# LANL-Bioinformatics/FaQCs

Measured on AMD Instinct MI355X. Metric: M reads/sec (paired 2x150bp), higher is better.
Workload: dtype u8; 1 GPU; synthetic 100M-pair 2x150bp Q33 reads resident in HBM per GPU, BWA_plus -q 5 --min_L 50, 1 step = 1 pass (trim_lds + counter all-reduce); pairs_per_gpu=100000000, read_len=150, terminal_n_supplied=True

## Files before the change

faqcs_amd/csrc/faqcs_capi.hip:

```cpp
#include "faqcs_ctx.h"

static uint8_t na_to_bits_host(char c)
{
    switch (c) {
    case 'A': case 'a': return 1;  case 'C': case 'c': return 2;  case 'G': case 'g': return 4;
    case 'T': case 't': return 8;  case 'M': case 'm': return 3;  case 'R': case 'r': return 5;
    case 'S': case 's': return 6;  case 'V': case 'v': return 7;  case 'W': case 'w': return 9;
    case 'Y': case 'y': return 10; case 'H': case 'h': return 11; case 'K': case 'k': return 12;
    case 'D': case 'd': return 13; case 'B': case 'b': return 14; case 'N': case 'n': return 15;
    case '-': return 16;
    }
    return 0;
}

static void build_tables(const faqcs_params &p, std::vector<uint32_t> &lcthr, std::vector<int32_t> &avgq,
                         std::vector<float> &norm, std::vector<uint32_t> &magic, std::vector<uint32_t> &base)
{
    const int N = FAQCS_TAB_LEN + 1;
    lcthr.assign(N, 0xffffffffu); avgq.assign(N, 0); norm.assign(N, 0.f); magic.assign(N, 0);
    const volatile float lc = p.low_complexity_cutoff_ratio;
    const volatile float avg = p.average_quality;
    for (int len = 1; len < N; ++len) {
        uint32_t mono = 0xffff, di = 0xffff;
        volatile float nrm = (float)(1.0 / (double)len);
// ... 40 lines not shown
    if (p->n_adapters > FAQCS_MAX_ADAPTERS)
        return fail(FAQCS_E_INVAL, "faqcs_create: " + std::to_string(p->n_adapters) + " adapters, at most " + std::to_string(FAQCS_MAX_ADAPTERS) + " are supported");
    if (p->mode < 0 || p->mode > 2) return fail(FAQCS_E_INVAL, "trim.cpp:trim_read: Undefined trimming mode!");
    if (p->quality < -93 || p->quality > 93) return fail(FAQCS_E_INVAL, "faqcs_create: quality threshold outside [-93, 93]");
    if (p->kmer_rarefaction && (p->kmer < 2 || p->kmer > 31 || p->split_size == 0)) return fail(FAQCS_E_INVAL, "faqcs_create: kmer / split_size out of range");
    int ndev = 0;
    if (hipGetDeviceCount(&ndev) != hipSuccess || ndev == 0)
        return fail(FAQCS_E_NODEVICE, "faqcs_create: no HIP device (the FaQCs MI355X hot path has no CPU fallback)");
    if (device_id < 0) HIPCHK(hipGetDevice(&device_id));
    HIPCHK(hipSetDevice(device_id));
    std::unique_ptr<faqcs_ctx, void (*)(faqcs_ctx *)> guard(new faqcs_ctx(), faqcs_destroy);
    faqcs_ctx *c = guard.get();
    c->prm = *p;
    c->prm.adapter_seq = nullptr;
    c->device = device_id;
    hipDeviceProp_t prop;
    HIPCHK(hipGetDeviceProperties(&prop, device_id));
    c->n_cu = prop.multiProcessorCount > 0 ? prop.multiProcessorCount : 256;
    HIPCHK(hipStreamCreateWithFlags(&c->compute, hipStreamNonBlocking));
    HIPCHK(hipStreamCreateWithFlags(&c->copy, hipStreamNonBlocking));
    HIPCHK(hipStreamCreateWithFlags(&c->aux, hipStreamNonBlocking));
    for (auto &rs : c->rec) { HIPCHK(hipEventCreateWithFlags(&rs.trimmed, hipEventDisableTiming)); HIPCHK(hipEventCreateWithFlags(&rs.folded, hipEventDisableTiming)); }
    HIPCHK(hipEventCreateWithFlags(&c->copied, hipEventDisableTiming));
    for (auto &sl : c->slot) HIPCHK(hipEventCreateWithFlags(&sl.done, hipEventDisableTiming));
    for (auto &e : c->ticket_ev) HIPCHK(hipEventCreateWithFlags(&e, hipEventDisableTiming));
    faqcs_counters_layout(p->max_read_length, p->n_adapters, &c->lay);

    std::vector<uint32_t> lcthr, magic, basetab; std::vector<int32_t> avgq; std::vector<float> norm;
    build_tables(*p, lcthr, avgq, norm, magic, basetab);
    HIPCHK(upload(&c->d_lcthr, lcthr)); HIPCHK(upload(&c->d_avgq, avgq)); HIPCHK(upload(&c->d_norm, norm));
    HIPCHK(upload(&c->d_magic, magic)); HIPCHK(upload(&c->d_basetab, basetab));
    HIPCHK(hipMalloc((void **)&c->d_counters, c->lay.total * sizeof(uint64_t)));
    HIPCHK(hipMemset(c->d_counters, 0, c->lay.total * sizeof(uint64_t)));
    HIPCHK(hipMalloc((void **)&c->d_err, 256));
    HIPCHK(hipMemset(c->d_err, 0, 256));
    {
        const size_t dwords = (size_t)c->n_cu * FAQCS_PARTIAL_FLUSHES * FAQCS_PARTIAL_ROW + (size_t)c->n_cu;
        HIPCHK(hipMalloc((void **)&c->d_partials, dwords * sizeof(uint32_t)));
        HIPCHK(hipMemset(c->d_partials, 0, dwords * sizeof(uint32_t)));
    }

    if (p->n_adapters) {
        std::vector<uint8_t> bits; std::vector<uint32_t> start(1, 0);
        for (uint32_t j = 0; j < p->n_adapters; ++j) {
            const char *s = p->adapter_seq[j];
            const size_t L = strlen(s);
            if (L == 0 || L > FAQCS_MAX_ADAPTER_LENGTH)
                return fail(FAQCS_E_INVAL, "faqcs_create: adapter " + std::to_string(j) + " has " + std::to_string(L) + " bases, 1 ... " +
                                               std::to_string(FAQCS_MAX_ADAPTER_LENGTH) + " are supported");
            c->adapters.emplace_back(s);
            for (size_t k = 0; k < L; ++k) {
                const uint8_t b = na_to_bits_host(s[k]);
                if (!b) return fail(FAQCS_E_BASE, "seq_overlap.cpp:na_to_bits: Unknown base!");
                bits.push_back(b);
            }
            start.push_back((uint32_t)bits.size());
        }
        std::vector<uint32_t> planes, wstart(1, 0);
        for (uint32_t j = 0; j < p->n_adapters; ++j) {
            const uint32_t L = start[j + 1] - start[j], nw = (L + 31) / 32;
            for (uint32_t w = 0; w < nw; ++w) {
                uint32_t pl[4] = {0, 0, 0, 0};
                for (uint32_t k = 0; k < 32 && 32 * w + k < L; ++k)
                    for (int b = 0; b < 4; ++b) pl[b] |= (uint32_t)((bits[start[j] + 32 * w + k] >> b) & 1u) << k;
                planes.insert(planes.end(), pl, pl + 4);
            }
            wstart.push_back(wstart.back() + nw);
        }
        HIPCHK(upload(&c->d_abits, bits)); HIPCHK(upload(&c->d_astart, start));
        HIPCHK(upload(&c->d_aplanes, planes)); HIPCHK(upload(&c->d_awstart, wstart));
        c->adapter_plane_dwords = (uint32_t)planes.size();
        for (uint32_t j = 0; j < p->n_adapters; ++j) c->adapter_longest = std::max(c->adapter_longest, start[j + 1] - start[j]);
        c->match_rate = (float)(1.0 - (double)p->filterAdapterMismatchRate);
        if (p->n_adapters > FAQCS_ADAPTER_GROUP || c->adapter_longest > FAQCS_ADAPTER_SINGLE_LENGTH) {
            std::vector<uint32_t> wgrp;
            for (uint32_t j = 0; j < p->n_adapters;) {
                faqcs_ctx::AdapterGroupHost g{j, 0, wstart[j], 0, 0};
                while (j < p->n_adapters && g.n < FAQCS_ADAPTER_GROUP && 4u * (wstart[j + 1] - g.w0) <= FAQCS_ADAPTER_TPL_CAP) {
                    g.longest = std::max(g.longest, start[j + 1] - start[j]);
                    ++g.n; ++j;
                }
                g.plane_dwords = 4u * (wstart[j] - g.w0);
                for (uint32_t k = g.j0; k <= j; ++k) wgrp.push_back(wstart[k] - g.w0);
                c->agroups.push_back(g);
            }
            HIPCHK(upload(&c->d_awstart_grp, wgrp));
        }
    }

    DevParams &d = c->dp;
    memset(&d, 0, sizeof(d));
    d.mode = p->mode; d.Q = p->quality; d.in_off = p->input_quality_offset; d.out_off = p->output_quality_offset;
    auto cap16 = [](uint32_t v) { return v > 65535u ? 65535u : v; };
    d.min_len = cap16(p->min_read_length); d.max_poly_n = cap16(p->max_num_poly_N); d.trim5 = cap16(p->trim_5); d.trim3 = cap16(p->trim_3);
    d.replace_q = p->replace_to_N_q; d.protect5 = p->protect_5; d.qc_only = p->qc_only;
    d.has_adapters = p->n_adapters ? 1 : 0; d.avgq_on = p->average_quality > 0.0f ? 1 : 0;
    d.R = p->max_read_length; d.n_adapters = p->n_adapters;
    d.lc_ratio = p->low_complexity_cutoff_ratio; d.avg_q = p->average_quality;
    if (const char *e = getenv("FAQCS_DBG")) d.dbg = (uint32_t)strtoul(e, nullptr, 0);
    d.lc_thr = c->d_lcthr; d.avgq_min_v = c->d_avgq; d.comp_norm = c->d_norm; d.div_magic = c->d_magic; d.base_tab = c->d_basetab;
    d.partials = c->d_partials;
    d.partial_rows = c->d_partials + (size_t)c->n_cu * FAQCS_PARTIAL_FLUSHES * FAQCS_PARTIAL_ROW;
    d.lay = c->lay;

    c->kmer_active = p->kmer_rarefaction ? 1 : 0;
    if (p->kmer_rarefaction) {
        uint64_t slots = p->kmer_table_slots ? p->kmer_table_slots : (1ull << 28);
        uint64_t pow2 = 1; while (pow2 < slots) pow2 <<= 1;
        if (pow2 < (uint64_t)KG_SLICE_MIN << 16) pow2 = (uint64_t)KG_SLICE_MIN << 16;
        if (pow2 > (uint64_t)KG_SLICE_MAX << 16) return fail(FAQCS_E_INVAL, "faqcs_create: kmer_table_slots above 2^32");
        c->kt.mask = pow2 - 1;
        { uint32_t lg = 0; while ((1ull << lg) < pow2) ++lg; if (lg > 46) return fail(FAQCS_E_INVAL, "faqcs_create: kmer_table_slots too large"); c->kt.shift = 62 - lg; }
        if (const char *e = getenv("FAQCS_KMER_DIRECT")) c->kg.direct = atoi(e) != 0;
        c->kt.ovf_mask = std::max<uint64_t>(pow2 >> 4, 1ull << 16) - 1;
        { const uint32_t lg = 62 - c->kt.shift;
          int f = (int)lg - 27; f = f < 0 ? 0 : (f > 3 ? 3 : f);
          if (const char *e = getenv("FAQCS_KMER_FINE_BITS")) { const int v = atoi(e); if (v >= 0 && v <= 3) f = v; }
          while (f > 0 && (pow2 >> (16 + f)) < 16) --f;
          while (f < 3 && (pow2 >> (16 + f)) > (uint64_t)KG_SLICE_MAX / 8) ++f;
          c->kt.fine = (uint32_t)f; }
        HIPCHK(hipMalloc((void **)&c->kt.dirty, (size_t)(1u << (16 + c->kt.fine)) / 8));
        HIPCHK(hipMemset(c->kt.dirty, 0, (size_t)(1u << (16 + c->kt.fine)) / 8));
        HIPCHK(hipMalloc((void **)&c->kt.slots, kmer_table_total(c->kt) * sizeof(KmerSlot)));
        HIPCHK(hipMalloc((void **)&c->kt.stats, 64));
        HIPCHK(faqcs_launch_kmer_table_init(c->kt, c->n_cu, c->compute));
        HIPCHK(hipMemset(c->kt.stats, 0, 64));
        c->snap_cap = 4096;
        HIPCHK(hipMalloc((void **)&c->d_snaps, c->snap_cap * 16));
    }
    *out = guard.release();
    return 0;
}

extern "C" void faqcs_destroy(faqcs_ctx *c)
{
    if (!c) return;
    (void)hipSetDevice(c->device);
    if (c->compute) (void)hipStreamSynchronize(c->compute);
    if (c->copy) (void)hipStreamSynchronize(c->copy);
    if (c->aux) (void)hipStreamSynchronize(c->aux);
    for (auto &t : c->timings) { (void)hipEventDestroy(t.a); (void)hipEventDestroy(t.b); (void)hipEventDestroy(t.p); (void)hipEventDestroy(t.k0); (void)hipEventDestroy(t.k1); }
    if (c->comm) comm_release(c->comm);
    if (c->comm_ev) (void)hipEventDestroy(c->comm_ev);
    c->emit.release(); c->parse.release(); c->render.release(); c->inflate.release(); c->deflate.release();
    if (c->ins_a) (void)hipEventDestroy(c->ins_a);
    if (c->ins_b) (void)hipEventDestroy(c->ins_b);
    for (int k = 0; k < 2; ++k) { if (c->fwd_free[k]) (void)hipEventDestroy(c->fwd_free[k]); if (c->fwd_copied[k]) (void)hipEventDestroy(c->fwd_copied[k]); c->fwd_items[k].release(); }
    void *ptrs[] = {c->d_lcthr, c->d_basetab, c->d_avgq, c->d_norm, c->d_magic, c->d_counters, c->d_err, c->d_partials, c->d_abits, c->d_astart, c->d_aplanes, c->d_awstart,
                    c->d_awstart_grp, c->kt.slots, c->kt.stats, c->kt.dirty, c->d_fold_claim, c->d_snaps, c->d_ob, c->d_tot_by_epoch, c->d_first_hist};
    for (void *q : ptrs) if (q) (void)hipFree(q);
    for (auto &sl : c->slot) { sl.seq.release(); sl.qual.release(); sl.tn.release(); sl.off.release(); if (sl.done) (void)hipEventDestroy(sl.done); }
    for (auto &e : c->ticket_ev) if (e) (void)hipEventDestroy(e);
    c->s_seg.release(); c->s_sl.release(); c->s_hit.release(); c->s_res.release(); c->s_astate.release(); c->s_amask.release();
    for (auto &rs : c->rec) { rs.pre.release(); rs.post.release(); if (rs.trimmed) (void)hipEventDestroy(rs.trimmed); if (rs.folded) (void)hipEventDestroy(rs.folded); }
    if (c->aux) (void)hipStreamDestroy(c->aux);
    c->ob_items.release(); c->ob_wave_count.release(); c->ob_wave_offset.release();
    { void *kg_ptrs[] = {c->kg.dev.l1, c->kg.dev.l2, c->kg.dev.cur1, c->kg.dev.cur2, c->kg.dev.run_epoch, c->kg.dev.first_hist, c->kg.dev.tot_by_epoch, c->kg.dev.dense, c->kg.dev.big, c->kg.dev.n_big, c->kg.dev.redo};
      for (void *q : kg_ptrs) if (q) (void)hipFree(q);
      c->kg.defer.release();
      c->ks.l1.release(); c->ks.spill.release(); c->ks.cur1.release(); c->ks.run_epoch.release(); c->ks.defer.release(); c->ks.scratch.release();
      for (auto &ev : c->kg.flush_ev) { (void)hipEventDestroy(ev.first); (void)hipEventDestroy(ev.second); } }
    if (c->copied) (void)hipEventDestroy(c->copied);
    if (c->compute) (void)hipStreamDestroy(c->compute);
    if (c->copy) (void)hipStreamDestroy(c->copy);
    delete c;
}

extern "C" int faqcs_set_quality(faqcs_ctx *c, int quality)
{
    if (!c) return fail(FAQCS_E_INVAL, "null ctx");
    if (quality < -93 || quality > 93) return fail(FAQCS_E_INVAL, "faqcs_set_quality: quality threshold outside [-93, 93]");
    c->prm.quality = quality;
    c->dp.Q = quality;
    return 0;
}

static int take_timing(faqcs_ctx *c, Timing *&tm)
{
    if (c->timing_used == c->timings.size()) {
        Timing t; HIPCHK(hipEventCreate(&t.a)); HIPCHK(hipEventCreate(&t.b)); HIPCHK(hipEventCreate(&t.p)); HIPCHK(hipEventCreate(&t.k0)); HIPCHK(hipEventCreate(&t.k1));
        t.adapter = false; t.kmer = false; c->timings.push_back(t);
    }
    tm = &c->timings[c->timing_used++];
    tm->adapter = c->prm.n_adapters != 0;
    tm->kmer = false;
    return 0;
}

static int enqueue_adapter(faqcs_ctx *c, Timing &t, const Submission &s)
{
    const uint32_t n = s.n;
    HIPCHK(hipEventRecord(t.p, c->compute));
    HIPCHK(c->s_sl.reserve(n)); HIPCHK(c->s_hit.reserve(n)); HIPCHK(c->s_seg.reserve(s.n_seg + 1));
    HIPCHK(hipMemcpyAsync(c->s_seg.p, s.seg, (s.n_seg + 1) * 4, hipMemcpyHostToDevice, c->compute));
    auto launch = [&](const AdapterDev &A, const AdapterGroup *G) {
        return faqcs_launch_adapter(A, G, s.seq, s.off, n, s.max_len, c->s_seg.p, s.n_seg, c->s_sl.p, c->s_hit.p,
                                    c->d_counters + c->lay.adapter_stats, c->d_err, c->dp.dbg, c->n_cu, c->compute);
    };
    if (c->agroups.empty()) {
        AdapterDev A{c->d_abits, c->d_astart, c->d_aplanes, c->d_awstart, c->prm.n_adapters, c->match_rate, c->adapter_longest, c->adapter_plane_dwords};
        HIPCHK(launch(A, nullptr));
        return 0;
    }
    AdapterGroup G{};
    G.mask_words = (s.max_len + 63) / 64;
    HIPCHK(c->s_astate.reserve(n)); HIPCHK(c->s_amask.reserve((size_t)n * G.mask_words));
    HIPCHK(hipMemsetAsync(c->s_astate.p, 0, (size_t)n * sizeof(uint4), c->compute));
    G.state = c->s_astate.p; G.mask = c->s_amask.p; G.gstart = c->d_astart;
    for (size_t k = 0; k < c->agroups.size(); ++k) {
        const faqcs_ctx::AdapterGroupHost &g = c->agroups[k];
        AdapterDev A{c->d_abits, c->d_astart + g.j0, c->d_aplanes + 4 * (size_t)g.w0, c->d_awstart_grp + g.j0 + k, g.n, c->match_rate,
                     g.longest, g.plane_dwords};
        G.j0 = g.j0; G.last = k + 1 == c->agroups.size() ? 1u : 0u;
        HIPCHK(launch(A, &G));
    }
    return 0;
}

static int enqueue_trim(faqcs_ctx *c, Timing &t, const Submission &s, const uint32_t *d_sl, const uint16_t *d_hit)
{
    const uint32_t n = s.n, max_len = s.max_len;
    HIPCHK(hipEventRecord(t.a, c->compute));
    const bool wide = max_len > 256;
    const int set = (int)(c->n_enqueued++ & 1);
    faqcs_ctx::RecSet &rs = c->rec[set];
    if (rs.used) { HIPCHK(hipStreamWaitEvent(c->compute, rs.folded, 0)); rs.used = false; }
    const char *e_long = getenv("FAQCS_TRIM_LONG");
    const bool force_long = e_long && atoi(e_long) != 0;
    const bool long_reads = max_len > FAQCS_FAST_READ_LENGTH || force_long;
    const size_t need = long_reads ? (size_t)n / 2 + 1 : (size_t)n * (wide ? 2 : 1);
    if (need > rs.pre.cap) { HIPCHK(hipStreamSynchronize(c->aux)); HIPCHK(hipStreamSynchronize(c->compute)); }
    HIPCHK(rs.pre.reserve(need)); HIPCHK(rs.post.reserve(need));
    DevParams dp = c->dp;
    static const bool tail_on = [] { const char *e = getenv("FAQCS_TAIL_FOLD"); return !e || atoi(e) != 0; }();
    if (c->pending_fold >= 0 && !c->pending_wide && tail_on) {
        const faqcs_ctx::RecSet &ps = c->rec[c->pending_fold];
        if (!c->d_fold_claim) HIPCHK(hipMalloc((void **)&c->d_fold_claim, 8));
        HIPCHK(hipMemsetAsync(c->d_fold_claim, 0, 8, c->compute));
        dp.fold_pre = ps.pre.p; dp.fold_post = ps.post.p; dp.fold_n = c->pending_n; dp.fold_claim = c->d_fold_claim;
        dp.fold_dst_pre = c->d_counters + c->lay.pre_comp; dp.fold_dst_post = c->d_counters + c->lay.post_comp;
    }
    HIPCHK(faqcs_launch_trim(dp, s.seq, s.qual, s.off, n, max_len, d_sl, d_hit, s.res, rs.pre.p, rs.post.p,
                             c->d_counters, c->d_err, c->n_cu, c->compute, s.tn));
    HIPCHK(hipEventRecord(t.b, c->compute));
    c->trim_kernel = faqcs_last_trim_kernel();
    if (c->pending_fold >= 0) {
        if (!(dp.fold_n && faqcs_last_trim_folded())) {
            faqcs_ctx::RecSet &ps = c->rec[c->pending_fold];
            HIPCHK(hipStreamWaitEvent(c->aux, ps.trimmed, 0));
            HIPCHK(faqcs_launch_composition(ps.pre.p, ps.post.p, c->pending_n, c->pending_wide, c->d_norm, c->d_counters + c->lay.pre_comp,
                                            c->d_counters + c->lay.post_comp, c->n_cu, c->aux));
            HIPCHK(hipEventRecord(ps.folded, c->aux));
            ps.used = true;
        }
        c->pending_fold = -1;
    }
    static const bool no_comp = [] { const char *e = getenv("FAQCS_DIAG_NO_COMPOSITION"); return e && atoi(e) != 0; }();
    if (!(c->dp.dbg & 1u) && !long_reads && !no_comp) {
        HIPCHK(hipEventRecord(rs.trimmed, c->compute));
        c->pending_fold = set; c->pending_n = n; c->pending_wide = wide;
    }
    return 0;
}

static int enqueue(faqcs_ctx *c, const uint8_t *d_seq, const uint8_t *d_qual, const uint32_t *d_off, uint32_t n,
                   uint32_t max_len, const uint32_t *seg, uint32_t n_seg, faqcs_read_result *d_res, const uint8_t *d_tn = nullptr,
                   const uint32_t *host_off = nullptr)
{
    const Submission s{d_seq, d_qual, d_tn, d_off, seg, host_off, n, max_len, n_seg, d_res};
    Timing *tm = nullptr;
    const bool adapters = s.n && c->prm.n_adapters;
    if (s.n) { if (int rc = take_timing(c, tm)) return rc; }
    if (adapters) { if (int rc = enqueue_adapter(c, *tm, s)) return rc; }
    if (s.n) { if (int rc = enqueue_trim(c, *tm, s, adapters ? c->s_sl.p : nullptr, adapters ? c->s_hit.p : nullptr)) return rc; }
    return enqueue_kmers(c, tm, s);
}

static int scan_offsets(const uint32_t *off, uint32_t n, uint32_t cap, uint32_t *max_len)
{
    uint32_t m = 0;
    for (uint32_t i = 0; i < n; ++i) {
        if (off[i + 1] < off[i]) return fail(FAQCS_E_INVAL, "faqcs_submit: offsets must be non-decreasing");
        const uint32_t l = off[i + 1] - off[i];
        m = l > m ? l : m;
    }
    if (m > cap) return fail(FAQCS_E_INVAL, "faqcs_submit: read longer than max_read_length");
    if (m > FAQCS_MAX_READ_LENGTH) return fail(FAQCS_E_INVAL, "faqcs_submit: reads longer than FAQCS_MAX_READ_LENGTH bases are not supported by the HIP kernels");
    *max_len = m;
    return 0;
}

static int check_segments(const faqcs_batch *b)
{
    if (!b || !b->offset) return fail(FAQCS_E_INVAL, "faqcs_submit: null batch");
    if (!b->segment_start || b->segment_start[0] != 0 || b->segment_start[b->n_segments] != b->n_reads)
        return fail(FAQCS_E_INVAL, "faqcs_submit: segment_start must span [0, n_reads]");
    for (uint32_t s = 0; s < b->n_segments; ++s)
        if (b->segment_start[s + 1] < b->segment_start[s]) return fail(FAQCS_E_INVAL, "faqcs_submit: segment_start must be non-decreasing");
    return 0;
}

extern "C" int faqcs_submit_async(faqcs_ctx *c, const faqcs_batch *b, faqcs_read_result *results, uint64_t *ticket)
{
    if (!c) return fail(FAQCS_E_INVAL, "null ctx");
    if (int rc = check_segments(b)) return rc;
    HIPCHK(hipSetDevice(c->device));
    const uint32_t n = b->n_reads;
    uint32_t max_len = 0;
    if (int rc = scan_offsets(b->offset, n, c->prm.max_read_length, &max_len)) return rc;
    const uint32_t o0 = b->offset[0], o1 = b->offset[n];
    const size_t bytes = (size_t)(o1 - o0);
    faqcs_ctx::Slot &sl = c->slot[c->n_submits & 1];
    hipEvent_t tk = c->ticket_ev[c->n_submits & 7];
    if (c->n_submits >= 8) HIPCHK(hipEventSynchronize(tk));
    if (sl.used) {
        if (bytes + FAQCS_ARENA_PAD_BEFORE + FAQCS_ARENA_PAD_AFTER > sl.seq.cap || (size_t)n + 1 > sl.off.cap || (b->terminal_n && (size_t)n + 64 > sl.tn.cap)) HIPCHK(hipEventSynchronize(sl.done));
        else HIPCHK(hipStreamWaitEvent(c->copy, sl.done, 0));
    }
    HIPCHK(sl.seq.reserve(bytes + FAQCS_ARENA_PAD_BEFORE + FAQCS_ARENA_PAD_AFTER)); HIPCHK(sl.qual.reserve(bytes + FAQCS_ARENA_PAD_BEFORE + FAQCS_ARENA_PAD_AFTER)); HIPCHK(sl.off.reserve((size_t)n + 1));
    if (b->terminal_n) HIPCHK(sl.tn.reserve((size_t)n + 64));
    if ((size_t)n + 1 > c->s_res.cap) HIPCHK(hipStreamSynchronize(c->compute));
    HIPCHK(c->s_res.reserve((size_t)n + 1));
    if (bytes) {
        HIPCHK(hipMemcpyAsync(sl.seq.p + 16, b->seq + o0, bytes, hipMemcpyHostToDevice, c->copy));
        HIPCHK(hipMemcpyAsync(sl.qual.p + 16, b->qual + o0, bytes, hipMemcpyHostToDevice, c->copy));
    }
    HIPCHK(hipMemcpyAsync(sl.off.p, b->offset, ((size_t)n + 1) * 4, hipMemcpyHostToDevice, c->copy));
    const uint8_t *d_tn = nullptr;
    if (b->terminal_n && n) {
        HIPCHK(hipMemcpyAsync(sl.tn.p, b->terminal_n, n, hipMemcpyHostToDevice, c->copy));
        d_tn = sl.tn.p;
    }
    HIPCHK(hipEventRecord(c->copied, c->copy));
    HIPCHK(hipStreamWaitEvent(c->compute, c->copied, 0));
    const uint8_t *d_seq = sl.seq.p + 16 - o0, *d_qual = sl.qual.p + 16 - o0;
    if (int rc = enqueue(c, d_seq, d_qual, sl.off.p, n, max_len, b->segment_start, b->n_segments, c->s_res.p, d_tn, b->offset)) return rc;
    if (n && results) HIPCHK(hipMemcpyAsync(results, c->s_res.p, (size_t)n * sizeof(faqcs_read_result), hipMemcpyDeviceToHost, c->compute));
    HIPCHK(hipEventRecord(sl.done, c->compute));
    HIPCHK(hipEventRecord(tk, c->compute));
    sl.used = true;
    if (ticket) *ticket = c->n_submits;
    ++c->n_submits;
    return 0;
}

extern "C" int faqcs_submit(faqcs_ctx *c, const faqcs_batch *b, faqcs_read_result *results)
{
    return faqcs_submit_async(c, b, results, nullptr);
}

extern "C" int faqcs_wait(faqcs_ctx *c, uint64_t ticket)
{
    if (!c) return fail(FAQCS_E_INVAL, "null ctx");
    if (ticket >= c->n_submits) return fail(FAQCS_E_INVAL, "faqcs_wait: unknown ticket");
    if (ticket + 8 < c->n_submits) return 0;
    HIPCHK(hipEventSynchronize(c->ticket_ev[ticket & 7]));
    return 0;
}

extern "C" void *faqcs_host_alloc(size_t bytes)
{
    void *p = nullptr;
    if (hipHostMalloc(&p, bytes, hipHostMallocPortable) != hipSuccess) return nullptr;
    return p;
}

extern "C" void faqcs_host_free(void *p)
{
    if (p) (void)hipHostFree(p);
}

extern "C" int faqcs_submit_device(faqcs_ctx *c, const faqcs_batch *b, faqcs_read_result *d_results)
{
    if (!c) return fail(FAQCS_E_INVAL, "null ctx");
    if (!b || !b->segment_start) return fail(FAQCS_E_INVAL, "faqcs_submit_device: null batch");
    HIPCHK(hipSetDevice(c->device));
    const uint32_t n = b->n_reads;
    uint32_t max_len = b->max_read_len ? b->max_read_len : c->prm.max_read_length;
    if (max_len > c->prm.max_read_length) return fail(FAQCS_E_INVAL, "faqcs_submit_device: max_read_len exceeds the context capacity");
    if (max_len > FAQCS_MAX_READ_LENGTH) return fail(FAQCS_E_INVAL, "faqcs_submit_device: reads longer than FAQCS_MAX_READ_LENGTH bases are not supported by the HIP kernels");
    if (!d_results) { HIPCHK(c->s_res.reserve((size_t)n + 1)); d_results = c->s_res.p; }
    return enqueue(c, b->seq, b->qual, b->offset, n, max_len, b->segment_start, b->n_segments, d_results, b->terminal_n);
}

extern "C" int faqcs_terminal_n_flags(int device_id, const uint8_t *d_seq, const uint32_t *d_offset, uint32_t n_reads, uint8_t *d_flags)
{
    if (!d_seq || !d_offset || !d_flags) return fail(FAQCS_E_INVAL, "null argument");
    if (device_id >= 0) HIPCHK(hipSetDevice(device_id));
    HIPCHK(faqcs_launch_terminal_n_flags(d_seq, d_offset, n_reads, d_flags, nullptr));
    HIPCHK(hipDeviceSynchronize());
    return 0;
}

int fold_pending_now(faqcs_ctx *c)
{
    if (c->pending_fold < 0) return 0;
    faqcs_ctx::RecSet &ps = c->rec[c->pending_fold];
    HIPCHK(faqcs_launch_composition(ps.pre.p, ps.post.p, c->pending_n, c->pending_wide, c->d_norm, c->d_counters + c->lay.pre_comp,
                                    c->d_counters + c->lay.post_comp, c->n_cu, c->compute));
    c->pending_fold = -1;
    return 0;
}

extern "C" int faqcs_sync(faqcs_ctx *c)
{
    if (!c) return fail(FAQCS_E_INVAL, "null ctx");
    HIPCHK(hipSetDevice(c->device));
    HIPCHK(hipStreamSynchronize(c->copy));
    if (int rc = fold_pending_now(c)) return rc;
    HIPCHK(hipStreamSynchronize(c->compute));
    HIPCHK(hipStreamSynchronize(c->aux));
    for (size_t i = 0; i < c->kg.flush_ev_used; ++i) {
        float ms = 0.f;
        if (hipEventElapsedTime(&ms, c->kg.flush_ev[i].first, c->kg.flush_ev[i].second) == hipSuccess) c->kmer_flush_ms += ms;
    }
    c->kg.flush_ev_used = 0;
    for (size_t i = 0; i < c->timing_used; ++i) {
        float ms = 0.f;
        if (hipEventElapsedTime(&ms, c->timings[i].a, c->timings[i].b) == hipSuccess) { c->kernel_ms += ms; ++c->kernel_launches; }
        if (c->timings[i].kmer && hipEventElapsedTime(&ms, c->timings[i].k0, c->timings[i].k1) == hipSuccess) c->kmer_ms += ms;
        if (c->timings[i].adapter && hipEventElapsedTime(&ms, c->timings[i].p, c->timings[i].a) == hipSuccess) c->adapter_ms += ms;
    }
    c->timing_used = 0;
    if (int rc = resolve_points(c)) return rc;
    uint32_t e = 0;
    HIPCHK(hipMemcpy(&e, c->d_err, 4, hipMemcpyDeviceToHost));
    if (e & 1u) return fail(FAQCS_E_QUALITY, "fastq.h:quality_score: Found a quality score value that is greater than the maximum allowed quality score");
    if (e & 2u) return fail(FAQCS_E_BASE, "seq_overlap.cpp:na_to_bits: Unknown base!");
    if (e & 4u) return fail(FAQCS_E_INVAL, "faqcs: internal error, the trim kernel's LDS block does not start at address 0");
    if (c->kt.stats) {
        unsigned long long st[3];
        HIPCHK(hipMemcpy(st, c->kt.stats, 24, hipMemcpyDeviceToHost));
        if (st[2] & 2ull) return fail(FAQCS_E_NOMEM, "faqcs: the k-mer exchange staging overflowed (more runs of k-mers per read than it is sized for): submit smaller batches");
        if (st[2]) return fail(FAQCS_E_KMER_FULL, "faqcs: device k-mer table is full (raise faqcs_params.kmer_table_slots)");
    }
    return 0;
}

extern "C" int faqcs_counters_device(faqcs_ctx *c, void **d_ptr, uint64_t *n_u64)
{
    if (!c || !d_ptr || !n_u64) return fail(FAQCS_E_INVAL, "null argument");
    *d_ptr = c->d_counters;
    *n_u64 = c->lay.total;
    return 0;
}

static int counters_copy(faqcs_ctx *c, void *d_dst, const void *d_src)
{
    HIPCHK(hipSetDevice(c->device));
    if (int rc = fold_pending_now(c)) return rc;
    HIPCHK(hipStreamSynchronize(c->aux));
    HIPCHK(hipMemcpyAsync(d_dst, d_src, c->lay.total * sizeof(uint64_t), hipMemcpyDeviceToDevice, c->compute));
    HIPCHK(hipStreamSynchronize(c->compute));
    return 0;
}

extern "C" int faqcs_counters_export(faqcs_ctx *c, void *d_dst, uint64_t n_u64)
{
    if (!c || !d_dst || n_u64 < c->lay.total) return fail(FAQCS_E_INVAL, "faqcs_counters_export: buffer too small");
    return counters_copy(c, d_dst, c->d_counters);
}

extern "C" int faqcs_counters_import(faqcs_ctx *c, const void *d_src, uint64_t n_u64)
{
    if (!c || !d_src || n_u64 < c->lay.total) return fail(FAQCS_E_INVAL, "faqcs_counters_import: buffer too small");
    return counters_copy(c, c->d_counters, d_src);
}

extern "C" int faqcs_finish(faqcs_ctx *c, uint64_t *counters, uint64_t n_u64)
{
    if (!c || !counters || n_u64 < c->lay.total) return fail(FAQCS_E_INVAL, "faqcs_finish: counter buffer too small");
    if (int rc = faqcs_sync(c)) return rc;
    HIPCHK(hipMemcpy(counters, c->d_counters, c->lay.total * sizeof(uint64_t), hipMemcpyDeviceToHost));
    return 0;
}

extern "C" int faqcs_reset_counters(faqcs_ctx *c)
{
    if (!c) return fail(FAQCS_E_INVAL, "null ctx");
    HIPCHK(hipSetDevice(c->device));
    c->pending_fold = -1;
    HIPCHK(hipStreamSynchronize(c->aux));
    HIPCHK(hipMemsetAsync(c->d_counters, 0, c->lay.total * sizeof(uint64_t), c->compute));
    return 0;
}

static int synth_fill_impl(int device_id, uint8_t *d_seq, uint8_t *d_qual, uint32_t *d_offset, uint32_t n_reads, uint32_t L,
                           uint64_t seed, uint64_t first_read, float adapter_frac, uint64_t genome_len)
{
    if (device_id >= 0) HIPCHK(hipSetDevice(device_id));
    if ((uint64_t)n_reads * L + L > 0xffffffffull) return fail(FAQCS_E_INVAL, "faqcs_synth_fill: arena exceeds 32-bit offsets");
    const char *at = getenv("FAQCS_SYNTH_AT");
    HIPCHK(faqcs_launch_synth(d_seq, d_qual, d_offset, n_reads, L, seed, first_read, adapter_frac, genome_len, at ? (float)atof(at) : -1.0f, nullptr));
    HIPCHK(hipDeviceSynchronize());
    return 0;
}

extern "C" int faqcs_synth_fill(int device_id, uint8_t *d_seq, uint8_t *d_qual, uint32_t *d_offset, uint32_t n_reads,
                                uint32_t L, uint64_t seed, uint64_t first_read, float adapter_frac)
{
    return synth_fill_impl(device_id, d_seq, d_qual, d_offset, n_reads, L, seed, first_read, adapter_frac, 0);
}

extern "C" int faqcs_synth_fill_genome(int device_id, uint8_t *d_seq, uint8_t *d_qual, uint32_t *d_offset, uint32_t n_reads,
                                       uint32_t L, uint64_t seed, uint64_t first_read, uint64_t genome_len)
{
    if (genome_len <= L) return fail(FAQCS_E_INVAL, "faqcs_synth_fill_genome: the genome must be longer than a read");
    return synth_fill_impl(device_id, d_seq, d_qual, d_offset, n_reads, L, seed, first_read, 0.f, genome_len);
}

extern "C" int faqcs_debug_words(faqcs_ctx *c, uint64_t *out, uint32_t n)
{
    if (!c || !out || n > 16) return fail(FAQCS_E_INVAL, "faqcs_debug_words: bad argument");
    HIPCHK(hipSetDevice(c->device));
    HIPCHK(hipStreamSynchronize(c->compute));
    HIPCHK(hipMemcpy(out, reinterpret_cast<const uint8_t *>(c->d_err) + 64, (size_t)n * 8, hipMemcpyDeviceToHost));
    HIPCHK(hipMemset(reinterpret_cast<uint8_t *>(c->d_err) + 64, 0, 128));
    return 0;
}

extern "C" int faqcs_kernel_report(faqcs_ctx *c, faqcs_kernel_times *out)
{
    if (!c || !out) return fail(FAQCS_E_INVAL, "null argument");
    if (int rc = faqcs_sync(c)) return rc;
    out->n_launches = c->kernel_launches;
    out->trim_ms = c->kernel_launches ? c->kernel_ms / (double)c->kernel_launches : 0.0;
    out->adapter_ms = c->kernel_launches ? c->adapter_ms / (double)c->kernel_launches : 0.0;
    out->trim_kernel = c->trim_kernel;
    out->kmer_ms = c->kernel_launches ? (c->kmer_ms + c->kmer_flush_ms) / (double)c->kernel_launches : 0.0;
    out->kmer_insert_ms = c->kernel_launches ? c->kmer_insert_ms / (double)c->kernel_launches : 0.0;
    c->kernel_ms = 0.0; c->adapter_ms = 0.0; c->kmer_ms = 0.0; c->kmer_insert_ms = 0.0; c->kmer_flush_ms = 0.0; c->kernel_launches = 0;
    return 0;
}

extern "C" int faqcs_kernel_time_ms(faqcs_ctx *c, double *avg_ms, uint64_t *n_launches)
{
    faqcs_kernel_times t;
    if (!c || !avg_ms || !n_launches) return fail(FAQCS_E_INVAL, "null argument");
    if (int rc = faqcs_kernel_report(c, &t)) return rc;
    *n_launches = t.n_launches; *avg_ms = t.trim_ms;
    return 0;
}
```

faqcs_amd/csrc/faqcs_ctx.h:

```cpp
#pragma once
#include <hip/hip_runtime.h>

#include <algorithm>
#include <cmath>
#include <cstdio>
#include <cstdlib>
#include <cstring>
#include <map>
#include <memory>
#include <string>
#include <vector>

#include "faqcs_dev.h"
#include "faqcs_host.h"
#include "faqcs_kmer.h"
#include "faqcs_skm.h"

struct AdapterDev {
    const uint8_t *bits;
    const uint32_t *start, *planes, *wstart;
    uint32_t n_adapters;
    float match_rate;
    uint32_t longest, plane_dwords;
};
const char *faqcs_last_trim_kernel();
bool faqcs_last_trim_folded();
hipError_t faqcs_launch_trim(const DevParams &P, const uint8_t *seq, const uint8_t *qual, const uint32_t *off,
                             uint32_t n_reads, uint32_t max_len, const uint32_t *ad_sl, const uint16_t *ad_hit,
                             faqcs_read_result *out, unsigned long long *rec_pre, unsigned long long *rec_post,
                             uint64_t *counters, uint32_t *err, int n_cu, hipStream_t st, const uint8_t *tn_flags);
hipError_t faqcs_launch_terminal_n_flags(const uint8_t *seq, const uint32_t *off, uint32_t n_reads, uint8_t *flags, hipStream_t st);
hipError_t faqcs_launch_composition(const unsigned long long *rec_pre, const unsigned long long *rec_post, uint32_t n, bool wide,
                                    const float *comp_norm, uint64_t *dst_pre, uint64_t *dst_post, int n_cu, hipStream_t st);
hipError_t faqcs_launch_adapter(const AdapterDev &A, const AdapterGroup *G, const uint8_t *seq, const uint32_t *off, uint32_t n_reads,
                                uint32_t max_len, const uint32_t *seg_start, uint32_t n_segments, uint32_t *ad_sl,
                                uint16_t *ad_hit, uint64_t *adapter_stats, uint32_t *err, uint32_t dbg, int n_cu, hipStream_t st);
hipError_t faqcs_launch_synth(uint8_t *d_seq, uint8_t *d_qual, uint32_t *d_offset, uint32_t n_reads, uint32_t L,
                              uint64_t seed, uint64_t first_read, float adapter_frac, uint64_t genome_len, float at_frac, hipStream_t st);

size_t faqcs_emit_scratch_bytes(uint32_t n_reads);
hipError_t faqcs_launch_emit_scan(const uint8_t *seq, const uint32_t *off, const uint8_t *tn, uint32_t n_reads, const faqcs_read_result *res,
                                  const uint8_t *keep, const faqcs_emit_out *out, void *scratch, hipStream_t st);
hipError_t faqcs_launch_emit_gather(const uint8_t *seq, const uint8_t *qual, uint32_t n_reads, const faqcs_emit_out *out, const void *scratch,
                                    int in_off, int out_off, uint32_t replace_q, int n_cu, hipStream_t st);

size_t faqcs_parse_scratch_bytes(unsigned long long n_text);
hipError_t faqcs_launch_parse_index(const uint8_t *text, unsigned long long n_text, int final, void *scratch, hipStream_t st);
hipError_t faqcs_launch_parse_records(const uint8_t *text, unsigned long long n_text, const faqcs_parse_out *out, void *scratch, int n_cu, hipStream_t st);
hipError_t faqcs_launch_parse_gather(const uint8_t *text, unsigned long long n_text, const faqcs_parse_out *out, const void *scratch, int n_cu, hipStream_t st);

size_t faqcs_render_scratch_bytes(uint32_t n_reads);
hipError_t faqcs_launch_render_scan(const faqcs_batch *b, const faqcs_read_result *res, const uint32_t *def_pos, const uint32_t *def_len,
                                    const uint8_t *select, const uint32_t *order, const faqcs_render_out *out, void *scratch, hipStream_t st);
hipError_t faqcs_launch_render_gather(const faqcs_batch *b, bool trimmed, const uint8_t *text, const faqcs_render_out *out, const void *scratch,
                                      int in_off, int out_off, uint32_t replace_q, int n_cu, hipStream_t st);

size_t faqcs_inflate_scratch_bytes(uint32_t n_members);
hipError_t faqcs_launch_inflate_scan(const uint8_t *comp, unsigned long long n_comp, const uint32_t *moff, uint32_t n, const faqcs_inflate_out *out, void *scratch, hipStream_t st);
hipError_t faqcs_launch_inflate_decode(const uint8_t *comp, const uint32_t *moff, uint32_t n, const faqcs_inflate_out *out, void *scratch, int n_cu, hipStream_t st);
size_t faqcs_deflate_scratch_bytes(uint32_t n, uint32_t n_data, uint32_t member_bytes, int n_cu);
hipError_t faqcs_launch_deflate_encode(const uint8_t *text, unsigned long long n_text, uint32_t member_bytes, uint32_t n, uint32_t n_data, void *scratch, int n_cu, hipStream_t st);
hipError_t faqcs_launch_deflate_gather(uint32_t member_bytes, uint32_t n, uint32_t n_data, const faqcs_deflate_out *out, void *scratch, int n_cu, hipStream_t st);

#define HIPCHK(x)                                                                                         \
    do {                                                                                                  \
        hipError_t e_ = (x);                                                                              \
        if (e_ != hipSuccess)                                                                             \
            return fail(FAQCS_E_NODEVICE, std::string(#x) + ": " + hipGetErrorString(e_));                \
    } while (0)

struct faqcs_ctx;

#pragma GCC visibility push(hidden)

template <class T> struct DevBuf {
    T *p = nullptr;
    size_t cap = 0;
    hipError_t reserve(size_t n)
    {
        if (n <= cap) return hipSuccess;
        if (p) (void)hipFree(p);
        p = nullptr; cap = 0;
        const size_t want = n + n / 4 + 64;
        hipError_t e = hipMalloc((void **)&p, want * sizeof(T));
        if (e == hipSuccess) cap = want;
        return e;
    }
    void release() { if (p) (void)hipFree(p); p = nullptr; cap = 0; }
};

struct Timing { hipEvent_t a, b, p, k0, k1; bool adapter, kmer; };

struct PackStage {
    DevBuf<uint4> scratch;
    hipEvent_t ev[3] = {nullptr, nullptr, nullptr};
    hipStream_t st = nullptr;
    bool timed = false;
    int begin(faqcs_ctx *c, size_t scratch_bytes);
    int mark(int i);
    int times(faqcs_ctx *c, const char *not_yet, double *first_ms, double *second_ms);
    void release();
};

#pragma GCC visibility pop

struct faqcs_ctx {
    faqcs_params prm;
    int device = 0, n_cu = 256;
    hipStream_t compute = nullptr, copy = nullptr;
    hipEvent_t copied = nullptr;
    DevParams dp;
    faqcs_layout lay;
    uint32_t *d_lcthr = nullptr, *d_magic = nullptr, *d_basetab = nullptr;
    int32_t *d_avgq = nullptr;
    float *d_norm = nullptr;
    uint64_t *d_counters = nullptr;
    uint32_t *d_err = nullptr;
    uint32_t *d_partials = nullptr;
    std::vector<std::string> adapters;
    uint8_t *d_abits = nullptr;
    uint32_t *d_astart = nullptr, *d_aplanes = nullptr, *d_awstart = nullptr;
    float match_rate = 0.f;
    uint32_t adapter_longest = 0, adapter_plane_dwords = 0;
    struct AdapterGroupHost { uint32_t j0, n, w0, longest, plane_dwords; };
    std::vector<AdapterGroupHost> agroups;
    uint32_t *d_awstart_grp = nullptr;
    DevBuf<uint4> s_astate;
    DevBuf<uint64_t> s_amask;
    struct Slot { DevBuf<uint8_t> seq, qual, tn; DevBuf<uint32_t> off; hipEvent_t done = nullptr; bool used = false; };
    Slot slot[2];
    uint64_t n_submits = 0;
    hipEvent_t ticket_ev[8] = {nullptr, nullptr, nullptr, nullptr, nullptr, nullptr, nullptr, nullptr};
    DevBuf<uint32_t> s_seg, s_sl;
    DevBuf<uint16_t> s_hit;
    DevBuf<faqcs_read_result> s_res;
    PackStage emit;
    PackStage parse;
    PackStage render;
    PackStage inflate;
    PackStage deflate;
    struct RecSet { DevBuf<unsigned long long> pre, post; hipEvent_t trimmed = nullptr, folded = nullptr; bool used = false; };
    RecSet rec[2];
    uint64_t n_enqueued = 0;
    int pending_fold = -1;
    uint32_t pending_n = 0;
    bool pending_wide = false;
    uint32_t *d_fold_claim = nullptr;
    hipStream_t aux = nullptr;
    uint64_t total_number = 0;
    int kmer_active = 0;
    std::vector<faqcs_rarefaction> points;
    struct PendingPoint { size_t point_index; size_t snap_index; };
    std::vector<PendingPoint> pending;
    KmerTable kt{nullptr, 0, nullptr, 0};
    bool partitioned = false;
    uint32_t part_rank = 0, part_world = 1, n_epochs = 0;
    std::vector<uint32_t> seg_epoch;
    DevBuf<ulonglong2> ob_items;
    bool ob_fresh = false;
    DevBuf<uint32_t> ob_wave_count;
    DevBuf<unsigned long long> ob_wave_offset;
    unsigned long long *d_ob = nullptr;
    unsigned long long *d_tot_by_epoch = nullptr, *d_first_hist = nullptr;
    unsigned long long *d_snaps = nullptr;
    size_t snap_cap = 0, n_snaps = 0;
    std::map<uint64_t, uint64_t> kmer_hist;
    struct KmerGroup {
        bool ready = false;
        bool direct = false;
        bool owner = false;
        bool skm = false;
        uint32_t skm_w = 1;
        DevBuf<uint32_t> defer;
        uint64_t cap_items = 0;
        uint64_t bound_items = 0;
        std::vector<uint32_t> run_epoch, upload[2];
        unsigned n_flushes = 0;
        uint64_t n_launches = 0;
        uint32_t epoch_base = 0;
        std::vector<uint64_t> sub_fill;
        KmerGroupDev dev{};
        uint32_t ep_cap = 0;
        uint32_t ep_used = 0;
        size_t points_final = 0;
        std::vector<std::pair<hipEvent_t, hipEvent_t>> flush_ev; size_t flush_ev_used = 0;
        bool table_live = false;
        bool pass_done = false;
        bool pass_used = false;
        bool hist_in_table = false;
        bool hist_in_overflow = false;
        uint64_t last_distinct = 0, last_total = 0;
    } kg;
    struct KmerSend {
        KmerGroupDev dev{};
        DevBuf<ulonglong2> l1, spill;
        DevBuf<uint32_t> cur1, run_epoch, defer;
        DevBuf<unsigned long long> scratch;
        uint32_t *spill_n = nullptr;
    } ks;
    std::vector<Timing> timings;
    size_t timing_used = 0;
    double kernel_ms = 0.0, adapter_ms = 0.0, kmer_ms = 0.0, kmer_insert_ms = 0.0, kmer_flush_ms = 0.0;
    uint64_t kernel_launches = 0;
    hipEvent_t ins_a = nullptr, ins_b = nullptr;
    DevBuf<ulonglong2> fwd_items[2];
    hipEvent_t fwd_free[2] = {nullptr, nullptr}, fwd_copied[2] = {nullptr, nullptr};
    unsigned fwd_n = 0;
    const char *trim_kernel = "";
    void *comm = nullptr;
    hipEvent_t comm_ev = nullptr;
};

struct Submission {
    const uint8_t *seq, *qual, *tn;
    const uint32_t *off, *seg, *host_off;
    uint32_t n, max_len, n_seg;
    faqcs_read_result *res;
};

FAQCS_HIDDEN int fold_pending_now(faqcs_ctx *c);
FAQCS_HIDDEN int enqueue_kmers(faqcs_ctx *c, Timing *tm, const Submission &s);
FAQCS_HIDDEN int resolve_points(faqcs_ctx *c);
FAQCS_HIDDEN void comm_release(void *comm);
```

faqcs_amd/csrc/faqcs_dev.h:

```cpp
#pragma once
#include <hip/hip_runtime.h>
#include <stdint.h>

#include "../../include/faqcs_mi.h"

#define FAQCS_WAVE 64
#define FAQCS_FAST_READ_LENGTH 1024
#define FAQCS_TAB_LEN FAQCS_FAST_READ_LENGTH

struct DevParams {
    int32_t mode, Q, in_off, out_off;
    uint32_t min_len, max_poly_n, trim5, trim3, replace_q;
    uint32_t protect5, qc_only, has_adapters, avgq_on;
    uint32_t R;
    uint32_t n_adapters;
    uint32_t dbg;
    uint32_t wide_records;
    float lc_ratio, avg_q;
    const uint32_t *lc_thr;
    const int32_t  *avgq_min_v;
    const uint32_t *div_magic;
    const float    *comp_norm;
    const uint32_t *base_tab;
    uint32_t *partials;
    uint32_t *partial_rows;
    faqcs_layout lay;
    const unsigned long long *fold_pre, *fold_post;
    uint32_t fold_n;
    uint32_t *fold_claim;
    uint64_t *fold_dst_pre, *fold_dst_post;
};

#define FAQCS_ADAPTER_GROUP 64
#define FAQCS_ADAPTER_TPL_CAP 4096
#define FAQCS_ADAPTER_SINGLE_LENGTH 8192

struct AdapterGroup {
    uint4 *state;
    uint64_t *mask;
    const uint32_t *gstart;
    uint32_t j0;
    uint32_t mask_words;
    uint32_t last;
};

enum { FS_SLOTS = 32 };
enum { FAQCS_PARTIAL_ROW = 16896 };
enum { FAQCS_PARTIAL_FLUSHES = 8 };

#define BT_SHIFT(code) (6 * (code))
#define BT_FIELDS 0x3fffffffu
#define BT_IS_NU (1u << 31)
#define BT_IS_GU (1u << 30)

#define CR_VALID (1ull << 63)

#ifdef __HIPCC__
__device__ __forceinline__ uint32_t umax_(uint32_t a, uint32_t b) { return a > b ? a : b; }
__device__ __forceinline__ uint32_t umin_(uint32_t a, uint32_t b) { return a < b ? a : b; }
__device__ __forceinline__ int uni(int v) { return __builtin_amdgcn_readfirstlane(v); }
__device__ __forceinline__ uint32_t uniu(uint32_t v) { return (uint32_t)__builtin_amdgcn_readfirstlane((int)v); }

__device__ __forceinline__ int wave_incl_scan_add(int v)
{
    v += __builtin_amdgcn_update_dpp(0, v, 0x111, 0xf, 0xf, false);
    v += __builtin_amdgcn_update_dpp(0, v, 0x112, 0xf, 0xf, false);
    v += __builtin_amdgcn_update_dpp(0, v, 0x114, 0xf, 0xf, false);
    v += __builtin_amdgcn_update_dpp(0, v, 0x118, 0xf, 0xf, false);
    v += __builtin_amdgcn_update_dpp(0, v, 0x142, 0xa, 0xf, false);
    v += __builtin_amdgcn_update_dpp(0, v, 0x143, 0xc, 0xf, false);
    return v;
}
__device__ __forceinline__ uint32_t wave_max_u32(uint32_t v)
{
    v = umax_(v, (uint32_t)__builtin_amdgcn_update_dpp(0, (int)v, 0x111, 0xf, 0xf, false));
    v = umax_(v, (uint32_t)__builtin_amdgcn_update_dpp(0, (int)v, 0x112, 0xf, 0xf, false));
    v = umax_(v, (uint32_t)__builtin_amdgcn_update_dpp(0, (int)v, 0x114, 0xf, 0xf, false));
    v = umax_(v, (uint32_t)__builtin_amdgcn_update_dpp(0, (int)v, 0x118, 0xf, 0xf, false));
    v = umax_(v, (uint32_t)__builtin_amdgcn_update_dpp(0, (int)v, 0x142, 0xa, 0xf, false));
    v = umax_(v, (uint32_t)__builtin_amdgcn_update_dpp(0, (int)v, 0x143, 0xc, 0xf, false));
    return (uint32_t)__builtin_amdgcn_readlane((int)v, 63);
}
__device__ __forceinline__ int wave_sum_i32(int v) { return __builtin_amdgcn_readlane(wave_incl_scan_add(v), 63); }

#define FAQCS_ROW_ALL(OP)                                                              \
    v = OP(v, __builtin_amdgcn_update_dpp(0, v, 0xB1, 0xf, 0xf, false));                \
    v = OP(v, __builtin_amdgcn_update_dpp(0, v, 0x4E, 0xf, 0xf, false));                \
    v = OP(v, __builtin_amdgcn_update_dpp(0, v, 0x141, 0xf, 0xf, false));               \
    v = OP(v, __builtin_amdgcn_update_dpp(0, v, 0x140, 0xf, 0xf, false));
__device__ __forceinline__ int op_add_(int a, int b) { return a + b; }
__device__ __forceinline__ int op_or_(int a, int b) { return a | b; }
__device__ __forceinline__ int op_umax_(int a, int b) { return (int)umax_((uint32_t)a, (uint32_t)b); }
__device__ __forceinline__ int row_all_sum(int v) { FAQCS_ROW_ALL(op_add_) return v; }
__device__ __forceinline__ uint32_t row_all_or(uint32_t x) { int v = (int)x; FAQCS_ROW_ALL(op_or_) return (uint32_t)v; }
__device__ __forceinline__ uint32_t row_all_umax(uint32_t x) { int v = (int)x; FAQCS_ROW_ALL(op_umax_) return (uint32_t)v; }
__device__ __forceinline__ int row_incl_scan_add(int v)
{
    v += __builtin_amdgcn_update_dpp(0, v, 0x111, 0xf, 0xf, false);
    v += __builtin_amdgcn_update_dpp(0, v, 0x112, 0xf, 0xf, false);
    v += __builtin_amdgcn_update_dpp(0, v, 0x114, 0xf, 0xf, false);
    v += __builtin_amdgcn_update_dpp(0, v, 0x118, 0xf, 0xf, false);
    return v;
}
__device__ __forceinline__ uint32_t row_next(uint32_t v) { return (uint32_t)__builtin_amdgcn_update_dpp(0, (int)v, 0x101, 0xf, 0xf, false); }
__device__ __forceinline__ uint32_t row_prev(uint32_t v) { return (uint32_t)__builtin_amdgcn_update_dpp(0, (int)v, 0x111, 0xf, 0xf, false); }
__device__ __forceinline__ uint32_t row_incl_scan_umax(uint32_t x)
{
    int v = (int)x;
    v = op_umax_(v, __builtin_amdgcn_update_dpp(0, v, 0x111, 0xf, 0xf, false));
    v = op_umax_(v, __builtin_amdgcn_update_dpp(0, v, 0x112, 0xf, 0xf, false));
    v = op_umax_(v, __builtin_amdgcn_update_dpp(0, v, 0x114, 0xf, 0xf, false));
    v = op_umax_(v, __builtin_amdgcn_update_dpp(0, v, 0x118, 0xf, 0xf, false));
    return (uint32_t)v;
}

template <int LPR> struct RowOps;
template <> struct RowOps<16> {
    static __device__ __forceinline__ int all_sum(int v) { return row_all_sum(v); }
    static __device__ __forceinline__ uint32_t all_or(uint32_t v) { return row_all_or(v); }
    static __device__ __forceinline__ uint32_t all_umax(uint32_t v) { return row_all_umax(v); }
    static __device__ __forceinline__ int incl_scan_add(int v) { return row_incl_scan_add(v); }
    static __device__ __forceinline__ uint32_t incl_scan_umax(uint32_t v) { return row_incl_scan_umax(v); }
    static __device__ __forceinline__ uint32_t next(uint32_t v) { return row_next(v); }
    static __device__ __forceinline__ uint32_t prev(uint32_t v) { return row_prev(v); }
};
template <> struct RowOps<8> {
#define FAQCS_HALF_ALL(OP)                                                             \
    v = OP(v, __builtin_amdgcn_update_dpp(0, v, 0xB1, 0xf, 0xf, false));                \
    v = OP(v, __builtin_amdgcn_update_dpp(0, v, 0x4E, 0xf, 0xf, false));                \
    v = OP(v, __builtin_amdgcn_update_dpp(0, v, 0x141, 0xf, 0xf, false));
    static __device__ __forceinline__ int all_sum(int v) { FAQCS_HALF_ALL(op_add_) return v; }
    static __device__ __forceinline__ uint32_t all_or(uint32_t x) { int v = (int)x; FAQCS_HALF_ALL(op_or_) return (uint32_t)v; }
    static __device__ __forceinline__ uint32_t all_umax(uint32_t x) { int v = (int)x; FAQCS_HALF_ALL(op_umax_) return (uint32_t)v; }
#undef FAQCS_HALF_ALL
    static __device__ __forceinline__ int ge_(int k) { return ((int)(threadIdx.x & 7u) >= k) ? -1 : 0; }
    static __device__ __forceinline__ int incl_scan_add(int v)
    {
        v += __builtin_amdgcn_update_dpp(0, v, 0x111, 0xf, 0xf, false) & ge_(1);
        v += __builtin_amdgcn_update_dpp(0, v, 0x112, 0xf, 0xf, false) & ge_(2);
        v += __builtin_amdgcn_update_dpp(0, v, 0x114, 0xf, 0xa, false);
        return v;
    }
    static __device__ __forceinline__ uint32_t incl_scan_umax(uint32_t x)
    {
        int v = (int)x;
        v = op_umax_(v, __builtin_amdgcn_update_dpp(0, v, 0x111, 0xf, 0xf, false) & ge_(1));
        v = op_umax_(v, __builtin_amdgcn_update_dpp(0, v, 0x112, 0xf, 0xf, false) & ge_(2));
        v = op_umax_(v, __builtin_amdgcn_update_dpp(0, v, 0x114, 0xf, 0xf, false) & ge_(4));
        return (uint32_t)v;
    }
    static __device__ __forceinline__ uint32_t next(uint32_t v)
    {
        return (uint32_t)__builtin_amdgcn_update_dpp(0, (int)v, 0x101, 0xf, 0xf, false) & (((threadIdx.x & 7u) == 7u) ? 0u : 0xffffffffu);
    }
    static __device__ __forceinline__ uint32_t prev(uint32_t v)
    {
        return (uint32_t)__builtin_amdgcn_update_dpp(0, (int)v, 0x111, 0xf, 0xf, false) & (uint32_t)ge_(1);
    }
};
template <> struct RowOps<4> {
#define FAQCS_QUAD_ALL(OP)                                                             \
    v = OP(v, __builtin_amdgcn_update_dpp(0, v, 0xB1, 0xf, 0xf, false));                \
    v = OP(v, __builtin_amdgcn_update_dpp(0, v, 0x4E, 0xf, 0xf, false));
    static __device__ __forceinline__ int all_sum(int v) { FAQCS_QUAD_ALL(op_add_) return v; }
    static __device__ __forceinline__ uint32_t all_or(uint32_t x) { int v = (int)x; FAQCS_QUAD_ALL(op_or_) return (uint32_t)v; }
    static __device__ __forceinline__ uint32_t all_umax(uint32_t x) { int v = (int)x; FAQCS_QUAD_ALL(op_umax_) return (uint32_t)v; }
#undef FAQCS_QUAD_ALL
    static __device__ __forceinline__ int ge_(int k) { return ((int)(threadIdx.x & 3u) >= k) ? -1 : 0; }
    static __device__ __forceinline__ int incl_scan_add(int v)
    {
        v += __builtin_amdgcn_update_dpp(0, v, 0x90, 0xf, 0xf, false) & ge_(1);
        v += __builtin_amdgcn_update_dpp(0, v, 0x44, 0xf, 0xf, false) & ge_(2);
        return v;
    }
    static __device__ __forceinline__ uint32_t incl_scan_umax(uint32_t x)
    {
        int v = (int)x;
        v = op_umax_(v, __builtin_amdgcn_update_dpp(0, v, 0x90, 0xf, 0xf, false) & ge_(1));
        v = op_umax_(v, __builtin_amdgcn_update_dpp(0, v, 0x44, 0xf, 0xf, false) & ge_(2));
        return (uint32_t)v;
    }
    static __device__ __forceinline__ uint32_t next(uint32_t v)
    {
// ... 74 lines not shown
```

faqcs_amd/csrc/faqcs_trim_common.h:

```cpp
#pragma once
#include "faqcs_dev.h"

#include <stdlib.h>

static inline hipError_t ensure_dynamic_lds(const void *kernel, size_t bytes, unsigned long long &done)
{
    int dev = 0;
    hipError_t e = hipGetDevice(&dev);
    if (e != hipSuccess) return e;
    const unsigned long long bit = 1ull << (dev & 63);
    if (__atomic_load_n(&done, __ATOMIC_ACQUIRE) & bit) return hipSuccess;
    e = hipFuncSetAttribute(kernel, hipFuncAttributeMaxDynamicSharedMemorySize, (int)bytes);
    if (e == hipSuccess) __atomic_fetch_or(&done, bit, __ATOMIC_RELEASE);
    return e;
}

namespace {

template <int C, int LPR, int WQ_ = 0> struct RowCfg {
    static constexpr int D = (C + 3) / 4;
    static constexpr int W = LPR * C;
    static constexpr int WQ = WQ_ ? WQ_ : W;
    static constexpr bool HQ8 = W > 768;
    static constexpr int HQ8_EVERY = 16;
    static constexpr int HQ = HQ8 ? FAQCS_NQ * W / 2 : FAQCS_NQ * WQ;
    static constexpr int KEY_BIAS = LPR <= 16 ? (1 << 16) : (1 << 18);
    static constexpr int PB = LPR <= 16 ? 9 : 11;
    static constexpr int FK = 2 * W;
    static constexpr int HB = FAQCS_NBASE * W;
    static constexpr int O_HQ = 0;
    static constexpr int O_HB = O_HQ + HQ;
    static constexpr int O_LEN = O_HB + HB;
    static constexpr int O_RQ = O_LEN + W + 2;
    static constexpr int O_BQPRE = O_RQ + 42;
    static constexpr int O_BQPOST = O_BQPRE + 42;
    static constexpr int O_FS = O_BQPOST + 42;
    static constexpr int N_ZERO = O_FS + FS_SLOTS;
    static constexpr int O_TBASE = N_ZERO;
    static constexpr int O_TLC = O_TBASE + 256;
    static constexpr int O_TAVGQ = O_TLC + W + 1;
    static constexpr int O_TMAGIC = O_TAVGQ + W + 1;
    static constexpr int BMW = D <= 4 ? 4 : 8;
    static constexpr int O_TBM = (O_TMAGIC + W + 1 + 3) & ~3;
    static constexpr int LDS_DWORDS = O_TBM + BMW * (C + 2);
    static constexpr int JB = C > 16 ? 5 : 4;
};

template <int D> struct __attribute__((packed, aligned(1))) PackedBytes { uint32_t w[D]; };

__device__ __forceinline__ int med3i(int x, int lo, int hi) { return x < lo ? lo : (x > hi ? hi : x); }

template <int C> __device__ __forceinline__ uint32_t range_mask(int lo, int hi, int pbase)
{
    const int s = med3i(lo - pbase, 0, C);
    int e = med3i(hi - pbase, 0, C);
    e = e > s ? e : s;
    uint32_t m;
    asm("v_bfm_b32 %0, %1, %2" : "=v"(m) : "v"(e - s), "v"(s));
    return m;
}
template <int K> __device__ __forceinline__ uint32_t byte_times4(uint32_t w, uint32_t two)
{
    uint32_t r;
    if (K == 0) asm("v_lshlrev_b32_sdwa %0, %1, %2 dst_sel:DWORD dst_unused:UNUSED_PAD src0_sel:DWORD src1_sel:BYTE_0" : "=v"(r) : "v"(two), "v"(w));
    else if (K == 1) asm("v_lshlrev_b32_sdwa %0, %1, %2 dst_sel:DWORD dst_unused:UNUSED_PAD src0_sel:DWORD src1_sel:BYTE_1" : "=v"(r) : "v"(two), "v"(w));
    else if (K == 2) asm("v_lshlrev_b32_sdwa %0, %1, %2 dst_sel:DWORD dst_unused:UNUSED_PAD src0_sel:DWORD src1_sel:BYTE_2" : "=v"(r) : "v"(two), "v"(w));
    else asm("v_lshlrev_b32_sdwa %0, %1, %2 dst_sel:DWORD dst_unused:UNUSED_PAD src0_sel:DWORD src1_sel:BYTE_3" : "=v"(r) : "v"(two), "v"(w));
    return r;
}
typedef const __attribute__((address_space(3))) uint32_t *lds_u32_ptr;
typedef __attribute__((address_space(3))) uint32_t *lds_u32_mut;
__device__ __forceinline__ void lds_add_u32(uint32_t byte_offset, uint32_t v)
{
    __hip_atomic_fetch_add((lds_u32_mut)(size_t)byte_offset, v, __ATOMIC_RELAXED, __HIP_MEMORY_SCOPE_WORKGROUP);
}
__device__ __forceinline__ void lds_add_u32_quiet(uint32_t byte_offset, uint32_t v)
{
    asm volatile("ds_add_u32 %0, %1" : : "v"(byte_offset), "v"(v) : "memory");
}
__device__ __forceinline__ void lds_add_u32_quiet(uint32_t *cell, uint32_t v) { lds_add_u32_quiet((uint32_t)(size_t)(lds_u32_mut)cell, v); }
template <int C, int J> struct BaseLookup {
    static __device__ __forceinline__ void run(const uint32_t t_base_lds, const uint32_t *ws, uint32_t two, uint32_t *inc)
    {
        inc[J] = *(lds_u32_ptr)(size_t)(byte_times4<J & 3>(ws[J >> 2], two) + t_base_lds);
        BaseLookup<C, J + 1>::run(t_base_lds, ws, two, inc);
    }
};
template <int C> struct BaseLookup<C, C> {
    static __device__ __forceinline__ void run(const uint32_t, const uint32_t *, uint32_t, uint32_t *) {}
};
__device__ __forceinline__ uint32_t umax3_(uint32_t a, uint32_t b, uint32_t c)
{
    uint32_t r;
    asm("v_max3_u32 %0, %1, %2, %3" : "=v"(r) : "v"(a), "v"(b), "v"(c));
    return r;
}
__device__ __forceinline__ int bit_m1(uint32_t mask, int j)
{
    int r;
    asm("v_bfe_i32 %0, %1, %2, 1" : "=v"(r) : "v"(mask), "n"(j));
    return r;
}

}

template <int C, int LPR, int NW, bool PAST_END = true>
__device__ __noinline__ void flush_block(uint32_t *smem, uint64_t *counters, const uint32_t R, const int tid)
{
    using Cfg = RowCfg<C, LPR>;
    constexpr int W = Cfg::W;
    uint32_t *hq = smem + Cfg::O_HQ, *hb = smem + Cfg::O_HB, *hlen = smem + Cfg::O_LEN, *hrq = smem + Cfg::O_RQ;
    uint32_t *hbqpre = smem + Cfg::O_BQPRE, *hbqpost = smem + Cfg::O_BQPOST, *lfs = smem + Cfg::O_FS;
    faqcs_layout L;
    {
        uint64_t o = 0;
        L.filter_stats = o;    o += 32;
        L.pre_read_qhist = o;  o += FAQCS_NQ;
        L.pre_base_qhist = o;  o += FAQCS_NQ;
        L.post_read_qhist = o; o += FAQCS_NQ;
        L.post_base_qhist = o; o += FAQCS_NQ;
        L.pre_len_hist = o;    o += (uint64_t)R + 1;
        L.post_len_hist = o;   o += (uint64_t)R + 1;
        L.pre_qual = o;        o += (uint64_t)R * FAQCS_NQ;
        L.post_qual = o;       o += (uint64_t)R * FAQCS_NQ;
        L.pre_base = o;        o += (uint64_t)R * FAQCS_NBASE;
        L.post_base = o;
    }
    __syncthreads();
    for (int i = tid; i < (Cfg::HQ8 ? 0 : Cfg::HQ); i += NW * 64) {
        const uint32_t v = hq[i];
        if (v) {
            hq[i] = 0;
            const uint32_t q = i / W, p = i % W;
            uint32_t pre = v & 0xffffu;
            if (PAST_END && q == 0) {
                uint32_t shorter = 0;
                for (uint32_t l = 0; l <= p; ++l) shorter += hlen[l] & 0xffffu;
                pre -= shorter;
            }
            if (p < R) {
                if (pre) atomicAdd((unsigned long long *)(counters + L.pre_qual + (uint64_t)p * FAQCS_NQ + q), (unsigned long long)pre);
                if (v >> 16) atomicAdd((unsigned long long *)(counters + L.post_qual + (uint64_t)p * FAQCS_NQ + q), (unsigned long long)(v >> 16));
            }
        }
    }
    __syncthreads();
    for (int i = tid; i < Cfg::HB; i += NW * 64) {
        const uint32_t v = hb[i];
        if (v) {
            hb[i] = 0;
            const uint32_t c = i / W, p = i % W;
            if (p < R) {
                if (v & 0xffffu) atomicAdd((unsigned long long *)(counters + L.pre_base + (uint64_t)p * FAQCS_NBASE + c), (unsigned long long)(v & 0xffffu));
                if (v >> 16) atomicAdd((unsigned long long *)(counters + L.post_base + (uint64_t)p * FAQCS_NBASE + c), (unsigned long long)(v >> 16));
            }
        }
    }
    for (int i = tid; i <= W; i += NW * 64) {
        const uint32_t v = hlen[i];
        if (v && (uint32_t)i <= R) {
            hlen[i] = 0;
            if (v & 0xffffu) atomicAdd((unsigned long long *)(counters + L.pre_len_hist + i), (unsigned long long)(v & 0xffffu));
            if (v >> 16) atomicAdd((unsigned long long *)(counters + L.post_len_hist + i), (unsigned long long)(v >> 16));
        }
    }
    if (tid < FAQCS_NQ) {
        const uint32_t v = hrq[tid], x = hbqpre[tid], y = hbqpost[tid];
        hrq[tid] = 0; hbqpre[tid] = 0; hbqpost[tid] = 0;
        if (v & 0xffffu) atomicAdd((unsigned long long *)(counters + L.pre_read_qhist + tid), (unsigned long long)(v & 0xffffu));
        if (v >> 16) atomicAdd((unsigned long long *)(counters + L.post_read_qhist + tid), (unsigned long long)(v >> 16));
        if (x) atomicAdd((unsigned long long *)(counters + L.pre_base_qhist + tid), (unsigned long long)x);
        if (y) atomicAdd((unsigned long long *)(counters + L.post_base_qhist + tid), (unsigned long long)y);
    }
    if (tid >= 64 && tid < 64 + FAQCS_NUM_STAT) {
        const int k = tid - 64;
        const uint32_t v = lfs[k];
        if (v) { atomicAdd((unsigned long long *)(counters + L.filter_stats + k), (unsigned long long)v); lfs[k] = 0; }
    }
    __syncthreads();
}

template <int C, int LPR, int NW>
__device__ __noinline__ void flush_hq8(uint32_t *smem, uint64_t *counters, const uint32_t R, const int tid)
{
    using Cfg = RowCfg<C, LPR>;
    constexpr int HW = Cfg::W / 2;
    uint32_t *hq = smem + Cfg::O_HQ;
    const uint64_t pre_qual = 32 + 4 * FAQCS_NQ + 2 * ((uint64_t)R + 1), post_qual = pre_qual + (uint64_t)R * FAQCS_NQ;
    __syncthreads();
    for (int i = tid; i < Cfg::HQ; i += NW * 64) {
        const uint32_t v = hq[i];
        if (v) {
            hq[i] = 0;
            const uint32_t q = i / HW, p = 2u * (uint32_t)(i % HW);
#pragma unroll
            for (int h = 0; h < 2; ++h) {
                const uint32_t a = (v >> (16 * h)) & 0xffu, b = (v >> (16 * h + 8)) & 0xffu;
                if (p + h < R) {
                    if (a) atomicAdd((unsigned long long *)(counters + pre_qual + (uint64_t)(p + h) * FAQCS_NQ + q), (unsigned long long)a);
                    if (b) atomicAdd((unsigned long long *)(counters + post_qual + (uint64_t)(p + h) * FAQCS_NQ + q), (unsigned long long)b);
                }
            }
        }
    }
    __syncthreads();
}

struct ReadOutcome {
    uint32_t an, fl, pAT, pCG, cAT, cCG, N;
    int Vpre, Vpost;
};
struct FsAcc { uint32_t tot = 0, trim = 0, len = 0, qt = 0; };
__device__ __forceinline__ void fs_acc_flush(FsAcc &f, const int lane, uint32_t *lfs)
{
    const uint32_t m = (1u << 20) - 1u;
    const uint32_t s_tot = (uint32_t)wave_sum_i32((int)f.tot), s_trim = (uint32_t)wave_sum_i32((int)f.trim), s_len = (uint32_t)wave_sum_i32((int)f.len);
    const uint32_t s_qt = (uint32_t)wave_sum_i32((int)f.qt);
    const uint32_t s_nn = 0, s_lc = 0, s_avg = 0;
    if (lane == 0) {
        if (s_tot) { lds_add_u32_quiet(&lfs[FAQCS_TOTAL_COUNT], s_tot >> 20); lds_add_u32_quiet(&lfs[FAQCS_TOTAL_NUMBER], s_tot >> 20); lds_add_u32_quiet(&lfs[FAQCS_TOTAL_LENGTH], s_tot & m); }
        if (s_trim) { lds_add_u32_quiet(&lfs[FAQCS_TOTAL_TRIMMED_NUMBER], s_trim >> 20); lds_add_u32_quiet(&lfs[FAQCS_TOTAL_TRIMMED_LENGTH], s_trim & m); }
        if (s_len) { lds_add_u32_quiet(&lfs[FAQCS_READ_LENGTH], s_len >> 20); lds_add_u32_quiet(&lfs[FAQCS_BASE_LENGTH], s_len & m); }
        if (s_nn) { lds_add_u32_quiet(&lfs[FAQCS_READ_NN], s_nn >> 20); lds_add_u32_quiet(&lfs[FAQCS_BASE_NN], s_nn & m); }
        if (s_avg) { lds_add_u32_quiet(&lfs[FAQCS_READ_AVG_Q], s_avg >> 20); lds_add_u32_quiet(&lfs[FAQCS_BASE_AVG_Q], s_avg & m); }
        if (s_qt) { lds_add_u32_quiet(&lfs[FAQCS_READ_QUAL_TRIM], s_qt >> 20); lds_add_u32_quiet(&lfs[FAQCS_BASE_QUAL_TRIM], s_qt & m); }
        if (s_lc) { lds_add_u32_quiet(&lfs[FAQCS_READ_LOW_COMPLEXITY], s_lc >> 20); lds_add_u32_quiet(&lfs[FAQCS_BASE_LOW_COMPLEXITY], s_lc & m); }
    }
    f = FsAcc();
}

__device__ __forceinline__ void chunk_epilogue_pre(const bool mine, const bool e_err, const uint32_t e_len, const int Vpre, const int lane, uint32_t *hlen,
                                                   uint32_t *hrq, uint32_t *hbqpre, const uint32_t *t_magic, FsAcc *defer)
{
        int qb_pre = 0;
        if (mine && e_len > 0 && Vpre > 0) qb_pre = e_len == 1 ? Vpre : (int)__umulhi((uint32_t)Vpre, t_magic[e_len]);
        qb_pre = qb_pre > 41 ? 41 : qb_pre;
        const bool act = mine && !e_err;
        if (act) {
            const uint32_t key = e_len | ((uint32_t)qb_pre << 16);
            const bool same = key == (uint32_t)__builtin_amdgcn_readfirstlane((int)key);
            const uint32_t cnt = (uint32_t)__builtin_popcountll(__ballot(same));
            if (same) {
                if (lane == __ffsll((unsigned long long)__ballot(true)) - 1) {
                    lds_add_u32_quiet(hlen + e_len, cnt);
                    lds_add_u32_quiet(hrq + qb_pre, cnt);
                    if (e_len) lds_add_u32_quiet(hbqpre + qb_pre, cnt * e_len);
                }
            } else {
                lds_add_u32_quiet(hlen + e_len, 1u);
                lds_add_u32_quiet(hrq + qb_pre, 1u);
                if (e_len) lds_add_u32_quiet(hbqpre + qb_pre, e_len);
            }
        }
        const uint32_t one = 1u << 20;
        defer->tot += mine ? one | e_len : 0u;
}

template <int LPR>
__device__ __forceinline__ void chunk_epilogue(const ReadOutcome &o, const bool mine, const uint32_t my, const uint32_t v_len,
                                               const uint32_t v_hit, const int lane, uint32_t *hlen, uint32_t *hrq, uint32_t *hbqpre,
                                               uint32_t *hbqpost, uint32_t *lfs, const uint32_t *t_magic, uint2 *__restrict__ out,
                                               unsigned long long *__restrict__ rec_pre, unsigned long long *__restrict__ rec_post,
                                               const bool o_avgq_on, const uint32_t o_dbg, FsAcc *defer = nullptr, const bool wide_rt = false,
                                               const bool pre_done = false)
{
        const bool e_ret = (o.fl & FAQCS_F_VALID) != 0, e_err = (o.fl & FAQCS_F_ERR_QUALITY) != 0;
        const uint32_t e_len = v_len, e_n = o.an >> 16, e_filt = (o.fl & FAQCS_F_FILTER_MASK) >> FAQCS_F_FILTER_SHIFT;
        int qb_pre = 0, qb_post = 0;
        if (!defer && mine && e_len > 0 && o.Vpre > 0) qb_pre = e_len == 1 ? o.Vpre : (int)__umulhi((uint32_t)o.Vpre, t_magic[e_len]);
        if (e_ret && o.Vpost > 0) qb_post = e_n == 1 ? o.Vpost : (int)__umulhi((uint32_t)o.Vpost, t_magic[e_n]);
        qb_pre = qb_pre > 41 ? 41 : qb_pre;
        qb_post = qb_post > 41 ? 41 : qb_post;
        if (defer) {
            if (!pre_done) chunk_epilogue_pre(mine, e_err, e_len, o.Vpre, lane, hlen, hrq, hbqpre, t_magic, defer);
            const bool act = mine && !e_err;
            if (act && e_ret) {
                const uint32_t key = e_n | ((uint32_t)qb_post << 16);
                const bool same = key == (uint32_t)__builtin_amdgcn_readfirstlane((int)key);
                const uint32_t cnt = (uint32_t)__builtin_popcountll(__ballot(same));
                if (same) {
                    if (lane == __ffsll((unsigned long long)__ballot(true)) - 1) {
                        lds_add_u32_quiet(hlen + e_n, cnt << 16);
                        lds_add_u32_quiet(hrq + qb_post, cnt << 16);
                        lds_add_u32_quiet(hbqpost + qb_post, cnt * e_n);
                    }
                } else {
                    lds_add_u32_quiet(hlen + e_n, 0x10000u);
                    lds_add_u32_quiet(hrq + qb_post, 0x10000u);
                    lds_add_u32_quiet(hbqpost + qb_post, e_n);
                }
            }
        } else if (!(o_dbg & 2u) && mine && !e_err) {
            atomicAdd(hlen + e_len, 1u);
            atomicAdd(hrq + qb_pre, 1u);
            if (e_len) atomicAdd(hbqpre + qb_pre, e_len);
            if (e_ret) {
                atomicAdd(hlen + e_n, 0x10000u);
                atomicAdd(hrq + qb_post, 0x10000u);
                atomicAdd(hbqpost + qb_post, e_n);
            }
        }
        if (mine) {
            const bool bad_base = v_hit == 0xffffu;
            out[my] = make_uint2(e_ret ? o.an : 0u, (o.fl & 0x3ffu) | (bad_base ? (uint32_t)FAQCS_F_ERR_BASE : (v_hit << 16)));
            const bool pre_on = !e_err, post_on = e_ret && !e_err;
            const unsigned long long pA = o.pAT & 0xffffu, pT = o.pAT >> 16, pC = o.pCG & 0xffffu, pG = o.pCG >> 16, pn = o.N & 0xffffu;
            const unsigned long long cA = o.cAT & 0xffffu, cT = o.cAT >> 16, cC = o.cCG & 0xffffu, cG = o.cCG >> 16, cn = o.N >> 16;
            if (LPR <= 16 && !wide_rt) {
                rec_pre[my] = pre_on ? (CR_VALID | e_len | (pA << 9) | (pT << 18) | (pC << 27) | (pG << 36) | (pn << 45)) : 0ull;
                rec_post[my] = post_on ? (CR_VALID | e_n | (cA << 9) | (cT << 18) | (cC << 27) | (cG << 36) | (cn << 45)) : 0ull;
            } else {
                reinterpret_cast<ulonglong2 *>(rec_pre)[my] =
                    pre_on ? make_ulonglong2(CR_VALID | e_len | (pA << 11) | (pT << 22) | (pC << 33), pG | (pn << 11)) : make_ulonglong2(0ull, 0ull);
                reinterpret_cast<ulonglong2 *>(rec_post)[my] =
                    post_on ? make_ulonglong2(CR_VALID | e_n | (cA << 11) | (cT << 22) | (cC << 33), cG | (cn << 11)) : make_ulonglong2(0ull, 0ull);
            }
        }
        const bool e_rlen = e_filt == FAQCS_FILT_LENGTH_PRE || e_filt == FAQCS_FILT_LENGTH_POST;
        const uint32_t one = 1u << 20;
        if (defer) {
            defer->trim += e_ret ? one | e_n : 0u;
            defer->len += e_rlen ? one | e_n : 0u;
            defer->qt += (o.fl & FAQCS_F_QUAL_TRIMMED) ? one | (o.fl >> 20) : 0u;
            const uint32_t m = one - 1u;
            const bool is_nn = (o.fl & FAQCS_F_POLY_N_SEEN) != 0, is_lc = e_filt == FAQCS_FILT_LOW_COMPLEXITY, is_avg = o_avgq_on && e_filt == FAQCS_FILT_AVG_Q;
            if (__any(is_nn)) { const uint32_t v = (uint32_t)wave_sum_i32((int)(is_nn ? one | e_n : 0u)); if (lane == 0) { lds_add_u32_quiet(&lfs[FAQCS_READ_NN], v >> 20); lds_add_u32_quiet(&lfs[FAQCS_BASE_NN], v & m); } }
            if (__any(is_lc)) { const uint32_t v = (uint32_t)wave_sum_i32((int)(is_lc ? one | e_n : 0u)); if (lane == 0) { lds_add_u32_quiet(&lfs[FAQCS_READ_LOW_COMPLEXITY], v >> 20); lds_add_u32_quiet(&lfs[FAQCS_BASE_LOW_COMPLEXITY], v & m); } }
            if (__any(is_avg)) { const uint32_t v = (uint32_t)wave_sum_i32((int)(is_avg ? one | e_n : 0u)); if (lane == 0) { lds_add_u32_quiet(&lfs[FAQCS_READ_AVG_Q], v >> 20); lds_add_u32_quiet(&lfs[FAQCS_BASE_AVG_Q], v & m); } }
            return;
        }
        const uint32_t s_tot = (uint32_t)wave_sum_i32((int)(mine ? one | e_len : 0u));
        const uint32_t s_trim = (uint32_t)wave_sum_i32((int)(e_ret ? one | e_n : 0u));
        const uint32_t s_len = (uint32_t)wave_sum_i32((int)(e_rlen ? one | e_n : 0u));
        const uint32_t s_nn = (uint32_t)wave_sum_i32((int)((o.fl & FAQCS_F_POLY_N_SEEN) ? one | e_n : 0u));
        const uint32_t s_qt = (uint32_t)wave_sum_i32((int)((o.fl & FAQCS_F_QUAL_TRIMMED) ? one | (o.fl >> 20) : 0u));
        const uint32_t s_lc = (uint32_t)wave_sum_i32((int)(e_filt == FAQCS_FILT_LOW_COMPLEXITY ? one | e_n : 0u));
        uint32_t s_avg = 0;
        if (o_avgq_on) s_avg = (uint32_t)wave_sum_i32((int)(e_filt == FAQCS_FILT_AVG_Q ? one | e_n : 0u));
        if (lane == 0) {
            const uint32_t m = one - 1u;
            if (s_tot) { atomicAdd(&lfs[FAQCS_TOTAL_COUNT], s_tot >> 20); atomicAdd(&lfs[FAQCS_TOTAL_NUMBER], s_tot >> 20); atomicAdd(&lfs[FAQCS_TOTAL_LENGTH], s_tot & m); }
            if (s_trim) { atomicAdd(&lfs[FAQCS_TOTAL_TRIMMED_NUMBER], s_trim >> 20); atomicAdd(&lfs[FAQCS_TOTAL_TRIMMED_LENGTH], s_trim & m); }
            if (s_len) { atomicAdd(&lfs[FAQCS_READ_LENGTH], s_len >> 20); atomicAdd(&lfs[FAQCS_BASE_LENGTH], s_len & m); }
            if (s_nn) { atomicAdd(&lfs[FAQCS_READ_NN], s_nn >> 20); atomicAdd(&lfs[FAQCS_BASE_NN], s_nn & m); }
            if (s_avg) { atomicAdd(&lfs[FAQCS_READ_AVG_Q], s_avg >> 20); atomicAdd(&lfs[FAQCS_BASE_AVG_Q], s_avg & m); }
            if (s_qt) { atomicAdd(&lfs[FAQCS_READ_QUAL_TRIM], s_qt >> 20); atomicAdd(&lfs[FAQCS_BASE_QUAL_TRIM], s_qt & m); }
            if (s_lc) { atomicAdd(&lfs[FAQCS_READ_LOW_COMPLEXITY], s_lc >> 20); atomicAdd(&lfs[FAQCS_BASE_LOW_COMPLEXITY], s_lc & m); }
        }
}

#ifdef __HIPCC__
template <int NT>
__device__ __forceinline__ void comp_fold_tail(uint32_t *tab, const DevParams &P, const int tid, const uint32_t which)
{
    constexpr int NE = FAQCS_NCOMP_BIN * FAQCS_NCOMP_KIND, ND = (NE + 1) / 2, U = 4;
    constexpr uint32_t CHUNK = NT * U, PER_CLAIM = 5, FLUSH_CLAIMS = 65535u / (CHUNK * PER_CLAIM);
    static_assert(FLUSH_CLAIMS >= 1, "a claim must fit the 16-bit counters");
    float *normt = reinterpret_cast<float *>(tab + ND);
    uint32_t *s_next = tab + ND + 512;
    const uint32_t n = P.fold_n, n_chunks = (n + CHUNK - 1) / CHUNK;
    if (tid == 0)
        *s_next = (__hip_atomic_load(&P.fold_claim[0], __ATOMIC_RELAXED, __HIP_MEMORY_SCOPE_AGENT) >= n_chunks &&
                   __hip_atomic_load(&P.fold_claim[1], __ATOMIC_RELAXED, __HIP_MEMORY_SCOPE_AGENT) >= n_chunks) ? 1u : 0u;
    __syncthreads();
    const bool nothing_left = *s_next != 0u;
    __syncthreads();
    if (nothing_left) return;
    for (int i = tid; i < ND; i += NT) tab[i] = 0;
    for (int i = tid; i < 512; i += NT) normt[i] = i <= FAQCS_TAB_LEN ? P.comp_norm[i] : 0.0f;
    __syncthreads();
#pragma unroll 1
    for (uint32_t pass = 0; pass < 2; ++pass) {
        const uint32_t a = which ^ pass;
        const unsigned long long *__restrict__ rec = a ? P.fold_post : P.fold_pre;
        uint64_t *__restrict__ dst = a ? P.fold_dst_post : P.fold_dst_pre;
        uint32_t since_flush = 0;
        bool dirty = false;
#pragma unroll 1
        for (;;) {
            if (tid == 0) *s_next = atomicAdd(&P.fold_claim[a], PER_CLAIM);
            __syncthreads();
            const uint32_t c0 = *s_next;
            __syncthreads();
            if (c0 >= n_chunks) break;
            dirty = true;
#pragma unroll 1
            for (uint32_t c = c0; c < c0 + PER_CLAIM && c < n_chunks; ++c) {
                unsigned long long x[U];
#pragma unroll
                for (int u = 0; u < U; ++u) { const uint32_t i = c * CHUNK + (uint32_t)(u * NT + tid); x[u] = i < n ? rec[i] : 0ull; }
#pragma unroll
                for (int u = 0; u < U; ++u) {
                    uint32_t nbin = 0xffffffffu;
                    if (x[u] & CR_VALID) {
                        const uint32_t len = (uint32_t)(x[u] & 511u);
                        uint32_t cnt[5];
#pragma unroll
                        for (int k = 0; k < 5; ++k) cnt[k] = (uint32_t)(x[u] >> (9 + 9 * k)) & 511u;
                        const float norm = normt[len];
                        uint32_t idx[6];
#pragma unroll
                        for (int k = 0; k < 5; ++k) idx[k] = (uint32_t)__fmul_rn(norm, (float)cnt[k]);
                        idx[5] = idx[3] + idx[2];
#pragma unroll
                        for (int k = 0; k < 6; ++k) {
                            if (k == 4) continue;
                            const uint32_t e = idx[k] * FAQCS_NCOMP_KIND + k;
                            atomicAdd(&tab[e >> 1], 1u << (16 * (e & 1u)));
                        }
                        nbin = idx[4] * FAQCS_NCOMP_KIND + 4;
                    }
                    constexpr uint32_t bin0 = 4u;
                    const unsigned long long zero = __ballot(nbin == bin0);
                    if (zero != 0ull && (tid & 63) == __builtin_ctzll(zero)) atomicAdd(&tab[bin0 >> 1], (uint32_t)__popcll(zero) << (16 * (bin0 & 1u)));
                    if (nbin != 0xffffffffu && nbin != bin0) atomicAdd(&tab[nbin >> 1], 1u << (16 * (nbin & 1u)));
                }
            }
            if (++since_flush == FLUSH_CLAIMS) {
                __syncthreads();
                for (int d = tid; d < ND; d += NT) {
                    const uint32_t v = tab[d];
                    if (v) {
                        tab[d] = 0;
                        if (v & 0xffffu) atomicAdd((unsigned long long *)(dst + 2 * d), (unsigned long long)(v & 0xffffu));
                        if (v >> 16) atomicAdd((unsigned long long *)(dst + 2 * d + 1), (unsigned long long)(v >> 16));
                    }
                }
                __syncthreads();
                since_flush = 0; dirty = false;
            }
        }
        if (dirty) {
            __syncthreads();
            for (int d = tid; d < ND; d += NT) {
                const uint32_t v = tab[d];
                if (v) {
                    tab[d] = 0;
                    if (v & 0xffffu) atomicAdd((unsigned long long *)(dst + 2 * d), (unsigned long long)(v & 0xffffu));
                    if (v >> 16) atomicAdd((unsigned long long *)(dst + 2 * d + 1), (unsigned long long)(v >> 16));
                }
            }
            __syncthreads();
        }
    }
}
#endif
```

faqcs_amd/csrc/faqcs_trim_kernel.hip:

```cpp
#include "faqcs_trim_common.h"

#ifndef FAQCS_TRIM_NW
#define FAQCS_TRIM_NW 4
#endif
#ifndef FAQCS_TRIM_MINWAVES
#define FAQCS_TRIM_MINWAVES 3
#endif

template <int C, int LPR, int NW, bool WINDOWED, bool GENERIC>
__global__ __launch_bounds__(NW * 64, (LPR == 8 || C > 10) ? 2 : FAQCS_TRIM_MINWAVES) void trim_filter_accumulate(
    const DevParams P, const uint8_t *__restrict__ seq, const uint8_t *__restrict__ qual,
    const uint32_t *__restrict__ off, const uint32_t n_reads, const uint32_t *__restrict__ ad_sl,
    const uint16_t *__restrict__ ad_hit, uint2 *__restrict__ out, unsigned long long *__restrict__ rec_pre,
    unsigned long long *__restrict__ rec_post, uint64_t *__restrict__ counters, uint32_t *__restrict__ err)
{
    using Cfg = RowCfg<C, LPR>;
    using RW = RowOps<LPR>;
    constexpr int D = Cfg::D, W = Cfg::W, KEY_BIAS = Cfg::KEY_BIAS, PB = Cfg::PB, FK = Cfg::FK;
    constexpr uint32_t PMX = (1u << PB) - 1u;
    constexpr int JB = Cfg::JB;
    constexpr uint32_t JM = (1u << JB) - 1u;
    static_assert(!Cfg::HQ8 || NW * Cfg::HQ8_EVERY <= 255, "an 8-bit cell must not overflow between two flushes");
    constexpr uint32_t CMASK = (1u << C) - 1u;
    extern __shared__ __attribute__((aligned(16))) uint32_t smem[];
// ... 340 lines not shown
#pragma unroll
                            for (int j = 0; j < C; ++j) {
                                const uint32_t lastnon = umax_(umax_(excl, loc[j]), (uint32_t)a);
                                best = umax_(best, ((nw >> j) & 1u) ? (uint32_t)(pbase + j) + 1u - lastnon : 0u);
                            }
                            trip = RW::all_umax(best) >= K;
                        }
                    }
                    if (trip) {
                        flags |= FAQCS_F_POLY_N_SEEN;
                        if (!o_qc_only) { ret = false; filt = FAQCS_FILT_POLY_N; }
                    }
                }

                uint32_t cAT = pAT, cCG = pCG, cN = pN;
                int V_post = V_pre;
                uint32_t repbits = 0;
                if (o_replace_q > 0) {
#pragma unroll
                    for (int j = 0; j < C; ++j) repbits |= (uint32_t)(q[j] < (int)o_replace_q) << j;
                    repbits &= gubits & win2;
                }
                if (!(o_dbg & 16u) && __any(ret && (!whole || repbits))) {
                    uint32_t cp = 0;
#pragma unroll
                    for (int j = 0; j < C; ++j) {
                        const uint32_t w = ((repbits >> j) & 1u) ? (1u << BT_SHIFT(4)) : incf[j];
                        cp += w & (uint32_t)bit_m1(win2, j);
                    }
                    const uint32_t at = (cp & 63u) | (((cp >> 6) & 63u) << 16), cg = ((cp >> 12) & 63u) | (((cp >> 18) & 63u) << 16);
                    cAT = (uint32_t)RW::all_sum((int)at);
                    cCG = (uint32_t)RW::all_sum((int)cg);
                    cN = (uint32_t)RW::all_sum((int)((cp >> 24) & 63u));
                    const bool clean = V_pre == len * Q - (WINDOWED ? 0 : T) && !WINDOWED;
                    if (__all(!ret || (clean && have_sums))) {
                        V_post = n * Q - (hi_sum - lo_sum);
                    } else {
                        int sv = 0;
#pragma unroll
                        for (int j = 0; j < C; ++j) {
                            const int sq = (int)(int8_t)((wq[j >> 2] >> (8 * (j & 3))) & 0xffu);
                            sv += (sq - in_off) & bit_m1(win2, j);
                        }
                        V_post = RW::all_sum(sv);
                    }
                }
                const uint32_t cA = cAT & 0xffffu, cT = cAT >> 16, cC = cCG & 0xffffu, cG = cCG >> 16;

                if (ret && o_avgq_on && V_post < t_avgq[n]) { ret = false; filt = FAQCS_FILT_AVG_Q; }

                if (ret && !(o_dbg & 16u)) {
                    const uint32_t thr = t_lc[n];
                    const uint32_t mthr = thr & 0xffffu, dthr = thr >> 16;
                    bool trip = cA >= mthr || cT >= mthr || cG >= mthr || cC >= mthr;
                    const uint32_t nbig = (cA >= dthr) + (cT >= dthr) + (cC >= dthr) + (cG >= dthr);
                    if (__any(!trip && nbig >= 2)) {
                        uint32_t cls[C];
#pragma unroll
                        for (int j = 0; j < C; ++j) {
                            const uint32_t w = (((repbits >> j) & 1u) ? 0u : incf[j] & 0xffffffu) & (uint32_t)bit_m1(win2, j);
                            cls[j] = w ? (uint32_t)(__builtin_ctz(w) / 6) : 7u;
                        }
                        const uint32_t prev_last = RW::prev(cls[C - 1] + 1u);
                        const uint32_t cnts[4] = {cA, cT, cC, cG};
#pragma unroll
                        for (int x = 0; x < 4; ++x)
#pragma unroll
                            for (int y = 0; y < 4; ++y)
                                if (x != y) {
                                    int dc = 0;
#pragma unroll
                                    for (int j = 0; j < C; ++j) {
                                        const uint32_t pv = j ? cls[j - 1] : prev_last - 1u;
                                        dc += (pv == (uint32_t)x && cls[j] == (uint32_t)y) ? 1 : 0;
                                    }
                                    dc = RW::all_sum(dc);
                                    trip = trip || (cnts[x] >= dthr && cnts[y] >= dthr && (uint32_t)dc >= dthr);
                                }
                    }
                    if (trip) { ret = false; filt = FAQCS_FILT_LOW_COMPLEXITY; }
                }

                if (read_err) { any_err = 1; flags |= FAQCS_F_ERR_QUALITY; }
                if (!(o_dbg & 2u)) {
                    if (__any(read_err)) {
#pragma unroll
                        for (int j = 0; j < C; ++j) { q[j] = read_err ? 0 : q[j]; incf[j] = read_err ? 0u : incf[j]; }
                    }
                    const uint32_t inr = Cfg::HQ8 ? ((act && !read_err) ? range_mask<C>(0, len, pbase) : 0u) : 0u;
                    const uint32_t counted = (act && !read_err) ? 1u : 0u;
                    const uint32_t pb4 = 4u * (uint32_t)pbase;
                    const uint32_t postm = ret ? (Cfg::HQ8 ? (win2 & inr) : win2) : 0u;
                    if (Cfg::HQ8) {
#pragma unroll
                        for (int j = 0; j < C; ++j) {
                            const int qq = q[j];
                            const uint32_t x = ((inr >> j) & 1u) | ((uint32_t)bit_m1(postm, j) & 0x100u);
                            lds_add_u32(__umul24((uint32_t)qq, (uint32_t)(W / 2 * 4)) + (uint32_t)(Cfg::O_HQ * 4) + 4u * (uint32_t)((pbase + j) >> 1),
                                        x << (16 * ((pbase + j) & 1)));
                        }
                    }
                    if (o_replace_q > 0) {
#pragma unroll
                        for (int j = 0; j < C; ++j) {
                            const int qq = q[j];
                            if (!Cfg::HQ8) lds_add_u32(__umul24((uint32_t)qq, (uint32_t)(W * 4)) + pb4 + (uint32_t)(Cfg::O_HQ * 4 + 4 * j),
                                                       counted | ((uint32_t)bit_m1(postm, j) & 0x10000u));
                            bpre[j] += incf[j];
                            const uint32_t w = ((repbits >> j) & 1u) ? (1u << BT_SHIFT(4)) : incf[j];
                            bpost[j] += w & (uint32_t)bit_m1(postm, j);
                        }
                    } else {
#pragma unroll
                        for (int j = 0; j < C; ++j) {
                            const int qq = q[j];
                            if (!Cfg::HQ8) lds_add_u32(__umul24((uint32_t)qq, (uint32_t)(W * 4)) + pb4 + (uint32_t)(Cfg::O_HQ * 4 + 4 * j),
                                                       counted | ((uint32_t)bit_m1(postm, j) & 0x10000u));
                            bpre[j] += incf[j];
                            bpost[j] += incf[j] & (uint32_t)bit_m1(postm, j);
                        }
                    }
                }

                if (rl == t) {
                    st_an = (uint32_t)a | ((uint32_t)n << 16);
                    st_fl = flags | (ret ? FAQCS_F_VALID : 0u) | (filt << FAQCS_F_FILTER_SHIFT) | (qt_removed << 20);
                    st_pAT = pAT; st_pCG = pCG; st_cAT = cAT; st_cCG = cCG; st_N = pN | (cN << 16);
                    st_Vpre = V_pre; st_Vpost = V_post;
                }
                if (Cfg::HQ8 && (t % Cfg::HQ8_EVERY) == Cfg::HQ8_EVERY - 1) flush_hq8<C, LPR, NW>(smem, counters, P.R, tid);
            }

            if (!(o_dbg & 32u)) {
                const ReadOutcome oc{st_an, st_fl, st_pAT, st_pCG, st_cAT, st_cCG, st_N, st_Vpre, st_Vpost};
                chunk_epilogue<LPR>(oc, mine, my, v_len, v_hit, lane, smem + Cfg::O_LEN, smem + Cfg::O_RQ, smem + Cfg::O_BQPRE,
                                    smem + Cfg::O_BQPOST, smem + Cfg::O_FS, smem + Cfg::O_TMAGIC, out, rec_pre, rec_post, o_avgq_on, o_dbg);
            }
        }

        const bool block_flush = ((it + 1) % FLUSH_EVERY) == 0 || it + 1 == n_iter;
        if (((it + 1) % REG_FLUSH_EVERY) == 0 || block_flush) spill_base_regs();

        if (block_flush && !(o_dbg & 64u)) flush_block<C, LPR, NW>(smem, counters, P.R, tid);
    }
    if (__any(any_err != 0) && lane == 0) atomicOr(err, 1u);
}

#ifndef FAQCS_COMP_U
#define FAQCS_COMP_U 4
#endif
template <int NT, bool WIDE>
__global__ __launch_bounds__(NT) void composition_histogram(const unsigned long long *__restrict__ rec_a, const unsigned long long *__restrict__ rec_b,
                                                            const uint32_t n, const float *__restrict__ comp_norm,
                                                            uint64_t *__restrict__ dst_a, uint64_t *__restrict__ dst_b )
{
    constexpr int NE = FAQCS_NCOMP_BIN * FAQCS_NCOMP_KIND;
    constexpr int ND = (NE + 1) / 2;
    constexpr int U = FAQCS_COMP_U;
    extern __shared__ __attribute__((aligned(16))) uint32_t tab[];
    const int tid = threadIdx.x;
    const bool second = (blockIdx.x & 1u) != 0u;
    const unsigned long long *__restrict__ rec = second ? rec_b : rec_a;
    uint64_t *__restrict__ dst = second ? dst_b : dst_a;
    const uint32_t bid = blockIdx.x >> 1, nblk = gridDim.x >> 1;
    float *normt = reinterpret_cast<float *>(tab + ND);
    constexpr int NNORM = WIDE ? FAQCS_TAB_LEN + 1 : 512;
    for (int i = tid; i < ND; i += NT) tab[i] = 0;
    for (int i = tid; i < NNORM; i += NT) normt[i] = i <= FAQCS_TAB_LEN ? comp_norm[i] : 0.0f;
    __syncthreads();
    const uint32_t per_round = nblk * NT * U;
    const uint32_t rounds = (n + per_round - 1) / per_round;
    constexpr uint32_t FLUSH_EVERY = 65535u / (NT * U);
    for (uint32_t r = 0; r < rounds; ++r) {
        const uint32_t i0 = (r * nblk + bid) * (NT * U) + tid;
        unsigned long long x[U], y[U];
#pragma unroll
        for (int u = 0; u < U; ++u) {
            const uint32_t i = i0 + u * NT;
            x[u] = 0; y[u] = 0;
            if (i < n) {
                if (WIDE) { const ulonglong2 v = reinterpret_cast<const ulonglong2 *>(rec)[i]; x[u] = v.x; y[u] = v.y; }
                else x[u] = rec[i];
            }
        }
#pragma unroll
        for (int u = 0; u < U; ++u) {
            uint32_t nbin = 0xffffffffu;
            if (x[u] & CR_VALID) {
                uint32_t len, cnt[5];
                if (WIDE) {
                    len = (uint32_t)(x[u] & 2047u);
                    cnt[0] = (uint32_t)(x[u] >> 11) & 2047u; cnt[1] = (uint32_t)(x[u] >> 22) & 2047u; cnt[2] = (uint32_t)(x[u] >> 33) & 2047u;
                    cnt[3] = (uint32_t)y[u] & 2047u; cnt[4] = (uint32_t)(y[u] >> 11) & 2047u;
                } else {
                    len = (uint32_t)(x[u] & 511u);
#pragma unroll
                    for (int k = 0; k < 5; ++k) cnt[k] = (uint32_t)(x[u] >> (9 + 9 * k)) & 511u;
                }
                const float norm = normt[len];
                uint32_t idx[6];
#pragma unroll
                for (int k = 0; k < 5; ++k) idx[k] = (uint32_t)__fmul_rn(norm, (float)cnt[k]);
                idx[5] = idx[3] + idx[2];
#pragma unroll
                for (int k = 0; k < 6; ++k) {
                    if (k == 4) continue;
                    const uint32_t e = idx[k] * FAQCS_NCOMP_KIND + k;
                    atomicAdd(&tab[e >> 1], 1u << (16 * (e & 1u)));
                }
                nbin = idx[4] * FAQCS_NCOMP_KIND + 4;
            }
            {
                constexpr uint32_t bin0 = 4u;
                const unsigned long long zero = __ballot(nbin == bin0);
                if (zero != 0ull && (int)(threadIdx.x & 63u) == __builtin_ctzll(zero)) atomicAdd(&tab[bin0 >> 1], (uint32_t)__popcll(zero) << (16 * (bin0 & 1u)));
                if (nbin != 0xffffffffu && nbin != bin0) atomicAdd(&tab[nbin >> 1], 1u << (16 * (nbin & 1u)));
            }
        }
        if (((r + 1) % FLUSH_EVERY) == 0 || r + 1 == rounds) {
            __syncthreads();
            for (int d = tid; d < ND; d += NT) {
                const uint32_t v = tab[d];
                if (v) {
                    tab[d] = 0;
                    if (v & 0xffffu) atomicAdd((unsigned long long *)(dst + 2 * d), (unsigned long long)(v & 0xffffu));
                    if (v >> 16) atomicAdd((unsigned long long *)(dst + 2 * d + 1), (unsigned long long)(v >> 16));
                }
            }
            __syncthreads();
        }
    }
}

template <int C, int LPR, int NW, bool WINDOWED, bool GENERIC>
static hipError_t launch_trim_t(const DevParams &P, const uint8_t *seq, const uint8_t *qual, const uint32_t *off,
                                uint32_t n_reads, const uint32_t *ad_sl, const uint16_t *ad_hit, faqcs_read_result *out,
                                unsigned long long *rec_pre, unsigned long long *rec_post, uint64_t *counters, uint32_t *err,
                                int n_cu, hipStream_t st)
{
    constexpr size_t lds = (size_t)RowCfg<C, LPR>::LDS_DWORDS * 4;
    static unsigned long long attr_done = 0;
    auto kern = trim_filter_accumulate<C, LPR, NW, WINDOWED, GENERIC>;
    if (hipError_t e = ensure_dynamic_lds(reinterpret_cast<const void *>(kern), lds, attr_done); e != hipSuccess) return e;
    const uint32_t chunks = (n_reads + 63) / 64;
    int blocks_per_cu = (int)((160 * 1024) / lds);
    constexpr int minwaves = (LPR == 8 || C > 10) ? 2 : (FAQCS_TRIM_MINWAVES > 2 ? FAQCS_TRIM_MINWAVES : 2);
    const int by_waves = (4 * minwaves + NW - 1) / NW;
    if (blocks_per_cu > by_waves) blocks_per_cu = by_waves;
    if (blocks_per_cu < 1) blocks_per_cu = 1;
    uint32_t grid = (chunks + NW - 1) / NW;
    const uint32_t cap = (uint32_t)(n_cu * blocks_per_cu);
    if (grid > cap) grid = cap;
    if (grid == 0) return hipSuccess;
    hipLaunchKernelGGL(kern, dim3(grid), dim3(NW * 64), lds, st, P, seq, qual, off, n_reads, ad_sl, ad_hit,
                       reinterpret_cast<uint2 *>(out), rec_pre, rec_post, counters, err);
    return hipGetLastError();
}

template <int C, int LPR, int NW, class... Args>
static hipError_t launch_trim_variant(const bool windowed, const bool generic, const Args &...args)
{
    return windowed ? (generic ? launch_trim_t<C, LPR, NW, true, true>(args...) : launch_trim_t<C, LPR, NW, true, false>(args...))
                    : (generic ? launch_trim_t<C, LPR, NW, false, true>(args...) : launch_trim_t<C, LPR, NW, false, false>(args...));
}

hipError_t faqcs_launch_trim_long(const DevParams &P, const uint8_t *seq, const uint8_t *qual, const uint32_t *off, uint32_t n_reads,
                                  const uint32_t *ad_sl, const uint16_t *ad_hit, faqcs_read_result *out, uint64_t *counters, uint32_t *err,
                                  int n_cu, hipStream_t st, uint32_t *lead_trail, uint32_t max_len);
hipError_t faqcs_launch_trim_lds(const DevParams &P, const uint8_t *seq, const uint8_t *qual, const uint32_t *off,
                                 uint32_t n_reads, uint32_t max_len, const uint32_t *ad_sl, const uint16_t *ad_hit,
                                 faqcs_read_result *out, unsigned long long *rec_pre, unsigned long long *rec_post,
                                 uint64_t *counters, uint32_t *err, int n_cu, hipStream_t st, const uint8_t *tn_flags);

static thread_local const char *g_last_trim_kernel = "";
const char *faqcs_last_trim_kernel() { return g_last_trim_kernel; }
bool faqcs_trim_lds_tail_folded();
static thread_local bool g_last_trim_folded = false;
bool faqcs_last_trim_folded() { return g_last_trim_folded; }

hipError_t faqcs_launch_trim(const DevParams &P, const uint8_t *seq, const uint8_t *qual, const uint32_t *off,
                             uint32_t n_reads, uint32_t max_len, const uint32_t *ad_sl, const uint16_t *ad_hit,
                             faqcs_read_result *out, unsigned long long *rec_pre, unsigned long long *rec_post,
                             uint64_t *counters, uint32_t *err, int n_cu, hipStream_t st, const uint8_t *tn_flags)
{
    g_last_trim_folded = false;
    {
        const char *e_long = getenv("FAQCS_TRIM_LONG");
        const bool force_long = e_long && atoi(e_long) != 0;
        if (max_len > FAQCS_FAST_READ_LENGTH || force_long) {
            g_last_trim_kernel = "trim_long";
            return faqcs_launch_trim_long(P, seq, qual, off, n_reads, ad_sl, ad_hit, out, counters, err, n_cu, st, reinterpret_cast<uint32_t *>(rec_pre), max_len);
        }
    }
    {
        static const bool lds_on = [] { const char *e = getenv("FAQCS_TRIM_LDS"); return !e || atoi(e) != 0; }();
        if (lds_on) {
            const hipError_t e = faqcs_launch_trim_lds(P, seq, qual, off, n_reads, max_len, ad_sl, ad_hit, out, rec_pre, rec_post, counters, err, n_cu, st, tn_flags);
            if (e != hipErrorNotSupported) { g_last_trim_kernel = "trim_lds"; g_last_trim_folded = e == hipSuccess && faqcs_trim_lds_tail_folded(); return e; }
        }
    }
    g_last_trim_kernel = "trim_filter_accumulate";
    const bool windowed = P.has_adapters || ((P.trim5 || P.trim3) && !P.qc_only);
    const bool generic = !(P.mode == FAQCS_MODE_BWA_PLUS && !P.protect5 && !P.qc_only && P.replace_q == 0 && !P.avgq_on &&
                           P.max_poly_n == 2 && P.dbg == 0);
    constexpr int NW = FAQCS_TRIM_NW;
#define FAQCS_TRIM_ARGS P, seq, qual, off, n_reads, ad_sl, ad_hit, out, rec_pre, rec_post, counters, err, n_cu, st
    if (max_len <= 64) return launch_trim_variant<16, 4, NW>(windowed, generic, FAQCS_TRIM_ARGS);
    if (max_len <= 76) return launch_trim_variant<19, 4, NW>(windowed, generic, FAQCS_TRIM_ARGS);
    if (max_len <= 104) return launch_trim_variant<13, 8, NW>(windowed, generic, FAQCS_TRIM_ARGS);
    if (max_len <= 128) return launch_trim_variant<16, 8, NW>(windowed, generic, FAQCS_TRIM_ARGS);
    if (max_len <= 152) return launch_trim_variant<19, 8, NW>(windowed, generic, FAQCS_TRIM_ARGS);
    if (max_len <= 160) return launch_trim_variant<20, 8, NW>(windowed, generic, FAQCS_TRIM_ARGS);
    if (max_len <= 208) return launch_trim_variant<13, 16, NW>(windowed, generic, FAQCS_TRIM_ARGS);
    if (max_len <= 256) return launch_trim_variant<16, 16, NW>(windowed, generic, FAQCS_TRIM_ARGS);
    if (max_len <= 320) return launch_trim_variant<10, 32, NW>(windowed, generic, FAQCS_TRIM_ARGS);
    if (max_len <= 512)
        return (windowed || generic) ? launch_trim_t<16, 32, NW, true, true>(FAQCS_TRIM_ARGS) : launch_trim_t<16, 32, NW, false, false>(FAQCS_TRIM_ARGS);
    if (max_len <= 768) return launch_trim_t<12, 64, NW, true, true>(FAQCS_TRIM_ARGS);
    if (max_len <= 1024) return launch_trim_t<16, 64, 8, true, true>(FAQCS_TRIM_ARGS);
#undef FAQCS_TRIM_ARGS
    return hipErrorInvalidValue;
}

hipError_t faqcs_launch_composition(const unsigned long long *rec_pre, const unsigned long long *rec_post, uint32_t n, bool wide,
                                    const float *comp_norm, uint64_t *dst_pre, uint64_t *dst_post, int n_cu, hipStream_t st)
{
    if (n == 0) return hipSuccess;
    constexpr int NT = 1024;
    constexpr size_t lds = (size_t)((FAQCS_NCOMP_BIN * FAQCS_NCOMP_KIND + 1) / 2) * 4 + (size_t)(FAQCS_TAB_LEN + 1) * 4;
    static unsigned long long attr_done_w = 0, attr_done_n = 0;
    auto kern = wide ? composition_histogram<NT, true> : composition_histogram<NT, false>;
    if (hipError_t e = ensure_dynamic_lds(reinterpret_cast<const void *>(kern), lds, wide ? attr_done_w : attr_done_n); e != hipSuccess) return e;
    uint32_t per_array = (n + NT * FAQCS_COMP_U - 1) / (NT * FAQCS_COMP_U);
    if (per_array > (uint32_t)(n_cu / 2)) per_array = (uint32_t)(n_cu / 2);
    if (per_array < 1) per_array = 1;
    hipLaunchKernelGGL(kern, dim3(2 * per_array), dim3(NT), lds, st, rec_pre, rec_post, n, comp_norm, dst_pre, dst_post);
    return hipGetLastError();
}
```

faqcs_amd/csrc/faqcs_trim_lds_kernel.hip:

```cpp
#include "faqcs_trim_common.h"

#include <stdlib.h>
#include <type_traits>

#ifndef FAQCS_LDS_SUM_UNROLL
#define FAQCS_LDS_SUM_UNROLL 4
#endif
#ifndef FAQCS_LDS16_RPC
#define FAQCS_LDS16_RPC 32
#endif
#ifndef FAQCS_LDS16_NW
#define FAQCS_LDS16_NW 12
#endif
#ifndef FAQCS_LDS_SA_UNROLL
#define FAQCS_LDS_SA_UNROLL 2
#endif

namespace {

constexpr int lds_cq(int C, int LPR = 8) { return C == 19 ? 20 : C; }
constexpr int lds_qstride(int C, int LPR = 8) { return LPR == 16 ? lds_cq(C, LPR) + 1 : lds_cq(C, LPR); }
constexpr int lds_wq(int C, int LPR = 8) { return (LPR == 16 || C == 19) ? (LPR * lds_qstride(C, LPR) + 31) / 32 * 32 : 0; }
constexpr int lds_nrot(int C, int LPR = 8) { return LPR == 16 ? 2 : (C == 19 ? 4 : 1); }
constexpr int lds_maxlen(int C, int LPR = 8) { return LPR * C <= 252 ? LPR * C : (LPR * C == 256 ? 252 : LPR * C); }
constexpr bool lds_wide(int C, int LPR = 8) { return lds_maxlen(C, LPR) > 252; }

template <int C, int NW, int LPR = 8, int RPC = 64> struct LdsCfg {
    using Row = RowCfg<C, LPR, lds_wq(C, LPR)>;
    static constexpr int CQ = lds_cq(C, LPR);
    static constexpr int QSTRIDE = lds_qstride(C, LPR);
    static constexpr int NROT = lds_nrot(C, LPR);
    static constexpr bool ROT = NROT > 1;
    static constexpr int W = Row::W;
    static constexpr int MAXLEN = lds_maxlen(C, LPR);
    static constexpr int ND = (W + 3) / 4;
    static constexpr int NP = (W + 15) / 16;
    static constexpr int NWORD = (ND * 4 + 31) / 32;
    static constexpr int O_T2 = (Row::LDS_DWORDS + 3) & ~3;
    static constexpr int O_T3 = O_T2 + 512;
    static constexpr int O_CTR = O_T3 + 512;
    static constexpr int O_TBQ = O_CTR + 8;
    static constexpr int O_STG = O_TBQ + (ROT ? NROT * (CQ + 1) * 8 : 0);
    static constexpr int PADLEN = MAXLEN / 32 * 32;
    static constexpr int STG_BYTES = RPC * (PADLEN + 16 > MAXLEN ? PADLEN + 16 : MAXLEN) + 32;
    static constexpr int STG_DW = (STG_BYTES + 15) / 16 * 4;
    static constexpr int TAIL_PAD = W + 64 > 256 ? (W + 64) / 4 : 64;
    static constexpr int lds_dwords() { return O_STG + NW * STG_DW + TAIL_PAD; }
};

typedef uint32_t LdsPair2 __attribute__((ext_vector_type(2)));
typedef const __attribute__((address_space(3))) LdsPair2 *lds_u2c_ptr;
typedef __attribute__((address_space(3))) uint8_t *lds_u8_mut;
typedef const __attribute__((address_space(3))) uint8_t *lds_u8_ptr;
struct __attribute__((packed, aligned(1))) U32u { uint32_t w; };
typedef const __attribute__((address_space(3))) U32u *lds_u32u_ptr;

__device__ __forceinline__ uint32_t lds_ld(uint32_t byte_offset) { return *(lds_u32_ptr)(size_t)byte_offset; }
__device__ __forceinline__ uint32_t lds_ld_any(uint32_t byte_offset)
{
    const uint32_t a4 = byte_offset & ~3u;
    return __builtin_amdgcn_alignbyte(lds_ld(a4 + 4u), lds_ld(a4), byte_offset & 3u);
}
__device__ __forceinline__ uint32_t lds_ld_u8(uint32_t byte_offset) { return (uint32_t) * (lds_u8_ptr)(size_t)byte_offset; }
__device__ __forceinline__ void lds_st_u8(uint32_t byte_offset, uint32_t v) { *(lds_u8_mut)(size_t)byte_offset = (uint8_t)v; }

template <int K> __device__ __forceinline__ uint32_t byte_x8(uint32_t w, uint32_t three)
{
    uint32_t r;
    if (K == 0) asm("v_lshlrev_b32_sdwa %0, %1, %2 dst_sel:DWORD dst_unused:UNUSED_PAD src0_sel:DWORD src1_sel:BYTE_0" : "=v"(r) : "v"(three), "v"(w));
    else if (K == 1) asm("v_lshlrev_b32_sdwa %0, %1, %2 dst_sel:DWORD dst_unused:UNUSED_PAD src0_sel:DWORD src1_sel:BYTE_1" : "=v"(r) : "v"(three), "v"(w));
    else if (K == 2) asm("v_lshlrev_b32_sdwa %0, %1, %2 dst_sel:DWORD dst_unused:UNUSED_PAD src0_sel:DWORD src1_sel:BYTE_2" : "=v"(r) : "v"(three), "v"(w));
    else asm("v_lshlrev_b32_sdwa %0, %1, %2 dst_sel:DWORD dst_unused:UNUSED_PAD src0_sel:DWORD src1_sel:BYTE_3" : "=v"(r) : "v"(three), "v"(w));
    return r;
}
template <int K> __device__ __forceinline__ uint32_t byte_mul(uint32_t w, uint32_t m)
{
    uint32_t r;
    if (K == 0) asm("v_mul_u32_u24_sdwa %0, %1, %2 dst_sel:DWORD dst_unused:UNUSED_PAD src0_sel:DWORD src1_sel:BYTE_0" : "=v"(r) : "v"(m), "v"(w));
    else if (K == 1) asm("v_mul_u32_u24_sdwa %0, %1, %2 dst_sel:DWORD dst_unused:UNUSED_PAD src0_sel:DWORD src1_sel:BYTE_1" : "=v"(r) : "v"(m), "v"(w));
    else if (K == 2) asm("v_mul_u32_u24_sdwa %0, %1, %2 dst_sel:DWORD dst_unused:UNUSED_PAD src0_sel:DWORD src1_sel:BYTE_2" : "=v"(r) : "v"(m), "v"(w));
    else asm("v_mul_u32_u24_sdwa %0, %1, %2 dst_sel:DWORD dst_unused:UNUSED_PAD src0_sel:DWORD src1_sel:BYTE_3" : "=v"(r) : "v"(m), "v"(w));
    return r;
}
__device__ __forceinline__ uint32_t low_bytes_(int nb) { return nb >= 4 ? 0xffffffffu : ((1u << (8 * nb)) - 1u); }
__device__ __forceinline__ uint32_t bit_range_(int s, int e)
{
    const uint32_t hi = e >= 32 ? 0xffffffffu : ((1u << e) - 1u), lo = s >= 32 ? 0xffffffffu : ((1u << s) - 1u);
    return hi & ~lo;
}

template <bool DESC, int CB>
__device__ __forceinline__ void walk_step(const uint32_t w, const int it, const int c0, const int dc, int &rb, const int rlim, int &a, int &K, int &best)
{
    unsigned long long sv, t;
    int s = uni(it), c = uni(c0);
#define FAQCS_WALK_POS(J, J2, B)                                                                                   \
    "v_cmpx_le_i32 vcc, " #J ", %[rb]\n\t"                                                                         \
    "v_cmp_gt_i32 vcc, 0, %[K]\n\t"                                                                                \
    "v_cmp_le_i32 %[t], %[rlim], %[s]\n\t"                                                                         \
    "s_or_b64 vcc, vcc, %[t]\n\t"                                                                                  \
    "v_cndmask_b32 %[rb], " #J2 ", %[rb], vcc\n\t"                                                                 \
    "v_sub_u32_sdwa %[a], %[a], %[w] dst_sel:DWORD dst_unused:UNUSED_PAD src0_sel:DWORD src1_sel:BYTE_" #B "\n\t"  \
    "v_lshl_add_u32 %[K], %[a], %[cb], %[c]\n\t"                                                                   \
    "v_max_i32 %[best], %[best], %[K]\n\t"                                                                         \
    "s_add_i32 %[s], %[s], 1\n\t"                                                                                  \
    "s_add_i32 %[c], %[c], %[dc]\n\t"
    if (DESC)
        asm volatile("s_mov_b64 %[sv], exec\n\t" FAQCS_WALK_POS(0, 2, 3) FAQCS_WALK_POS(1, 3, 2) FAQCS_WALK_POS(2, 4, 1) FAQCS_WALK_POS(3, 5, 0)
                     "s_mov_b64 exec, %[sv]\n\t"
                     "v_add_u32 %[rb], -4, %[rb]"
                     : [rb] "+v"(rb), [a] "+v"(a), [K] "+v"(K), [best] "+v"(best), [s] "+s"(s), [c] "+s"(c), [sv] "=&s"(sv), [t] "=&s"(t)
                     : [w] "v"(w), [rlim] "v"(rlim), [dc] "s"(dc), [cb] "n"(CB)
                     : "vcc");
    else
        asm volatile("s_mov_b64 %[sv], exec\n\t" FAQCS_WALK_POS(0, 2, 0) FAQCS_WALK_POS(1, 3, 1) FAQCS_WALK_POS(2, 4, 2) FAQCS_WALK_POS(3, 5, 3)
                     "s_mov_b64 exec, %[sv]\n\t"
                     "v_add_u32 %[rb], -4, %[rb]"
                     : [rb] "+v"(rb), [a] "+v"(a), [K] "+v"(K), [best] "+v"(best), [s] "+s"(s), [c] "+s"(c), [sv] "=&s"(sv), [t] "=&s"(t)
                     : [w] "v"(w), [rlim] "v"(rlim), [dc] "s"(dc), [cb] "n"(CB)
                     : "vcc");
#undef FAQCS_WALK_POS
}

template <int NI>
__device__ __forceinline__ void dma_span(const uint8_t *g, const uint32_t nbytes, uint32_t *slot, const int lane)
{
    const uint8_t *gl = g + lane * 16;
    const uint32_t l16 = (uint32_t)lane * 16u;
#pragma unroll
    for (int i = 0; i < NI; ++i) {
        if ((uint32_t)(i * 1024) >= nbytes) break;
        if (l16 < nbytes - (uint32_t)(i * 1024))
            __builtin_amdgcn_global_load_lds((const __attribute__((address_space(1))) void *)(gl + i * 1024),
                                             (__attribute__((address_space(3))) void *)(slot + i * 256), 16, 0, 0);
    }
}

template <int NI>
__device__ __forceinline__ void dma_rows(const uint8_t *g, const uint32_t L, const uint32_t n_rows, uint32_t *slot, const int lane)
{
    const uint32_t U = L / 16u + 1u, total = n_rows * U;
    const uint32_t M = (65536u + U - 1u) / U;
#pragma unroll
    for (int i = 0; i < NI; ++i) {
        if ((uint32_t)(i * 64) >= total) break;
        const uint32_t u = (uint32_t)(i * 64 + lane);
        if (u < total) {
            const uint32_t r = (u * M) >> 16, col = u - r * U;
            __builtin_amdgcn_global_load_lds((const __attribute__((address_space(1))) void *)(g + (size_t)(r * L + col * 16u)),
                                             (__attribute__((address_space(3))) void *)(slot + i * 256), 16, 0, 0);
        }
    }
}

template <int W, int STG_BYTES>
__device__ __forceinline__ void pad_behind_span(const uint32_t slot_b, const uint32_t span, const uint32_t slack, const int lane, const uint32_t in_off)
{
    if ((uint32_t)lane < slack) lds_st_u8(slot_b + (uint32_t)lane, in_off);
    const uint32_t o0 = span + (uint32_t)lane;
#pragma unroll
    for (int i = 0; i < (W + 20 + 63) / 64; ++i)
        if (lane < W + 20 - 64 * i && o0 < (uint32_t)(STG_BYTES - 64 * i)) lds_st_u8((slot_b + o0) + (uint32_t)(64 * i), in_off);
}

struct ExactQ { int sv, svp, mq; };
__device__ __noinline__ ExactQ exact_quality(const uint8_t *__restrict__ qual, const uint32_t v_off, const int len, const uint32_t patch,
                                             const int a, const int n, const int in_off, const bool need)
{
    const int lead = (int)(patch & 0xffffu), trail = (int)(patch >> 16);
    ExactQ r{0, 0, 0};
#pragma unroll 1
    for (int p = 0; __any(need && p < len); ++p) {
        if (need && p < len) {
            int v = (int)(int8_t)qual[(size_t)v_off + p] - in_off;
            if (p < lead || p >= trail) v = 0;
            r.sv += v;
            r.mq = r.mq > v ? r.mq : v;
            if ((unsigned)(p - a) < (unsigned)n) r.svp += v;
        }
    }
    return r;
}
struct ExactB { uint32_t npre, npost; bool trip; };
__device__ __noinline__ ExactB exact_bases(const uint8_t *__restrict__ seq, const uint32_t v_off, const int len, const int a, const int n,
                                           const bool need, const bool dinuc, const uint32_t dthr)
{
    ExactB r{0u, 0u, false};
    uint32_t prev = 4u, dmax = 0;
    uint32_t dc0 = 0, dc1 = 0, dc2 = 0, dc3 = 0;
#pragma unroll 1
    for (int p = 0; __any(need && p < len); ++p) {
        if (need && p < len) {
            const uint32_t b = (uint32_t)seq[(size_t)v_off + p];
            const bool inw = (unsigned)(p - a) < (unsigned)n;
            const uint32_t u = b & 0xdfu;
            const uint32_t isn = u == 'N' ? 1u : 0u;
            r.npre += isn;
            r.npost += inw ? isn : 0u;
            uint32_t cur = u == 'A' ? 0u : u == 'T' ? 1u : u == 'C' ? 2u : u == 'G' ? 3u : 4u;
            if (!inw) cur = 4u;
            if (dinuc && cur < 4u && prev < 4u && cur != prev) {
                const uint32_t k = prev * 4u + cur, sh = 8u * (k & 3u);
                uint32_t &d = (k >> 2) == 0 ? dc0 : (k >> 2) == 1 ? dc1 : (k >> 2) == 2 ? dc2 : dc3;
                uint32_t c = (d >> sh) & 0xffu;
                c = c < 255u ? c + 1u : c;
                d = (d & ~(0xffu << sh)) | (c << sh);
                dmax = dmax > c ? dmax : c;
            }
            prev = cur;
        }
    }
    r.trip = dinuc && dmax >= dthr;
    return r;
}

}

constexpr int lds_waves(int C, int LPR = 8, int RPC = 64) { return LPR == 4 ? 12 : LPR == 16 ? (RPC == 64 ? 6 : (C == 19 ? 12 : FAQCS_LDS16_NW)) : (C <= 19 ? 12 : 8); }

template <int C, int LPR, int NW>
__device__ __noinline__ void flush_block_partial(uint32_t *smem, uint32_t *__restrict__ row, const int tid)
{
    using Cfg = RowCfg<C, LPR, lds_wq(C, LPR)>;
    constexpr int N4 = (Cfg::N_ZERO + 3) / 4;
    static_assert(N4 * 4 <= FAQCS_PARTIAL_ROW, "partial-sum row");
    __syncthreads();
    for (int i = tid; i < N4; i += NW * 64) {
        const uint4 v = reinterpret_cast<const uint4 *>(smem)[i];
        reinterpret_cast<uint4 *>(row)[i] = v;
        if (4 * i + 3 < Cfg::N_ZERO) reinterpret_cast<uint4 *>(smem)[i] = make_uint4(0u, 0u, 0u, 0u);
        else for (int k = 4 * i; k < Cfg::N_ZERO; ++k) smem[k] = 0u;
    }
    __syncthreads();
}

template <int C, int LPR>
__global__ __launch_bounds__(1024) void fold_partials(const uint32_t *__restrict__ partials, const uint32_t *__restrict__ rows_used, const uint32_t n_blocks,
                                                      uint64_t *__restrict__ counters, const faqcs_layout lay, uint32_t *__restrict__ g_next)
{
    using Cfg = RowCfg<C, LPR, lds_wq(C, LPR)>;
    constexpr int W = Cfg::W;
    constexpr int CQ = lds_cq(C, LPR), QSTRIDE = lds_qstride(C, LPR);
    if (blockIdx.x == 0 && threadIdx.x == 0) *g_next = 0u;
    __shared__ unsigned long long part[2][16][64];
    const int i = blockIdx.x * 64 + (threadIdx.x & 63);
    unsigned long long lo = 0, hi = 0;
    if (i < Cfg::N_ZERO) {
        const bool halves = i < Cfg::O_BQPRE;
        for (uint32_t b = threadIdx.x >> 6; b < n_blocks; b += 16) {
            const uint32_t cnt = rows_used[b];
            const uint32_t *row = partials + (size_t)b * FAQCS_PARTIAL_FLUSHES * FAQCS_PARTIAL_ROW + i;
            for (uint32_t k = 0; k < cnt; ++k) {
                const uint32_t x = row[(size_t)k * FAQCS_PARTIAL_ROW];
                if (halves) { lo += x & 0xffffu; hi += x >> 16; } else lo += x;
            }
        }
    }
    part[0][threadIdx.x >> 6][threadIdx.x & 63] = lo;
    part[1][threadIdx.x >> 6][threadIdx.x & 63] = hi;
    __syncthreads();
    if (threadIdx.x >= 64 || i >= Cfg::N_ZERO) return;
    lo = 0; hi = 0;
#pragma unroll
    for (int g = 0; g < 16; ++g) { lo += part[0][g][threadIdx.x]; hi += part[1][g][threadIdx.x]; }
    if (!(lo | hi)) return;
    const uint64_t filter_stats = lay.filter_stats, pre_read_qhist = lay.pre_read_qhist, pre_base_qhist = lay.pre_base_qhist,
                   post_read_qhist = lay.post_read_qhist, post_base_qhist = lay.post_base_qhist, pre_len_hist = lay.pre_len_hist,
                   post_len_hist = lay.post_len_hist, pre_qual = lay.pre_qual, post_qual = lay.post_qual, pre_base = lay.pre_base,
                   post_base = lay.post_base;
    const uint32_t R = lay.max_read_length;
    auto add = [&](uint64_t idx, unsigned long long v) { if (v) atomicAdd((unsigned long long *)(counters + idx), v); };
    if (i < Cfg::O_HB) {
        const uint32_t q = (uint32_t)(i - Cfg::O_HQ) / Cfg::WQ, cell = (uint32_t)(i - Cfg::O_HQ) % Cfg::WQ;
        const uint32_t p = QSTRIDE == CQ ? cell : ((cell % QSTRIDE < (uint32_t)CQ && cell / QSTRIDE < (uint32_t)LPR) ? cell / QSTRIDE * CQ + cell % QSTRIDE : R);
        if (p < R) { add(pre_qual + (uint64_t)p * FAQCS_NQ + q, lo); add(post_qual + (uint64_t)p * FAQCS_NQ + q, hi); }
    } else if (i < Cfg::O_LEN) {
        const uint32_t c = (uint32_t)(i - Cfg::O_HB) / W, p = (uint32_t)(i - Cfg::O_HB) % W;
        if (p < R) { add(pre_base + (uint64_t)p * FAQCS_NBASE + c, lo); add(post_base + (uint64_t)p * FAQCS_NBASE + c, hi); }
    } else if (i < Cfg::O_RQ) {
        const uint32_t l = (uint32_t)(i - Cfg::O_LEN);
        if (l <= R) { add(pre_len_hist + l, lo); add(post_len_hist + l, hi); }
    } else if (i < Cfg::O_BQPRE) {
        const uint32_t k = (uint32_t)(i - Cfg::O_RQ);
        if (k < FAQCS_NQ) { add(pre_read_qhist + k, lo); add(post_read_qhist + k, hi); }
    } else if (i < Cfg::O_BQPOST) {
        add(pre_base_qhist + (uint32_t)(i - Cfg::O_BQPRE), lo);
    } else if (i < Cfg::O_FS) {
        add(post_base_qhist + (uint32_t)(i - Cfg::O_BQPOST), lo);
    } else {
        const uint32_t k = (uint32_t)(i - Cfg::O_FS);
        if (k < FAQCS_NUM_STAT) add(filter_stats + k, lo);
    }
}

template <int C, int NW, int LPR, int RPC> constexpr bool lds_tail_folds_v =
    LdsCfg<C, NW, LPR, RPC>::lds_dwords() >= (FAQCS_NCOMP_BIN * FAQCS_NCOMP_KIND + 1) / 2 + 512 + 8 && lds_maxlen(C, LPR) <= 256;
template <int C, int NW, bool WINDOWED, bool EXT, int LPR, int RPC>
__global__ __launch_bounds__(NW * 64, NW / 4) void trim_lds(
    const DevParams P, const uint8_t *__restrict__ seq, const uint8_t *__restrict__ qual,
    const uint32_t *__restrict__ off, const uint32_t n_reads, const uint32_t *__restrict__ ad_sl,
    const uint16_t *__restrict__ ad_hit, uint2 *__restrict__ out, unsigned long long *__restrict__ rec_pre,
    unsigned long long *__restrict__ rec_post, uint64_t *__restrict__ counters, uint32_t *__restrict__ err,
    const uint8_t *__restrict__ tn_flags)
{
    static_assert(LPR == 8 || (LPR == 16 && (C == 16 || C == 19)) || (LPR == 4 && (C == 13 || C == 19)), "lanes per read");
    using Cfg = RowCfg<C, LPR, lds_wq(C, LPR)>;
    static_assert(RPC <= 64 && (RPC * LPR) % 64 == 0, "reads per chunk: the same number for every row of LPR lanes");
    using T = LdsCfg<C, NW, LPR, RPC>;
    using RW = RowOps<LPR>;
    constexpr int TPR = RPC * LPR / 64;
    constexpr int D = Cfg::D, W = Cfg::W, ND = T::ND, NWORD = T::NWORD, NPOS = ND * 4, BMW = Cfg::BMW;
    constexpr int NI = (T::STG_BYTES + 1023) / 1024;
    constexpr bool WIDE = lds_wide(C, LPR);
    constexpr int AB = WIDE ? 9 : 8;
    constexpr uint32_t AM = (1u << AB) - 1u;
    constexpr int FB = 2 * AB;
    constexpr int CB = WIDE ? 9 : 8, CMAX = (1 << CB) - 1;
    static_assert(!Cfg::HQ8 && T::MAXLEN <= CMAX - 1, "step indices must fit the code field of the argmax keys");
    static_assert(T::lds_dwords() * 4 <= 160 * 1024, "LDS");
    extern __shared__ __attribute__((aligned(16))) uint32_t smem[];
    uint32_t *hb = smem + Cfg::O_HB;
    const uint32_t *t_lc = smem + Cfg::O_TLC;
    const uint32_t *t_bm = smem + Cfg::O_TBM;

#ifdef FAQCS_LDS_STAMPS
    const unsigned long long clk_entry = __builtin_amdgcn_s_memtime();
#endif
    const int tid = threadIdx.x;
    const int lane = tid & 63;
    const int rl = lane & (LPR - 1);
    const int rowb = lane & (64 - LPR);
    const int wave = uni(tid >> 6);
    const int pbase = rl * C;
    const bool owner = RPC == 64 || rl < TPR;
    const uint32_t ridx = RPC == 64 ? (uint32_t)lane : (uint32_t)((lane / LPR) * TPR + rl);

    for (int i = tid; i < Cfg::N_ZERO; i += NW * 64) smem[i] = 0u;
    for (int i = tid; i < 256; i += NW * 64) {
        const uint32_t w = P.base_tab[i];
        smem[T::O_T2 + 2 * i] = ((w >> BT_SHIFT(0)) & 1u) | (((w >> BT_SHIFT(1)) & 1u) << 8) | (((w >> BT_SHIFT(2)) & 1u) << 16) | (((w >> BT_SHIFT(3)) & 1u) << 24);
        smem[T::O_T2 + 2 * i + 1] = (w >> 31) | (((w >> BT_SHIFT(4)) & 1u) << 1);
    }
    for (int i = tid; i < 256; i += NW * 64) {
        const uint32_t f = P.base_tab[(i & 128) ? ((i ^ 0x88) & 127) : i] & BT_FIELDS;
        smem[T::O_T3 + 2 * i] = f;
        smem[T::O_T3 + 2 * i + 1] = i < 128 ? f : 0u;
    }
    for (int i = tid; i <= W; i += NW * 64) {
        smem[Cfg::O_TLC + i] = P.lc_thr[i];
        smem[Cfg::O_TAVGQ + i] = (uint32_t)P.avgq_min_v[i];
        smem[Cfg::O_TMAGIC + i] = P.div_magic[i];
    }
    for (int i = tid; i < BMW * (C + 2); i += NW * 64) {
        const int nb = med3i((i / BMW) - 4 * (i % BMW), 0, 4);
        smem[Cfg::O_TBM + i] = nb >= 4 ? 0xffffffffu : ((1u << (8 * nb)) - 1u);
    }
    constexpr int CQ = T::CQ;
    constexpr bool ROT = T::ROT;
    static_assert((CQ + 3) / 4 == D && (!ROT || CQ % 4 == 0), "Q-B works on the same number of dwords per lane");
    static_assert(T::QSTRIDE * LPR <= Cfg::WQ, "quality rows");
    const int pbase_q = rl * CQ;
    const uint32_t rot = ROT ? (uint32_t)((lane / LPR) & (T::NROT - 1)) : 0u;
    if (ROT) {
        for (int i = tid; i < T::NROT * (CQ + 1) * 8; i += NW * 64) {
            const int r_ = i / ((CQ + 1) * 8), vb_ = (i / 8) % (CQ + 1), k_ = i % 8;
            uint32_t w_ = 0;
            for (int b_ = 0; b_ < 4; ++b_)
                if (4 * k_ + b_ < CQ && (4 * k_ + b_ + r_) % CQ < vb_) w_ |= 0xffu << (8 * b_);
            smem[T::O_TBQ + i] = w_;
        }
    }
    uint32_t three = 3u, wx4 = (uint32_t)(Cfg::WQ * 4);
    asm volatile("" : "+v"(three), "+v"(wx4));
    if (tid == 0 && blockIdx.x == 0 && (uint32_t)(size_t)((lds_u32_ptr)smem) != 0u) atomicOr(err, 4u);
    const uint32_t total_chunks = (n_reads + RPC - 1) / RPC;
    const uint32_t n_groups = (total_chunks + NW - 1) / NW;
    uint32_t *g_next = err + 8;
    if (tid == 0) {
        smem[T::O_CTR] = (uint32_t)NW;
        smem[T::O_CTR + 1] = 0xffffffffu;
        smem[T::O_CTR + 4] = blockIdx.x;
        smem[T::O_CTR + 5] = 0xffffffffu; smem[T::O_CTR + 6] = 0xffffffffu; smem[T::O_CTR + 7] = 0xffffffffu;
        const uint32_t g1 = gridDim.x + atomicAdd(g_next, 1u);
        if (g1 < n_groups) smem[T::O_CTR + 5] = (1u << 20) | g1; else smem[T::O_CTR + 1] = (uint32_t)NW;
    }
    __syncthreads();

#ifdef FAQCS_LDS_TEST_FLUSH_CHUNKS
    constexpr uint32_t FLUSH_CHUNKS = (uint32_t)(FAQCS_LDS_TEST_FLUSH_CHUNKS) / NW * NW;
#else
    constexpr uint32_t FLUSH_CHUNKS = 65535u / RPC / NW * NW;
#endif
    constexpr uint32_t MAX_GROUPS = (uint32_t)FAQCS_PARTIAL_FLUSHES * FLUSH_CHUNKS / NW;
    constexpr uint32_t REG_FLUSH_EVERY = 63 / TPR;
    constexpr uint32_t NO_CHUNK = 0xffffffffu;
    auto lds_word = [&](const int i) { return uniu(*(volatile const __attribute__((address_space(3))) uint32_t *)(size_t)(uint32_t)((T::O_CTR + i) * 4)); };
    auto chunk_of = [&](const uint32_t c_) -> uint32_t {
        const uint32_t L = c_ / NW;
        for (;;) {
            if (c_ >= lds_word(1)) return NO_CHUNK;
            const uint32_t e = lds_word(4 + (int)(L & 3u));
            if ((e >> 20) == (L & 0xfffu)) return (e & 0xfffffu) * NW + c_ % NW;
            __builtin_amdgcn_s_sleep(8);
        }
    };

    const int in_off = P.in_off, Q = P.Q;
    uint32_t *slot = smem + T::O_STG + wave * T::STG_DW;
    const uint32_t slot_b = (uint32_t)(T::O_STG + wave * T::STG_DW) * 4u;
    const uint32_t offb = ((uint32_t)in_off & 0xffu) * 0x01010101u;
    const bool swar_ok = in_off >= 0 && in_off <= 86;
    const uint32_t hq_lane = (uint32_t)(Cfg::O_HQ * 4 + rl * T::QSTRIDE * 4) + rot * 4u - (uint32_t)in_off * (uint32_t)(Cfg::WQ * 4);
    const uint32_t *t_bmq = ROT ? smem + T::O_TBQ + rot * (uint32_t)((CQ + 1) * 8) : t_bm;
    constexpr int BMQ = ROT ? 8 : BMW, VQ = ROT ? CQ : C + 1;
    uint32_t bpre[C], bpost[C];
#pragma unroll
    for (int j = 0; j < C; ++j) { bpre[j] = 0; bpost[j] = 0; }
    uint32_t any_err = 0;
    FsAcc fs_acc;
    auto spill_base_regs = [&]() {
        uint32_t sh_c[FAQCS_NBASE], ad_c[FAQCS_NBASE], lane_o = (uint32_t)lane;
        asm volatile("" : "+v"(lane_o));
        const uint32_t hb_lane_o = (uint32_t)(Cfg::O_HB * 4) + (lane_o & (uint32_t)(LPR - 1)) * (uint32_t)(C * 4);
#pragma unroll
        for (int c = 0; c < FAQCS_NBASE; ++c) {
            uint32_t cp = (uint32_t)c + (lane_o / (uint32_t)LPR) % FAQCS_NBASE;
            cp = cp >= FAQCS_NBASE ? cp - FAQCS_NBASE : cp;
            sh_c[c] = cp * 6u;
            ad_c[c] = hb_lane_o + cp * (uint32_t)(W * 4);
        }
#pragma unroll
        for (int j = 0; j < C; ++j) {
            const uint32_t x = bpre[j], y = bpost[j];
#pragma unroll
            for (int c = 0; c < FAQCS_NBASE; ++c) {
                const uint32_t v = ((x >> sh_c[c]) & 63u) | (((y >> sh_c[c]) & 63u) << 16);
                lds_add_u32_quiet(ad_c[c] + (uint32_t)(j * 4), v);
            }
            bpre[j] = 0; bpost[j] = 0;
        }
        fs_acc_flush(fs_acc, lane, smem + Cfg::O_FS);
        asm volatile("s_waitcnt lgkmcnt(0)" ::: "memory");
    };

    struct RawB { uint32_t r[D + 1], mv[D], mh[D], ml[D]; };
    auto load_b = [&](const uint32_t i0, const uint32_t i1, RawB &x) {
        const int len = (int)(i0 >> 16), a = (int)(i1 & AM), n = (int)((i1 >> AB) & AM);
        const bool post = ((i1 >> FB) & 1u) != 0u, counted = ((i1 >> (FB + 1)) & 1u) != 0u;
        const int vb = counted ? med3i(len - pbase_q, 0, VQ) : 0;
        const int lo = post ? med3i(a - pbase_q, 0, VQ) : 0, hi = post ? med3i(a + n - pbase_q, 0, VQ) : 0;
#ifdef FAQCS_LDS_DIAG_LINEAR_LOADS
        const uint32_t qa = slot_b + (uint32_t)lane * 4u;
#pragma unroll
        for (int k = 0; k <= D; ++k) x.r[k] = lds_ld(qa + 256u * (uint32_t)k);
#else
        const uint32_t qa = (slot_b + (i0 & 0xffffu) + (uint32_t)pbase_q) & ~3u;
#pragma unroll
        for (int k = 0; k <= D; ++k) x.r[k] = lds_ld(qa + 4u * (uint32_t)k);
#endif
#pragma unroll
#ifdef FAQCS_LDS_DIAG_UNIFORM_MASKROWS
        for (int k = 0; k < D; ++k) { x.mv[k] = t_bmq[BMQ * VQ + k]; x.mh[k] = t_bmq[BMQ * VQ + k]; }
#else
        for (int k = 0; k < D; ++k) { x.mv[k] = t_bmq[BMQ * vb + k]; x.mh[k] = t_bmq[BMQ * hi + k]; }
#endif
        if (__any(lo != 0)) {
#pragma unroll
            for (int k = 0; k < D; ++k) x.ml[k] = t_bmq[BMQ * lo + k];
        } else {
#pragma unroll
            for (int k = 0; k < D; ++k) x.ml[k] = 0u;
        }
    };
#ifdef FAQCS_LDS_DIAG_CHECK_QB_ADDR
    unsigned long long *dbg_qb_bad = reinterpret_cast<unsigned long long *>(err + 16) + 3;
#endif
    uint32_t qb_sum = 0;
    auto quality_cells = [&](const RawB &x, const uint32_t i0, const uint32_t i1, auto undo_t, const int t, const bool sum) {
        constexpr bool undo = decltype(undo_t)::value;
        const uint32_t sh = ((i0 & 0xffffu) + (uint32_t)pbase_q + slot_b) & 3u;
        uint32_t cm[D], im[D], wq[D];
#pragma unroll
        for (int k = 0; k < D; ++k) {
            cm[k] = !undo ? x.mv[k] & 0x01010101u : 0u;
            im[k] = (x.mh[k] ^ x.ml[k]) & (undo ? 0xffffffffu : 0x01010101u);
            wq[k] = __builtin_amdgcn_alignbyte(x.r[k + 1], x.r[k], sh);
        }
        if (ROT) {
            uint32_t w0 = wq[0];
#pragma unroll
            for (int k = 0; k < D; ++k) wq[k] = __builtin_amdgcn_alignbyte(k + 1 < D ? wq[k + 1] : w0, wq[k], rot);
        }
        if (!undo && sum) {
            uint32_t qs = 0;
#pragma unroll
            for (int k = 0; k < D; ++k) {
                uint32_t m = x.mv[k];
                if (4 * k + 4 > CQ) m &= low_bytes_(CQ - 4 * k);
                qs = __builtin_amdgcn_sad_u8(wq[k] & m, 0u, qs);
            }
            qs = (uint32_t)RW::all_sum((int)qs);
            qb_sum = (rl == t) ? qs : qb_sum;
        }
#pragma unroll
        for (int j = 0; j < CQ; ++j) {
            const uint32_t b = (uint32_t)(j & 3);
            const uint32_t sel = undo ? (((b) << 24) | ((b) << 16) | 0x0c0cu) : ((0x0cu << 24) | (b << 16) | (0x0cu << 8) | (4u + b));
            const uint32_t data = __builtin_amdgcn_perm(cm[j >> 2], im[j >> 2], sel);
            const uint32_t ad = ((j & 3) == 0 ? byte_mul<0>(wq[j >> 2], wx4) : (j & 3) == 1 ? byte_mul<1>(wq[j >> 2], wx4)
                                 : (j & 3) == 2 ? byte_mul<2>(wq[j >> 2], wx4) : byte_mul<3>(wq[j >> 2], wx4)) +
                                ((ROT && j >= CQ - (T::NROT - 1) && rot >= (uint32_t)(CQ - j)) ? hq_lane - (uint32_t)(CQ * 4) : hq_lane);
#ifdef FAQCS_LDS_DIAG_CHECK_QB_ADDR
            {
                const uint32_t a_ = ad + 4u * (uint32_t)j;
                if (a_ < (uint32_t)(Cfg::O_HQ * 4) || a_ >= (uint32_t)((Cfg::O_HQ + Cfg::HQ) * 4)) atomicAdd(dbg_qb_bad, 1ull);
                else if (lane == 0 && j == 0) atomicAdd(dbg_qb_bad + 1, 1ull);
            }
#endif
#ifdef FAQCS_LDS_QB_NOCONFLICT
            lds_add_u32((ad & 0x3u) + (uint32_t)(Cfg::O_HQ * 4) + (uint32_t)lane * 4u + 256u * (uint32_t)j, data);
#elif !defined(FAQCS_LDS_NO_QB_ATOMICS)
            lds_add_u32(ad + 4u * (uint32_t)j, data);
#else
            asm volatile("" :: "v"(ad), "v"(data));
#endif
        }
    };
    uint32_t tot_pe = 0, tot_po = 0, tot_ce = 0, tot_co = 0;
    uint32_t tot_pn = 0;
    uint32_t seen7 = 0;
    bool pairhit = false;
// ... 567 lines not shown
#pragma unroll
                        for (int wd = 0; wd < NWORD; ++wd) {
                            if (8 * wd < kmax) {
                                uint32_t nw = 0;
#pragma unroll 2
                                for (int k = 8 * wd; k < 8 * wd + 8 && k < ND; ++k) {
                                    uint32_t w = lds_ld_any(slot_b + rows + 4u * (uint32_t)k) & low_bytes_(med3i(len - 4 * k, 0, 4));
                                    w ^= 0x4e4e4e4eu;
                                    const uint32_t nz = ((w & 0x7f7f7f7fu) + 0x7f7f7f7fu) | w;
                                    nw |= ((((~nz & 0x80808080u) >> 7) * 0x00204081u >> 21) & 0xfu) << (4 * (k & 7));
                                }
                                nub[wd] = scan ? nw : 0u;
                            }
                        }
                    }
                    if (P.max_poly_n != 0u) {
#pragma unroll
                        for (int w = 0; w < NWORD; ++w) run[w] = nub[w] & bit_range_(med3i(a - 32 * w, 0, 32), med3i(a + n - 32 * w, 0, 32));
#pragma unroll 1
                        for (uint32_t i = 1; i < P.max_poly_n && i <= (uint32_t)NPOS; ++i) {
                            uint32_t carry = 0;
#pragma unroll
                            for (int w = 0; w < NWORD; ++w) {
                                const uint32_t shifted = (run[w] << 1) | carry;
                                carry = run[w] >> 31;
                                run[w] = shifted & nub[w] & bit_range_(med3i(a - 32 * w, 0, 32), med3i(a + n - 32 * w, 0, 32));
                            }
                        }
#pragma unroll
                        for (int w = 0; w < NWORD; ++w) hit |= run[w];
                    }
                    polyn = P.max_poly_n == 0u || (hit != 0u && P.max_poly_n <= (uint32_t)NPOS);
                } else {
                    polyn = pairhit;
                }
                if (ret && polyn) {
                    flags |= FAQCS_F_POLY_N_SEEN;
                    if (do_trim) { ret = false; filt = FAQCS_FILT_POLY_N; }
                }
                if (EXT && ret && avgq_fail) { ret = false; filt = FAQCS_FILT_AVG_Q; }

                bool lc_trip = false, dinuc = false;
                uint32_t dthr = 0;
                if (ret) {
                    const uint32_t thr = t_lc[n];
                    const uint32_t mthr = thr & 0xffffu;
                    dthr = thr >> 16;
                    lc_trip = cA >= mthr || cT >= mthr || cG >= mthr || cC >= mthr;
                    dinuc = !lc_trip && ((cA >= dthr) + (cT >= dthr) + (cC >= dthr) + (cG >= dthr)) >= 2;
                }
                bool dinuc_general = false;
                if (__any(dinuc)) {
                    const int ncand = (int)(cA >= dthr) + (int)(cT >= dthr) + (int)(cC >= dthr) + (int)(cG >= dthr);
                    dinuc_general = dinuc && ncand > 2;
                    const bool two = dinuc && ncand == 2;
                    const uint32_t mA = cA >= dthr ? 0x000000ffu : 0u, mT = cT >= dthr ? 0x0000ff00u : 0u, mC = cC >= dthr ? 0x00ff0000u : 0u,
                                   mG = cG >= dthr ? 0xff000000u : 0u;
                    const uint32_t both = mA | mT | mC | mG;
                    const uint32_t mx = (both & 0xffu) ? 0xffu : (both & 0xff00u) ? 0xff00u : (both & 0xff0000u) ? 0xff0000u : (both ? 0xff000000u : 0u);
                    const uint32_t my_ = both & ~mx;
                    uint32_t dxy = 0, dyx = 0, prevx = 0, prevy = 0;
                    const int k0 = a >> 2, k1 = (a + n + 3) >> 2;
                    const int kmax2 = uni((int)wave_max_u32((uint32_t)(two && k1 > k0 ? k1 - k0 : 0)));
#pragma unroll 1
                    for (int i = 0; i < kmax2; ++i) {
                        const int k = k0 + i;
                        const uint32_t w = lds_ld_any(slot_b + rows + 4u * (uint32_t)k);
#pragma unroll
                        for (int j = 0; j < 4; ++j) {
                            const int p = 4 * k + j;
                            const uint32_t ad = (j == 0 ? byte_x8<0>(w, three) : j == 1 ? byte_x8<1>(w, three)
                                                 : j == 2 ? byte_x8<2>(w, three) : byte_x8<3>(w, three)) + (uint32_t)(T::O_T2 * 4);
                            uint32_t ex = ((lds_u2c_ptr)(size_t)ad)->x;
                            ex = ((unsigned)(p - a) < (unsigned)n) ? ex : 0u;
                            const uint32_t isx = (ex & mx) ? 1u : 0u, isy = (ex & my_) ? 1u : 0u;
                            dxy += prevx & isy;
                            dyx += prevy & isx;
                            prevx = isx; prevy = isy;
                        }
                    }
                    if (two) lc_trip = lc_trip || dxy >= dthr || dyx >= dthr;
                }
                if (__any(dinuc_general)) {
                    const ExactB xb = exact_bases(seq, v_off, len, a, n, dinuc_general, dinuc_general, dthr);
                    if (dinuc_general) lc_trip = lc_trip || xb.trip;
                }
                if (ret && lc_trip) { ret = false; filt = FAQCS_FILT_LOW_COMPLEXITY; }
            }

            FAQCS_STAMP(7)
            const bool veto = retc && !ret;
            if (__any(veto)) {
                const uint32_t vi1 = (uint32_t)a | ((uint32_t)n << AB) | (veto ? 1u << FB : 0u) | (veto ? 1u << (FB + 1) : 0u);
                FAQCS_S_LOOP(vi1, 1)
                asm volatile("s_waitcnt lgkmcnt(0)" ::: "memory");
                stage(qual, cs, ce, shq, pad_len);
                asm volatile("s_waitcnt vmcnt(0)" ::: "memory");
#ifdef FAQCS_LDS_DIAG_VERIFY_RESTAGE
                if (!pad_len) {
                    const uint32_t nb_ = ce - cs + shq;
                    uint32_t bad_ = 0, first_ = 0xffffffffu;
                    for (uint32_t u_ = (uint32_t)lane; u_ * 16u < nb_; u_ += 64u) {
                        const uint4 g_ = *reinterpret_cast<const uint4 *>(qual + cs - shq + (size_t)u_ * 16u);
                        const uint32_t l0_ = lds_ld(slot_b + u_ * 16u), l1_ = lds_ld(slot_b + u_ * 16u + 4u), l2_ = lds_ld(slot_b + u_ * 16u + 8u), l3_ = lds_ld(slot_b + u_ * 16u + 12u);
                        if (g_.x != l0_ || g_.y != l1_ || g_.z != l2_ || g_.w != l3_) { ++bad_; first_ = first_ == 0xffffffffu ? u_ : first_; }
                    }
                    if (bad_) {
                        atomicAdd(reinterpret_cast<unsigned long long *>(err + 16), (unsigned long long)bad_);
                        atomicMax(reinterpret_cast<unsigned long long *>(err + 16) + 1, ((unsigned long long)nb_ << 32) | first_);
                    }
                    atomicAdd(reinterpret_cast<unsigned long long *>(err + 16) + 2, 1ull);
                }
#endif
                pad_behind_span<W, T::STG_BYTES>(slot_b, pad_len ? (uint32_t)(RPC - 1) * pad_stride + pad_len + shq : ce - cs + shq, shq, lane, (uint32_t)in_off);
                if (__any((veto && tn) || badq)) {
#pragma unroll 1
                    for (int p = 0; __any(((veto && tn) || badq) && p < len); ++p) {
                        if (((veto && tn) || badq) && p < len) {
                            const uint32_t r = lds_ld_u8(slot_b + rowq + (uint32_t)p);
                            int v = (int)(int8_t)r - in_off;
                            v = v < 0 ? 0 : (v > 41 ? 41 : v);
                            if (p < (int)(v_patch & 0xffffu) || p >= (int)(v_patch >> 16)) v = 0;
                            lds_st_u8(slot_b + rowq + (uint32_t)p, (uint32_t)(v + in_off));
                        }
                    }
                }
                const uint32_t ui1 = (uint32_t)a | ((uint32_t)n << AB) | (veto ? 1u << FB : 0u);
#pragma unroll 1
                for (int t = 0; t < TPR; ++t) {
                    const uint32_t i1 = (uint32_t)__shfl((int)ui1, rowb + t);
                    if (!__any(((i1 >> FB) & 1u) != 0u)) continue;
                    const uint32_t i0 = (uint32_t)__shfl((int)qi0, rowb + t);
                    RawB x;
                    load_b(i0, i1, x);
                    quality_cells(x, i0, i1, std::true_type{}, t, false);
                }
                asm volatile("s_waitcnt lgkmcnt(0)" ::: "memory");
            }
#undef FAQCS_S_LOOP

            ChunkLoads ld_next = ld;
            pre_issued = chunk_next != NO_CHUNK;
            if (pre_issued) issue_loads(chunk_next, p_off, p_end, any_err >> 1, ld_next);
            any_err &= 1u;

            if (read_err) { any_err = 1; flags |= FAQCS_F_ERR_QUALITY; }
            oc.an = (uint32_t)a | ((uint32_t)n << 16);
            oc.fl = flags | (ret ? FAQCS_F_VALID : 0u) | (filt << FAQCS_F_FILTER_SHIFT);
            oc.pAT = pA | (pT << 16); oc.pCG = pC | (pG << 16);
            oc.cAT = cA | (cT << 16); oc.cCG = cC | (cG << 16);
            oc.N = pN | (cN << 16);
            oc.Vpre = V_pre; oc.Vpost = V_post;

            chunk_epilogue<LPR>(oc, mine, my, v_len, v_hit, lane, smem + Cfg::O_LEN, smem + Cfg::O_RQ, smem + Cfg::O_BQPRE,
                                smem + Cfg::O_BQPOST, smem + Cfg::O_FS, smem + Cfg::O_TMAGIC, out, rec_pre, rec_post, EXT && P.avgq_on != 0, 0u, &fs_acc,
                                WIDE && P.wide_records != 0u, true);
            ld = ld_next;
            }
        }

        FAQCS_STAMP(8)
        c_cur = c_next; chunk_cur = chunk_next;
    }
    if (__any((any_err & 1u) != 0) && lane == 0) atomicOr(err, 1u);
    if (tid == 0) P.partial_rows[blockIdx.x] = n_flushed;
    if (lds_tail_folds_v<C, NW, LPR, RPC> && P.fold_n) {
        __syncthreads();
        comp_fold_tail<NW * 64>(smem, P, tid, blockIdx.x & 1u);
    }
#ifdef FAQCS_LDS_STAMPS
    if (lane == 0) {
#pragma unroll
        for (int i = 0; i < 9; ++i) atomicAdd(reinterpret_cast<unsigned long long *>(err + 16) + i, st_acc[i]);
        atomicAdd(reinterpret_cast<unsigned long long *>(err + 16) + 9, __builtin_amdgcn_s_memtime() - clk0);
        atomicAdd(reinterpret_cast<unsigned long long *>(err + 16) + 11, st_flush);
#ifdef FAQCS_LDS_BLOCKLOG
        if (wave == 0) printf("block %u xcc %u chunks %u start %llu end %llu\n", blockIdx.x, __builtin_amdgcn_s_getreg((20 << 0) | (0 << 6) | (3 << 11)), smem[T::O_CTR + 1],
                              (unsigned long long)rt0, (unsigned long long)__builtin_amdgcn_s_memrealtime());
#endif
        if (wave == 0) {
            const unsigned long long te = __builtin_amdgcn_s_memrealtime();
            atomicMax(reinterpret_cast<unsigned long long *>(err + 16) + 13, te);
            atomicMax(reinterpret_cast<unsigned long long *>(err + 16) + 14, ~te);
            atomicMax(reinterpret_cast<unsigned long long *>(err + 16) + 15, ~rt0);
        }
        atomicAdd(reinterpret_cast<unsigned long long *>(err + 16) + 12, st_spill);
        (void)clk_entry;
        atomicAdd(reinterpret_cast<unsigned long long *>(err + 16) + 10, __builtin_amdgcn_s_memrealtime() - rt0);
    }
#endif
#undef FAQCS_STAMP
}

__global__ __launch_bounds__(256) void terminal_n_flags(const uint8_t *__restrict__ seq, const uint32_t *__restrict__ off, const uint32_t n, uint8_t *__restrict__ flags)
{
    const uint32_t i = blockIdx.x * 256u + threadIdx.x;
    if (i >= n) return;
    const uint32_t a = off[i], b = off[i + 1];
    flags[i] = b > a ? (uint8_t)((seq[a] == 'N' ? 1u : 0u) | (seq[(size_t)b - 1] == 'N' ? 2u : 0u)) : (uint8_t)0;
}
hipError_t faqcs_launch_terminal_n_flags(const uint8_t *seq, const uint32_t *off, uint32_t n_reads, uint8_t *flags, hipStream_t st)
{
    if (!n_reads) return hipSuccess;
    hipLaunchKernelGGL(terminal_n_flags, dim3((n_reads + 255) / 256), dim3(256), 0, st, seq, off, n_reads, flags);
    return hipGetLastError();
}

static thread_local bool g_trim_lds_tail_folded = false;
bool faqcs_trim_lds_tail_folded() { return g_trim_lds_tail_folded; }
template <int C, bool WINDOWED, bool EXT, int LPR = 8, int RPC = 64>
static hipError_t launch_trim_lds(const DevParams &P, const uint8_t *seq, const uint8_t *qual, const uint32_t *off,
                                  uint32_t n_reads, const uint32_t *ad_sl, const uint16_t *ad_hit, faqcs_read_result *out,
                                  unsigned long long *rec_pre, unsigned long long *rec_post, uint64_t *counters, uint32_t *err,
                                  int n_cu, hipStream_t st, const uint8_t *tn_flags)
{
    constexpr int NW = lds_waves(C, LPR, RPC);
    constexpr size_t lds = (size_t)LdsCfg<C, NW, LPR, RPC>::lds_dwords() * 4;
    static unsigned long long attr_done = 0;
    auto kern = trim_lds<C, NW, WINDOWED, EXT, LPR, RPC>;
    if (hipError_t e = ensure_dynamic_lds(reinterpret_cast<const void *>(kern), lds, attr_done); e != hipSuccess) return e;
    const uint32_t chunks = (n_reads + RPC - 1) / RPC;
    uint32_t grid = (chunks + NW - 1) / NW;
    if (grid > (uint32_t)n_cu) grid = (uint32_t)n_cu;
    if (grid == 0) return hipSuccess;
#ifdef FAQCS_LDS_TEST_FLUSH_CHUNKS
    if ((uint64_t)chunks > (uint64_t)grid * FAQCS_PARTIAL_FLUSHES * ((uint32_t)(FAQCS_LDS_TEST_FLUSH_CHUNKS) / NW * NW)) return hipErrorNotSupported;
#else
    if ((uint64_t)chunks > (uint64_t)grid * FAQCS_PARTIAL_FLUSHES * (65535u / RPC / NW * NW) * 3 / 4) return hipErrorNotSupported;
#endif
    hipLaunchKernelGGL(kern, dim3(grid), dim3(NW * 64), lds, st, P, seq, qual, off, n_reads, ad_sl, ad_hit,
                       reinterpret_cast<uint2 *>(out), rec_pre, rec_post, counters, err, tn_flags);
    if (hipError_t e = hipGetLastError(); e != hipSuccess) return e;
    g_trim_lds_tail_folded = lds_tail_folds_v<C, NW, LPR, RPC> && P.fold_n != 0;
    hipLaunchKernelGGL((fold_partials<C, LPR>), dim3((RowCfg<C, LPR, lds_wq(C, LPR)>::N_ZERO + 63) / 64), dim3(1024), 0, st, P.partials, P.partial_rows, grid, counters, P.lay, err + 8);
    return hipGetLastError();
}

template <int C, int LPR, int RPC, class... Args>
static hipError_t launch_trim_lds_variant(const bool windowed, const bool ext, const Args &...args)
{
    return ext ? (windowed ? launch_trim_lds<C, true, true, LPR, RPC>(args...) : launch_trim_lds<C, false, true, LPR, RPC>(args...))
               : (windowed ? launch_trim_lds<C, true, false, LPR, RPC>(args...) : launch_trim_lds<C, false, false, LPR, RPC>(args...));
}

hipError_t faqcs_launch_trim_lds(const DevParams &P, const uint8_t *seq, const uint8_t *qual, const uint32_t *off,
                                 uint32_t n_reads, uint32_t max_len, const uint32_t *ad_sl, const uint16_t *ad_hit,
                                 faqcs_read_result *out, unsigned long long *rec_pre, unsigned long long *rec_post,
                                 uint64_t *counters, uint32_t *err, int n_cu, hipStream_t st, const uint8_t *tn_flags)
{
    g_trim_lds_tail_folded = false;
    const bool windowed = P.has_adapters || ((P.trim5 || P.trim3) && !P.qc_only);
    const bool plain = P.mode == FAQCS_MODE_BWA_PLUS && !P.protect5 && !P.qc_only && P.replace_q == 0 && !P.avgq_on &&
                       P.max_poly_n == 2 && P.dbg == 0;
    const bool ext = !plain && P.replace_q == 0 && P.dbg == 0;
    if (!plain && !ext) return hipErrorNotSupported;
    DevParams Pw = P;
    Pw.wide_records = max_len > 256 ? 1u : 0u;
    static const bool lds4_on = [] { const char *e = getenv("FAQCS_TRIM_LDS4"); return !e || atoi(e) != 0; }();
    static const bool lds16_on = [] { const char *e = getenv("FAQCS_TRIM_LDS16"); return !e || atoi(e) != 0; }();
    constexpr uint32_t L16 = lds_maxlen(16, 16), L19 = lds_maxlen(19, 16);
#define FAQCS_LDS_ARGS(P) windowed, ext, P, seq, qual, off, n_reads, ad_sl, ad_hit, out, rec_pre, rec_post, counters, err, n_cu, st, tn_flags
    if (lds4_on && max_len > 0 && max_len <= 52) return launch_trim_lds_variant<13, 4, 64>(FAQCS_LDS_ARGS(P));
    if (lds4_on && max_len > 52 && max_len <= 76) return launch_trim_lds_variant<19, 4, 64>(FAQCS_LDS_ARGS(P));
    if (max_len > 76 && max_len <= 104) return launch_trim_lds_variant<13, 8, 64>(FAQCS_LDS_ARGS(P));
    if (max_len > 104 && max_len <= 152) return launch_trim_lds_variant<19, 8, 64>(FAQCS_LDS_ARGS(P));
    if (lds16_on && max_len > 152 && max_len <= L16) return launch_trim_lds_variant<16, 16, FAQCS_LDS16_RPC>(FAQCS_LDS_ARGS(P));
    if (lds16_on && max_len > L16 && max_len <= L19) return launch_trim_lds_variant<19, 16, 20>(FAQCS_LDS_ARGS(Pw));
#undef FAQCS_LDS_ARGS
    return hipErrorNotSupported;
}
```

Before: 8896 M reads/s.

## Count full-length read composition in LDS and skip record writes via chunk flags

Reads whose length equals the max read length (and that stay untrimmed) now have their base-composition histogram counted directly in LDS counters inside the trim kernel. These counts are folded by fold_partials. Each 64-read chunk writes a flag byte saying whether any pre/post records remain. Record stores are skipped for chunks with nothing left, and the composition and tail-fold passes skip loading those records. This targets the memory traffic of writing and re-reading 8-byte composition records, at the cost of extra LDS atomics, a larger LDS row and per-chunk flag writes.

```diff
diff --git a/faqcs_amd/csrc/faqcs_capi.hip b/faqcs_amd/csrc/faqcs_capi.hip
--- a/faqcs_amd/csrc/faqcs_capi.hip
+++ b/faqcs_amd/csrc/faqcs_capi.hip
@@ -216,7 +216,7 @@
     for (auto &sl : c->slot) { sl.seq.release(); sl.qual.release(); sl.tn.release(); sl.off.release(); if (sl.done) (void)hipEventDestroy(sl.done); }
     for (auto &e : c->ticket_ev) if (e) (void)hipEventDestroy(e);
     c->s_seg.release(); c->s_sl.release(); c->s_hit.release(); c->s_res.release(); c->s_astate.release(); c->s_amask.release();
-    for (auto &rs : c->rec) { rs.pre.release(); rs.post.release(); if (rs.trimmed) (void)hipEventDestroy(rs.trimmed); if (rs.folded) (void)hipEventDestroy(rs.folded); }
+    for (auto &rs : c->rec) { rs.pre.release(); rs.post.release(); rs.flags.release(); if (rs.trimmed) (void)hipEventDestroy(rs.trimmed); if (rs.folded) (void)hipEventDestroy(rs.folded); }
     if (c->aux) (void)hipStreamDestroy(c->aux);
     c->ob_items.release(); c->ob_wave_count.release(); c->ob_wave_offset.release();
     { void *kg_ptrs[] = {c->kg.dev.l1, c->kg.dev.l2, c->kg.dev.cur1, c->kg.dev.cur2, c->kg.dev.run_epoch, c->kg.dev.first_hist, c->kg.dev.tot_by_epoch, c->kg.dev.dense, c->kg.dev.big, c->kg.dev.n_big, c->kg.dev.redo};
@@ -293,8 +293,8 @@
     const bool force_long = e_long && atoi(e_long) != 0;
     const bool long_reads = max_len > FAQCS_FAST_READ_LENGTH || force_long;
     const size_t need = long_reads ? (size_t)n / 2 + 1 : (size_t)n * (wide ? 2 : 1);
-    if (need > rs.pre.cap) { HIPCHK(hipStreamSynchronize(c->aux)); HIPCHK(hipStreamSynchronize(c->compute)); }
-    HIPCHK(rs.pre.reserve(need)); HIPCHK(rs.post.reserve(need));
+    if (need > rs.pre.cap || (size_t)n / 64 + 1 > rs.flags.cap) { HIPCHK(hipStreamSynchronize(c->aux)); HIPCHK(hipStreamSynchronize(c->compute)); }
+    HIPCHK(rs.pre.reserve(need)); HIPCHK(rs.post.reserve(need)); HIPCHK(rs.flags.reserve((size_t)n / 64 + 1));
     DevParams dp = c->dp;
     static const bool tail_on = [] { const char *e = getenv("FAQCS_TAIL_FOLD"); return !e || atoi(e) != 0; }();
     if (c->pending_fold >= 0 && !c->pending_wide && tail_on) {
@@ -303,23 +303,26 @@
         HIPCHK(hipMemsetAsync(c->d_fold_claim, 0, 8, c->compute));
         dp.fold_pre = ps.pre.p; dp.fold_post = ps.post.p; dp.fold_n = c->pending_n; dp.fold_claim = c->d_fold_claim;
         dp.fold_dst_pre = c->d_counters + c->lay.pre_comp; dp.fold_dst_post = c->d_counters + c->lay.post_comp;
-    }
+        dp.fold_flags = ps.flagged ? ps.flags.p : nullptr;
+    }
+    static const bool no_comp = [] { const char *e = getenv("FAQCS_DIAG_NO_COMPOSITION"); return e && atoi(e) != 0; }();
+    dp.rec_flags = no_comp ? nullptr : rs.flags.p;
     HIPCHK(faqcs_launch_trim(dp, s.seq, s.qual, s.off, n, max_len, d_sl, d_hit, s.res, rs.pre.p, rs.post.p,
                              c->d_counters, c->d_err, c->n_cu, c->compute, s.tn));
     HIPCHK(hipEventRecord(t.b, c->compute));
     c->trim_kernel = faqcs_last_trim_kernel();
+    rs.flagged = faqcs_last_trim_flagged();
     if (c->pending_fold >= 0) {
         if (!(dp.fold_n && faqcs_last_trim_folded())) {
             faqcs_ctx::RecSet &ps = c->rec[c->pending_fold];
             HIPCHK(hipStreamWaitEvent(c->aux, ps.trimmed, 0));
             HIPCHK(faqcs_launch_composition(ps.pre.p, ps.post.p, c->pending_n, c->pending_wide, c->d_norm, c->d_counters + c->lay.pre_comp,
-                                            c->d_counters + c->lay.post_comp, c->n_cu, c->aux));
+                                            c->d_counters + c->lay.post_comp, c->n_cu, c->aux, ps.flagged ? ps.flags.p : nullptr));
             HIPCHK(hipEventRecord(ps.folded, c->aux));
             ps.used = true;
         }
         c->pending_fold = -1;
     }
-    static const bool no_comp = [] { const char *e = getenv("FAQCS_DIAG_NO_COMPOSITION"); return e && atoi(e) != 0; }();
     if (!(c->dp.dbg & 1u) && !long_reads && !no_comp) {
         HIPCHK(hipEventRecord(rs.trimmed, c->compute));
         c->pending_fold = set; c->pending_n = n; c->pending_wide = wide;
@@ -461,7 +464,7 @@
     if (c->pending_fold < 0) return 0;
     faqcs_ctx::RecSet &ps = c->rec[c->pending_fold];
     HIPCHK(faqcs_launch_composition(ps.pre.p, ps.post.p, c->pending_n, c->pending_wide, c->d_norm, c->d_counters + c->lay.pre_comp,
-                                    c->d_counters + c->lay.post_comp, c->n_cu, c->compute));
+                                    c->d_counters + c->lay.post_comp, c->n_cu, c->compute, ps.flagged ? ps.flags.p : nullptr));
     c->pending_fold = -1;
     return 0;
 }
diff --git a/faqcs_amd/csrc/faqcs_ctx.h b/faqcs_amd/csrc/faqcs_ctx.h
--- a/faqcs_amd/csrc/faqcs_ctx.h
+++ b/faqcs_amd/csrc/faqcs_ctx.h
@@ -25,13 +25,14 @@
 };
 const char *faqcs_last_trim_kernel();
 bool faqcs_last_trim_folded();
+bool faqcs_last_trim_flagged();
 hipError_t faqcs_launch_trim(const DevParams &P, const uint8_t *seq, const uint8_t *qual, const uint32_t *off,
                              uint32_t n_reads, uint32_t max_len, const uint32_t *ad_sl, const uint16_t *ad_hit,
                              faqcs_read_result *out, unsigned long long *rec_pre, unsigned long long *rec_post,
                              uint64_t *counters, uint32_t *err, int n_cu, hipStream_t st, const uint8_t *tn_flags);
 hipError_t faqcs_launch_terminal_n_flags(const uint8_t *seq, const uint32_t *off, uint32_t n_reads, uint8_t *flags, hipStream_t st);
 hipError_t faqcs_launch_composition(const unsigned long long *rec_pre, const unsigned long long *rec_post, uint32_t n, bool wide,
-                                    const float *comp_norm, uint64_t *dst_pre, uint64_t *dst_post, int n_cu, hipStream_t st);
+                                    const float *comp_norm, uint64_t *dst_pre, uint64_t *dst_post, int n_cu, hipStream_t st, const uint8_t *flags = nullptr);
 hipError_t faqcs_launch_adapter(const AdapterDev &A, const AdapterGroup *G, const uint8_t *seq, const uint32_t *off, uint32_t n_reads,
                                 uint32_t max_len, const uint32_t *seg_start, uint32_t n_segments, uint32_t *ad_sl,
                                 uint16_t *ad_hit, uint64_t *adapter_stats, uint32_t *err, uint32_t dbg, int n_cu, hipStream_t st);
@@ -139,7 +140,7 @@
     PackStage render;
     PackStage inflate;
     PackStage deflate;
-    struct RecSet { DevBuf<unsigned long long> pre, post; hipEvent_t trimmed = nullptr, folded = nullptr; bool used = false; };
+    struct RecSet { DevBuf<unsigned long long> pre, post; DevBuf<uint8_t> flags; hipEvent_t trimmed = nullptr, folded = nullptr; bool used = false, flagged = false; };
     RecSet rec[2];
     uint64_t n_enqueued = 0;
     int pending_fold = -1;
diff --git a/faqcs_amd/csrc/faqcs_dev.h b/faqcs_amd/csrc/faqcs_dev.h
--- a/faqcs_amd/csrc/faqcs_dev.h
+++ b/faqcs_amd/csrc/faqcs_dev.h
@@ -29,6 +29,9 @@
     uint32_t fold_n;
     uint32_t *fold_claim;
     uint64_t *fold_dst_pre, *fold_dst_post;
+    const uint8_t *fold_flags;
+    uint8_t *rec_flags;
+    uint32_t comp_len;
 };
 
 #define FAQCS_ADAPTER_GROUP 64
diff --git a/faqcs_amd/csrc/faqcs_trim_common.h b/faqcs_amd/csrc/faqcs_trim_common.h
--- a/faqcs_amd/csrc/faqcs_trim_common.h
+++ b/faqcs_amd/csrc/faqcs_trim_common.h
@@ -17,7 +17,7 @@
 
 namespace {
 
-template <int C, int LPR, int WQ_ = 0> struct RowCfg {
+template <int C, int LPR, int WQ_ = 0, int NCT_ = 0, int TBASE_ = 256> struct RowCfg {
     static constexpr int D = (C + 3) / 4;
     static constexpr int W = LPR * C;
     static constexpr int WQ = WQ_ ? WQ_ : W;
@@ -35,9 +35,11 @@
     static constexpr int O_BQPRE = O_RQ + 42;
     static constexpr int O_BQPOST = O_BQPRE + 42;
     static constexpr int O_FS = O_BQPOST + 42;
-    static constexpr int N_ZERO = O_FS + FS_SLOTS;
+    static constexpr int NCT = NCT_;
+    static constexpr int O_CT = O_FS + FS_SLOTS;
+    static constexpr int N_ZERO = O_CT + NCT;
     static constexpr int O_TBASE = N_ZERO;
-    static constexpr int O_TLC = O_TBASE + 256;
+    static constexpr int O_TLC = O_TBASE + TBASE_;
     static constexpr int O_TAVGQ = O_TLC + W + 1;
     static constexpr int O_TMAGIC = O_TAVGQ + W + 1;
     static constexpr int BMW = D <= 4 ? 4 : 8;
@@ -256,13 +258,21 @@
         defer->tot += mine ? one | e_len : 0u;
 }
 
+struct CompCount {
+    uint32_t ct_b, stride_b;
+    uint32_t Lc;
+    float norm;
+    uint32_t flags_b;
+    uint32_t chunk;
+};
+
 template <int LPR>
 __device__ __forceinline__ void chunk_epilogue(const ReadOutcome &o, const bool mine, const uint32_t my, const uint32_t v_len,
                                                const uint32_t v_hit, const int lane, uint32_t *hlen, uint32_t *hrq, uint32_t *hbqpre,
                                                uint32_t *hbqpost, uint32_t *lfs, const uint32_t *t_magic, uint2 *__restrict__ out,
                                                unsigned long long *__restrict__ rec_pre, unsigned long long *__restrict__ rec_post,
                                                const bool o_avgq_on, const uint32_t o_dbg, FsAcc *defer = nullptr, const bool wide_rt = false,
-                                               const bool pre_done = false)
+                                               const bool pre_done = false, const CompCount *cc = nullptr)
 {
         const bool e_ret = (o.fl & FAQCS_F_VALID) != 0, e_err = (o.fl & FAQCS_F_ERR_QUALITY) != 0;
         const uint32_t e_len = v_len, e_n = o.an >> 16, e_filt = (o.fl & FAQCS_F_FILTER_MASK) >> FAQCS_F_FILTER_SHIFT;
@@ -300,15 +310,40 @@
                 atomicAdd(hbqpost + qb_post, e_n);
             }
         }
+        bool pre_on = !e_err, post_on = e_ret && !e_err;
+        bool row_pre = true, row_post = true;
+        if (cc && cc->Lc != 0xffffffffu) {
+            const uint32_t uA = o.pAT & 0xffffu, uT = o.pAT >> 16, uC = o.pCG & 0xffffu, uG = o.pCG >> 16, uN = o.N & 0xffffu;
+            const bool tab_pre = mine && pre_on && e_len == cc->Lc, tab_post = tab_pre && post_on && e_n == cc->Lc;
+            const uint32_t d = tab_post ? 0x00010001u : 1u;
+            if (tab_pre) {
+                const uint32_t s = uG + uC;
+                const uint32_t dl = (uint32_t)__fmul_rn(cc->norm, (float)s) - (uint32_t)__fmul_rn(cc->norm, (float)uG) - (uint32_t)__fmul_rn(cc->norm, (float)uC) + 1u;
+                lds_add_u32_quiet(cc->ct_b + uA * 4u, d);
+                lds_add_u32_quiet(cc->ct_b + cc->stride_b + uT * 4u, d);
+                lds_add_u32_quiet(cc->ct_b + 2u * cc->stride_b + uC * 4u, d);
+                lds_add_u32_quiet(cc->ct_b + 3u * cc->stride_b + uG * 4u, d);
+                lds_add_u32_quiet(cc->ct_b + (5u + dl) * cc->stride_b + s * 4u, d);
+                if (uN) lds_add_u32_quiet(cc->ct_b + 4u * cc->stride_b + uN * 4u, d);
+            }
+            const unsigned long long z_pre = __ballot(tab_pre && uN == 0u), z_post = __ballot(tab_post && uN == 0u);
+            if (z_pre != 0ull && lane == __builtin_ctzll(z_pre))
+                lds_add_u32_quiet(cc->ct_b + 4u * cc->stride_b, (uint32_t)__popcll(z_pre) | ((uint32_t)__popcll(z_post) << 16));
+            pre_on = pre_on && !tab_pre; post_on = post_on && !tab_post;
+            row_pre = __any(mine && pre_on); row_post = __any(mine && post_on);
+            if (lane == 0) {
+                const uint64_t f = (uint64_t)*(lds_u32_ptr)(size_t)cc->flags_b | ((uint64_t)*(lds_u32_ptr)(size_t)(cc->flags_b + 4u) << 32);
+                reinterpret_cast<uint8_t *>(f)[cc->chunk] = (uint8_t)((row_pre ? 1u : 0u) | (row_post ? 2u : 0u));
+            }
+        }
         if (mine) {
             const bool bad_base = v_hit == 0xffffu;
             out[my] = make_uint2(e_ret ? o.an : 0u, (o.fl & 0x3ffu) | (bad_base ? (uint32_t)FAQCS_F_ERR_BASE : (v_hit << 16)));
-            const bool pre_on = !e_err, post_on = e_ret && !e_err;
             const unsigned long long pA = o.pAT & 0xffffu, pT = o.pAT >> 16, pC = o.pCG & 0xffffu, pG = o.pCG >> 16, pn = o.N & 0xffffu;
             const unsigned long long cA = o.cAT & 0xffffu, cT = o.cAT >> 16, cC = o.cCG & 0xffffu, cG = o.cCG >> 16, cn = o.N >> 16;
             if (LPR <= 16 && !wide_rt) {
-                rec_pre[my] = pre_on ? (CR_VALID | e_len | (pA << 9) | (pT << 18) | (pC << 27) | (pG << 36) | (pn << 45)) : 0ull;
-                rec_post[my] = post_on ? (CR_VALID | e_n | (cA << 9) | (cT << 18) | (cC << 27) | (cG << 36) | (cn << 45)) : 0ull;
+                if (row_pre) rec_pre[my] = pre_on ? (CR_VALID | e_len | (pA << 9) | (pT << 18) | (pC << 27) | (pG << 36) | (pn << 45)) : 0ull;
+                if (row_post) rec_post[my] = post_on ? (CR_VALID | e_n | (cA << 9) | (cT << 18) | (cC << 27) | (cG << 36) | (cn << 45)) : 0ull;
             } else {
                 reinterpret_cast<ulonglong2 *>(rec_pre)[my] =
                     pre_on ? make_ulonglong2(CR_VALID | e_len | (pA << 11) | (pT << 22) | (pC << 33), pG | (pn << 11)) : make_ulonglong2(0ull, 0ull);
@@ -355,6 +390,7 @@
 {
     constexpr int NE = FAQCS_NCOMP_BIN * FAQCS_NCOMP_KIND, ND = (NE + 1) / 2, U = 4;
     constexpr uint32_t CHUNK = NT * U, PER_CLAIM = 5, FLUSH_CLAIMS = 65535u / (CHUNK * PER_CLAIM);
+    static_assert(NT % 64 == 0, "the flag bytes are per 64 records");
     static_assert(FLUSH_CLAIMS >= 1, "a claim must fit the 16-bit counters");
     float *normt = reinterpret_cast<float *>(tab + ND);
     uint32_t *s_next = tab + ND + 512;
@@ -388,7 +424,10 @@
             for (uint32_t c = c0; c < c0 + PER_CLAIM && c < n_chunks; ++c) {
                 unsigned long long x[U];
 #pragma unroll
-                for (int u = 0; u < U; ++u) { const uint32_t i = c * CHUNK + (uint32_t)(u * NT + tid); x[u] = i < n ? rec[i] : 0ull; }
+                for (int u = 0; u < U; ++u) {
+                    const uint32_t i = c * CHUNK + (uint32_t)(u * NT + tid);
+                    x[u] = i < n && (!P.fold_flags || ((P.fold_flags[i >> 6] >> a) & 1u)) ? rec[i] : 0ull;
+                }
 #pragma unroll
                 for (int u = 0; u < U; ++u) {
                     uint32_t nbin = 0xffffffffu;
diff --git a/faqcs_amd/csrc/faqcs_trim_kernel.hip b/faqcs_amd/csrc/faqcs_trim_kernel.hip
--- a/faqcs_amd/csrc/faqcs_trim_kernel.hip
+++ b/faqcs_amd/csrc/faqcs_trim_kernel.hip
@@ -516,8 +516,10 @@
 template <int NT, bool WIDE>
 __global__ __launch_bounds__(NT) void composition_histogram(const unsigned long long *__restrict__ rec_a, const unsigned long long *__restrict__ rec_b,
                                                             const uint32_t n, const float *__restrict__ comp_norm,
-                                                            uint64_t *__restrict__ dst_a, uint64_t *__restrict__ dst_b )
+                                                            uint64_t *__restrict__ dst_a, uint64_t *__restrict__ dst_b ,
+                                                            const uint8_t *__restrict__ flags )
 {
+    static_assert(NT % 64 == 0, "the flag bytes are per 64 records: one for the 64 a wave loads");
     constexpr int NE = FAQCS_NCOMP_BIN * FAQCS_NCOMP_KIND;
     constexpr int ND = (NE + 1) / 2;
     constexpr int U = FAQCS_COMP_U;
@@ -542,7 +544,7 @@
         for (int u = 0; u < U; ++u) {
             const uint32_t i = i0 + u * NT;
             x[u] = 0; y[u] = 0;
-            if (i < n) {
+            if (i < n && (!flags || ((flags[i >> 6] >> (second ? 1 : 0)) & 1u))) {
                 if (WIDE) { const ulonglong2 v = reinterpret_cast<const ulonglong2 *>(rec)[i]; x[u] = v.x; y[u] = v.y; }
                 else x[u] = rec[i];
             }
@@ -639,8 +641,11 @@
 static thread_local const char *g_last_trim_kernel = "";
 const char *faqcs_last_trim_kernel() { return g_last_trim_kernel; }
 bool faqcs_trim_lds_tail_folded();
+bool faqcs_trim_lds_flagged();
 static thread_local bool g_last_trim_folded = false;
 bool faqcs_last_trim_folded() { return g_last_trim_folded; }
+static thread_local bool g_last_trim_flagged = false;
+bool faqcs_last_trim_flagged() { return g_last_trim_flagged; }
 
 hipError_t faqcs_launch_trim(const DevParams &P, const uint8_t *seq, const uint8_t *qual, const uint32_t *off,
                              uint32_t n_reads, uint32_t max_len, const uint32_t *ad_sl, const uint16_t *ad_hit,
@@ -648,6 +653,7 @@
                              uint64_t *counters, uint32_t *err, int n_cu, hipStream_t st, const uint8_t *tn_flags)
 {
     g_last_trim_folded = false;
+    g_last_trim_flagged = false;
     {
         const char *e_long = getenv("FAQCS_TRIM_LONG");
         const bool force_long = e_long && atoi(e_long) != 0;
@@ -660,7 +666,7 @@
         static const bool lds_on = [] { const char *e = getenv("FAQCS_TRIM_LDS"); return !e || atoi(e) != 0; }();
         if (lds_on) {
             const hipError_t e = faqcs_launch_trim_lds(P, seq, qual, off, n_reads, max_len, ad_sl, ad_hit, out, rec_pre, rec_post, counters, err, n_cu, st, tn_flags);
-            if (e != hipErrorNotSupported) { g_last_trim_kernel = "trim_lds"; g_last_trim_folded = e == hipSuccess && faqcs_trim_lds_tail_folded(); return e; }
+            if (e != hipErrorNotSupported) { g_last_trim_kernel = "trim_lds"; g_last_trim_folded = e == hipSuccess && faqcs_trim_lds_tail_folded(); g_last_trim_flagged = e == hipSuccess && faqcs_trim_lds_flagged(); return e; }
         }
     }
     g_last_trim_kernel = "trim_filter_accumulate";
@@ -687,7 +693,7 @@
 }
 
 hipError_t faqcs_launch_composition(const unsigned long long *rec_pre, const unsigned long long *rec_post, uint32_t n, bool wide,
-                                    const float *comp_norm, uint64_t *dst_pre, uint64_t *dst_post, int n_cu, hipStream_t st)
+                                    const float *comp_norm, uint64_t *dst_pre, uint64_t *dst_post, int n_cu, hipStream_t st, const uint8_t *flags)
 {
     if (n == 0) return hipSuccess;
     constexpr int NT = 1024;
@@ -698,6 +704,6 @@
     uint32_t per_array = (n + NT * FAQCS_COMP_U - 1) / (NT * FAQCS_COMP_U);
     if (per_array > (uint32_t)(n_cu / 2)) per_array = (uint32_t)(n_cu / 2);
     if (per_array < 1) per_array = 1;
-    hipLaunchKernelGGL(kern, dim3(2 * per_array), dim3(NT), lds, st, rec_pre, rec_post, n, comp_norm, dst_pre, dst_post);
+    hipLaunchKernelGGL(kern, dim3(2 * per_array), dim3(NT), lds, st, rec_pre, rec_post, n, comp_norm, dst_pre, dst_post, wide ? nullptr : flags);
     return hipGetLastError();
 }
diff --git a/faqcs_amd/csrc/faqcs_trim_lds_kernel.hip b/faqcs_amd/csrc/faqcs_trim_lds_kernel.hip
--- a/faqcs_amd/csrc/faqcs_trim_lds_kernel.hip
+++ b/faqcs_amd/csrc/faqcs_trim_lds_kernel.hip
@@ -25,8 +25,11 @@
 constexpr int lds_maxlen(int C, int LPR = 8) { return LPR * C <= 252 ? LPR * C : (LPR * C == 256 ? 252 : LPR * C); }
 constexpr bool lds_wide(int C, int LPR = 8) { return lds_maxlen(C, LPR) > 252; }
 
+constexpr int lds_nct(int C, int LPR = 8) { return LPR <= 8 ? 9 * (lds_maxlen(C, LPR) + 1) : 0; }
+template <int C, int LPR> using LdsRow = RowCfg<C, LPR, lds_wq(C, LPR), lds_nct(C, LPR), lds_nct(C, LPR) ? 0 : 256>;
+
 template <int C, int NW, int LPR = 8, int RPC = 64> struct LdsCfg {
-    using Row = RowCfg<C, LPR, lds_wq(C, LPR)>;
+    using Row = LdsRow<C, LPR>;
     static constexpr int CQ = lds_cq(C, LPR);
     static constexpr int QSTRIDE = lds_qstride(C, LPR);
     static constexpr int NROT = lds_nrot(C, LPR);
@@ -39,7 +42,7 @@
     static constexpr int O_T2 = (Row::LDS_DWORDS + 3) & ~3;
     static constexpr int O_T3 = O_T2 + 512;
     static constexpr int O_CTR = O_T3 + 512;
-    static constexpr int O_TBQ = O_CTR + 8;
+    static constexpr int O_TBQ = O_CTR + 12;
     static constexpr int O_STG = O_TBQ + (ROT ? NROT * (CQ + 1) * 8 : 0);
     static constexpr int PADLEN = MAXLEN / 32 * 32;
     static constexpr int STG_BYTES = RPC * (PADLEN + 16 > MAXLEN ? PADLEN + 16 : MAXLEN) + 32;
@@ -221,7 +224,7 @@
 template <int C, int LPR, int NW>
 __device__ __noinline__ void flush_block_partial(uint32_t *smem, uint32_t *__restrict__ row, const int tid)
 {
-    using Cfg = RowCfg<C, LPR, lds_wq(C, LPR)>;
+    using Cfg = LdsRow<C, LPR>;
     constexpr int N4 = (Cfg::N_ZERO + 3) / 4;
     static_assert(N4 * 4 <= FAQCS_PARTIAL_ROW, "partial-sum row");
     __syncthreads();
@@ -236,9 +239,10 @@
 
 template <int C, int LPR>
 __global__ __launch_bounds__(1024) void fold_partials(const uint32_t *__restrict__ partials, const uint32_t *__restrict__ rows_used, const uint32_t n_blocks,
-                                                      uint64_t *__restrict__ counters, const faqcs_layout lay, uint32_t *__restrict__ g_next)
-{
-    using Cfg = RowCfg<C, LPR, lds_wq(C, LPR)>;
+                                                      uint64_t *__restrict__ counters, const faqcs_layout lay, uint32_t *__restrict__ g_next,
+                                                      const float *__restrict__ comp_norm, const uint32_t comp_len)
+{
+    using Cfg = LdsRow<C, LPR>;
     constexpr int W = Cfg::W;
     constexpr int CQ = lds_cq(C, LPR), QSTRIDE = lds_qstride(C, LPR);
     if (blockIdx.x == 0 && threadIdx.x == 0) *g_next = 0u;
@@ -246,7 +250,7 @@
     const int i = blockIdx.x * 64 + (threadIdx.x & 63);
     unsigned long long lo = 0, hi = 0;
     if (i < Cfg::N_ZERO) {
-        const bool halves = i < Cfg::O_BQPRE;
+        const bool halves = i < Cfg::O_BQPRE || i >= Cfg::O_CT;
         for (uint32_t b = threadIdx.x >> 6; b < n_blocks; b += 16) {
             const uint32_t cnt = rows_used[b];
             const uint32_t *row = partials + (size_t)b * FAQCS_PARTIAL_FLUSHES * FAQCS_PARTIAL_ROW + i;
@@ -287,9 +291,17 @@
         add(pre_base_qhist + (uint32_t)(i - Cfg::O_BQPRE), lo);
     } else if (i < Cfg::O_FS) {
         add(post_base_qhist + (uint32_t)(i - Cfg::O_BQPOST), lo);
-    } else {
+    } else if (i < Cfg::O_CT) {
         const uint32_t k = (uint32_t)(i - Cfg::O_FS);
         if (k < FAQCS_NUM_STAT) add(filter_stats + k, lo);
+    } else {
+        constexpr uint32_t CTW = Cfg::NCT ? Cfg::NCT / 9 : 1;
+        const uint32_t r = (uint32_t)(i - Cfg::O_CT) / CTW, cnt = (uint32_t)(i - Cfg::O_CT) % CTW;
+        const float norm = comp_norm[comp_len];
+        const uint32_t idx = (uint32_t)__fmul_rn(norm, (float)cnt);
+        const uint32_t e = r < 5 ? idx * FAQCS_NCOMP_KIND + r
+                                 : (idx + 1u - (r - 5u)) * FAQCS_NCOMP_KIND + 5u;
+        if (cnt <= comp_len && e < (uint32_t)(FAQCS_NCOMP_BIN * FAQCS_NCOMP_KIND)) { add(lay.pre_comp + e, lo); add(lay.post_comp + e, hi); }
     }
 }
 
@@ -304,7 +316,7 @@
     const uint8_t *__restrict__ tn_flags)
 {
     static_assert(LPR == 8 || (LPR == 16 && (C == 16 || C == 19)) || (LPR == 4 && (C == 13 || C == 19)), "lanes per read");
-    using Cfg = RowCfg<C, LPR, lds_wq(C, LPR)>;
+    using Cfg = LdsRow<C, LPR>;
     static_assert(RPC <= 64 && (RPC * LPR) % 64 == 0, "reads per chunk: the same number for every row of LPR lanes");
     using T = LdsCfg<C, NW, LPR, RPC>;
     using RW = RowOps<LPR>;
@@ -377,6 +389,9 @@
     const uint32_t n_groups = (total_chunks + NW - 1) / NW;
     uint32_t *g_next = err + 8;
     if (tid == 0) {
+        smem[T::O_CTR + 2] = __float_as_uint(P.comp_norm[P.comp_len]);
+        smem[T::O_CTR + 3] = P.rec_flags ? P.comp_len : 0xffffffffu;
+        smem[T::O_CTR + 8] = (uint32_t)(uintptr_t)P.rec_flags; smem[T::O_CTR + 9] = (uint32_t)((uintptr_t)P.rec_flags >> 32);
         smem[T::O_CTR] = (uint32_t)NW;
         smem[T::O_CTR + 1] = 0xffffffffu;
         smem[T::O_CTR + 4] = blockIdx.x;
@@ -1250,9 +1265,11 @@
             oc.N = pN | (cN << 16);
             oc.Vpre = V_pre; oc.Vpost = V_post;
 
+            const CompCount cc{(uint32_t)(Cfg::O_CT * 4), (uint32_t)(Cfg::NCT / 9 * 4), lds_word(3), __uint_as_float(lds_word(2)), (uint32_t)((T::O_CTR + 8) * 4), chunk};
             chunk_epilogue<LPR>(oc, mine, my, v_len, v_hit, lane, smem + Cfg::O_LEN, smem + Cfg::O_RQ, smem + Cfg::O_BQPRE,
                                 smem + Cfg::O_BQPOST, smem + Cfg::O_FS, smem + Cfg::O_TMAGIC, out, rec_pre, rec_post, EXT && P.avgq_on != 0, 0u, &fs_acc,
-                                WIDE && P.wide_records != 0u, true);
+                                WIDE && P.wide_records != 0u, true,
+                                Cfg::NCT != 0 ? &cc : nullptr);
             ld = ld_next;
             }
         }
@@ -1306,6 +1323,8 @@
 
 static thread_local bool g_trim_lds_tail_folded = false;
 bool faqcs_trim_lds_tail_folded() { return g_trim_lds_tail_folded; }
+static thread_local bool g_trim_lds_flagged = false;
+bool faqcs_trim_lds_flagged() { return g_trim_lds_flagged; }
 template <int C, bool WINDOWED, bool EXT, int LPR = 8, int RPC = 64>
 static hipError_t launch_trim_lds(const DevParams &P, const uint8_t *seq, const uint8_t *qual, const uint32_t *off,
                                   uint32_t n_reads, const uint32_t *ad_sl, const uint16_t *ad_hit, faqcs_read_result *out,
@@ -1330,7 +1349,8 @@
                        reinterpret_cast<uint2 *>(out), rec_pre, rec_post, counters, err, tn_flags);
     if (hipError_t e = hipGetLastError(); e != hipSuccess) return e;
     g_trim_lds_tail_folded = lds_tail_folds_v<C, NW, LPR, RPC> && P.fold_n != 0;
-    hipLaunchKernelGGL((fold_partials<C, LPR>), dim3((RowCfg<C, LPR, lds_wq(C, LPR)>::N_ZERO + 63) / 64), dim3(1024), 0, st, P.partials, P.partial_rows, grid, counters, P.lay, err + 8);
+    g_trim_lds_flagged = lds_nct(C, LPR) != 0 && P.rec_flags != nullptr;
+    hipLaunchKernelGGL((fold_partials<C, LPR>), dim3((LdsRow<C, LPR>::N_ZERO + 63) / 64), dim3(1024), 0, st, P.partials, P.partial_rows, grid, counters, P.lay, err + 8, P.comp_norm, P.comp_len);
     return hipGetLastError();
 }
 
@@ -1347,6 +1367,7 @@
                                  uint64_t *counters, uint32_t *err, int n_cu, hipStream_t st, const uint8_t *tn_flags)
 {
     g_trim_lds_tail_folded = false;
+    g_trim_lds_flagged = false;
     const bool windowed = P.has_adapters || ((P.trim5 || P.trim3) && !P.qc_only);
     const bool plain = P.mode == FAQCS_MODE_BWA_PLUS && !P.protect5 && !P.qc_only && P.replace_q == 0 && !P.avgq_on &&
                        P.max_poly_n == 2 && P.dbg == 0;
@@ -1354,15 +1375,16 @@
     if (!plain && !ext) return hipErrorNotSupported;
     DevParams Pw = P;
     Pw.wide_records = max_len > 256 ? 1u : 0u;
+    Pw.comp_len = max_len;
     static const bool lds4_on = [] { const char *e = getenv("FAQCS_TRIM_LDS4"); return !e || atoi(e) != 0; }();
     static const bool lds16_on = [] { const char *e = getenv("FAQCS_TRIM_LDS16"); return !e || atoi(e) != 0; }();
     constexpr uint32_t L16 = lds_maxlen(16, 16), L19 = lds_maxlen(19, 16);
 #define FAQCS_LDS_ARGS(P) windowed, ext, P, seq, qual, off, n_reads, ad_sl, ad_hit, out, rec_pre, rec_post, counters, err, n_cu, st, tn_flags
-    if (lds4_on && max_len > 0 && max_len <= 52) return launch_trim_lds_variant<13, 4, 64>(FAQCS_LDS_ARGS(P));
-    if (lds4_on && max_len > 52 && max_len <= 76) return launch_trim_lds_variant<19, 4, 64>(FAQCS_LDS_ARGS(P));
-    if (max_len > 76 && max_len <= 104) return launch_trim_lds_variant<13, 8, 64>(FAQCS_LDS_ARGS(P));
-    if (max_len > 104 && max_len <= 152) return launch_trim_lds_variant<19, 8, 64>(FAQCS_LDS_ARGS(P));
-    if (lds16_on && max_len > 152 && max_len <= L16) return launch_trim_lds_variant<16, 16, FAQCS_LDS16_RPC>(FAQCS_LDS_ARGS(P));
+    if (lds4_on && max_len > 0 && max_len <= 52) return launch_trim_lds_variant<13, 4, 64>(FAQCS_LDS_ARGS(Pw));
+    if (lds4_on && max_len > 52 && max_len <= 76) return launch_trim_lds_variant<19, 4, 64>(FAQCS_LDS_ARGS(Pw));
+    if (max_len > 76 && max_len <= 104) return launch_trim_lds_variant<13, 8, 64>(FAQCS_LDS_ARGS(Pw));
+    if (max_len > 104 && max_len <= 152) return launch_trim_lds_variant<19, 8, 64>(FAQCS_LDS_ARGS(Pw));
+    if (lds16_on && max_len > 152 && max_len <= L16) return launch_trim_lds_variant<16, 16, FAQCS_LDS16_RPC>(FAQCS_LDS_ARGS(Pw));
     if (lds16_on && max_len > L16 && max_len <= L19) return launch_trim_lds_variant<19, 16, 20>(FAQCS_LDS_ARGS(Pw));
 #undef FAQCS_LDS_ARGS
     return hipErrorNotSupported;
```

Result: slower. 8536 M reads/s (-4.1%).
